# suchapalaver/krust

Measured on AMD Instinct MI355X. Metric: canonical k-mers/s at k=21, 100M x 150bp reads; bit-exact vs krust CPU, higher is better.
Workload: dtype u64; 1 GPU; S100M: 100000000 x 150 bp reads per GPU (rank r: reads [r x 100000000, (r + 1) x 100000000)), k=21, genome 2^27 bp, seed 20260130; resident in HBM; k=21, reads_per_gpu=100000000, distinct_per_gpu=1085824844, table_slots=2147483648, capacity_hint=1115311478, parallelism=reads sharded x1

## Files before the change

### krust_amd/csrc/batch.hip

```cpp
#include "ctx.hip.h"
#include "level1_api.h"

namespace khi {

template <bool QUAL>
void launch_count(kh_ctx *c, const uint8_t *abase, const uint8_t *qbase, int qaligned, u64 vbeg, u64 vend,
                  u64 wlo, u64 tile0, u64 ntiles) {
    u64 blocks = ntiles < (u64)grid_cap() ? ntiles : (u64)grid_cap();
    uint32_t tpb = (uint32_t)((ntiles + blocks - 1) / blocks);
    blocks = (ntiles + tpb - 1) / tpb;
    uint32_t thr = 0;
    if (QUAL) {
        int t = c->minq + 33;
        thr = (uint32_t)(t > 255 ? 255 : t);
    }
    hipLaunchKernelGGL(kh::count_direct_kernel<QUAL>, dim3((unsigned)blocks), dim3(kh::BLOCK), 0, c->stream, abase,
                       qbase, qaligned, vbeg, vend, wlo, tile0, ntiles, tpb, c->k, thr, table_geom(c, c->table, c->cap), c->d_ctr);
}

struct RangeArgs {
    const uint8_t *abase, *qbase;
    int qaligned;
    bool use_qual;
    u64 vbeg, vend, wlo;
    double survive = 1.0;
};

constexpr int KH_RETRY_FULL_SIZE = 1000;
constexpr int KH_RETRY_WIDE = 1001;

u64 sized_for(u64 n, double survive) {
    if (survive >= 1.0) return n;
    const double e = (double)n * (survive * 1.125 + 1.0 / 64) + 65536.0;
    return e >= (double)n ? n : (u64)e;
}

uint32_t qual_thr(const kh_ctx *c) {
    int t = c->minq + 33;
    return (uint32_t)(t > 255 ? 255 : t);
}

template <typename PT>
void launch_region(kh_ctx *c, const kh::PartGeom &g, u64 nregions, u64 hot, const u64 *bend, bool narrow, u64 skip, u64 expect);
bool region_small_groups(const kh_ctx *c, u64 expect, u64 nregions) {
    const int forced = c->knobs.region_nt;
    if (forced) return forced == 512;
    const double keys = c->est_keys ? (double)(c->distinct_known + c->est_keys) : c->hinted ? (double)c->hint_keys : (double)(c->distinct_known + expect);
    return !(keys > 0.6 * (double)c->cap && expect / nregions > 16384);
}
static bool want_heads(const kh_ctx *c) { return c->comm != nullptr || c->exports_seen || c->knobs.heads_always; }
template <>
void launch_region<u64>(kh_ctx *c, const kh::PartGeom &g, u64 nregions, u64 hot, const u64 *bend, bool, u64 skip, u64 expect) {
    const kh::TableGeom tg = table_geom(c, c->table, c->cap);
#define KH_REGION64(FRESH, NT) \
    hipLaunchKernelGGL((kh::region_count_kernel64<FRESH, NT>), dim3((unsigned)nregions), dim3(NT), 0, c->stream, tg, g, \
                       (const u64 *)c->keysB, bend, (const u64 *)c->bstart, c->rfail, c->rnew, hot, (uint32_t)c->table_dirty, c->rreal, skip)
    if (c->table_empty && region_small_groups(c, expect, nregions)) KH_REGION64(true, 512);
    else if (c->table_empty) KH_REGION64(true, kh::REGION_NT);
    else KH_REGION64(false, kh::REGION_NT);
#undef KH_REGION64
}
template <>
void launch_region<uint32_t>(kh_ctx *c, const kh::PartGeom &g, u64 nregions, u64 hot, const u64 *bend, bool narrow, u64 skip, u64 expect) {
    const kh::TableGeom tg = table_geom(c, c->table, c->cap);
    const int cb = (c->table_empty && !c->shard_shift && want_heads(c)) ? head_count_bits(c, nregions) : -1;
    c->rheads_cb = cb > 0 ? (uint32_t)cb : 0u;
    const bool pow2 = g.p2_bits != 0xFFFFFFFFu;
#define KH_REGION32_P(FRESH, NARROW, NT, DIRTY, CB, RH, P2) \
    hipLaunchKernelGGL((kh::region_count_kernel32<FRESH, NARROW, NT, P2>), dim3((unsigned)nregions), dim3(NT), 0, c->stream, tg, g, \
                       (const uint32_t *)c->keysB, bend, (const u64 *)c->bstart, c->rfail, c->rnew, hot, DIRTY, CB, RH, c->d_ctr, c->rreal, c->ntab, skip, \
                       (bend == (const u64 *)c->bend && g.p1_bits <= kh::MAX_P1_BITS) ? (const uint8_t *)c->heavy : (const uint8_t *)nullptr)
#define KH_REGION32(FRESH, NARROW, NT, DIRTY, CB, RH)                     \
    do {                                                                  \
        if (pow2) KH_REGION32_P(FRESH, NARROW, NT, DIRTY, CB, RH, true);  \
        else KH_REGION32_P(FRESH, NARROW, NT, DIRTY, CB, RH, false);      \
    } while (0)
    const bool small = region_small_groups(c, expect, nregions);
    if (c->table_empty && narrow && small) KH_REGION32(true, true, 512, 1u, c->rheads_cb, c->rheads);
    else if (c->table_empty && narrow) KH_REGION32(true, true, kh::REGION_NT, 1u, c->rheads_cb, c->rheads);
    else if (c->table_empty && small) KH_REGION32(true, false, 512, (uint32_t)c->table_dirty, c->rheads_cb, c->rheads);
    else if (c->table_empty) KH_REGION32(true, false, kh::REGION_NT, (uint32_t)c->table_dirty, c->rheads_cb, c->rheads);
    else if (narrow) KH_REGION32(false, true, kh::REGION_NT, 0u, 0u, (uint32_t *)nullptr);
    else KH_REGION32(false, false, kh::REGION_NT, 0u, 0u, (uint32_t *)nullptr);
#undef KH_REGION32
#undef KH_REGION32_P
}

constexpr double LOAD_SIZED = 0.50;
constexpr double LOAD_KEEP_MAX = 0.53;
constexpr double LOAD_KEEP_MIN = 0.36;
u64 policy_cap(double keys) {
    const u64 cap512 = 512ull * 1024 * kh::REGION_SLOTS;
    const double want = keys / LOAD_SIZED;
    if (want > (double)cap512 && keys / LOAD_KEEP_MAX <= (double)cap512) return cap512;
    return round_cap(std::max(want, (double)(2048ull * kh::REGION_SLOTS)));
}

template <typename PT>
int finish_batch(kh_ctx *c, const kh::PartGeom &g, PT *bufB, const u64 *bend, u64 nregions, u64 n_all, u64 n_ub, u64 ovf_lim, bool heavy_exact) {
    int rc;
    const bool was_empty = c->table_empty;
    const bool narrow_on = c->knobs.narrow;
    bool nar = sizeof(PT) == 4 && narrow_on && !c->narrow_banned && !c->shard_shift && (c->table_empty || c->narrow);
    if (nar && c->ntab_cap != c->cap) {
        if (c->ntab) {
            HIP_TRY(c, hipStreamSynchronize(c->stream));
            (void)dev_free(c->ntab);
            c->ntab = nullptr;
            c->ntab_cap = 0;
        }
        if (dev_malloc((void **)&c->ntab, c->cap * sizeof(u64)) != hipSuccess) {
            (void)hipGetLastError();
            c->ntab = nullptr;
            nar = false;
        } else {
            c->ntab_cap = c->cap;
        }
    }
    if (!nar && c->narrow && (rc = ensure_wide(c)) != KH_OK) return rc;
    if (!nar && (rc = need_table(c)) != KH_OK) return rc;
    if (nar) c->narrow_g = g;
    const u64 hot_cut = [&] {
        if (c->knobs.hot_cut) return c->knobs.hot_cut;
        return std::max<u64>(std::max<u64>(n_all >> 10, 1ull << 20), 64 * (n_all / nregions));
    }();
    if (hot_cut != ~0ull) {
        StageTimer t(c, ST_MISC);
        hipLaunchKernelGGL(kh::hot_list_kernel, dim3((unsigned)((nregions + kh::BLOCK - 1) / kh::BLOCK)), dim3(kh::BLOCK), 0, c->stream,
                           (const u64 *)c->bstart, bend, (u64)nregions, hot_cut, c->hot_list, c->d_ctr);
    }
    {
        StageTimer t(c, ST_REGION);
        launch_region<PT>(c, g, nregions, 4 * (n_ub / nregions) + 4096, bend, nar, hot_cut, n_ub);
    }
    if (nar) c->narrow = true;
    bool heads_marked = false;
    {
        StageTimer t(c, ST_MISC);
        hipLaunchKernelGGL(kh::region_reduce_kernel, dim3((unsigned)std::min<u64>(128, (nregions + kh::BLOCK - 1) / kh::BLOCK)), dim3(kh::BLOCK), 0, c->stream,
                           (const u64 *)c->bstart, (const uint8_t *)c->rfail, (const uint32_t *)c->rnew, (const u64 *)c->rreal, (u64)nregions, c->d_ctr);
        heads_marked = was_empty && sizeof(PT) == 4 && c->rheads_cb != 0 && c->ovf_pending && c->ovf_pending <= (64ull << 20) && !heavy_exact &&
                       mark_touched_regions(c, c->ovf_list, c->ovf, ovf_lim) == KH_OK;
        const int agg_env = c->knobs.ovf_agg;
        const bool ovf_agg = sizeof(PT) == 4 && agg_env != 0 && (agg_env == 1 || c->ovf_pending >= (1u << 16)) &&
                             (!nar || c->h_ctr->kmers + n_all < 0xFFFFFFFFull);
        if (c->ovf_pending && ovf_agg) {
            const unsigned grid = (unsigned)std::min<u64>(2048, (c->ovf_pending + 8191) / 8192);
            if (nar)
                hipLaunchKernelGGL((kh::ovf_agg_insert_kernel<true>), dim3(grid), dim3(kh::OVF_AGG_NT), 0, c->stream, table_geom(c, c->table, c->cap), g,
                                   (const kh::OvfEntry *)c->ovf_list, (const u64 *)c->ovf, ovf_lim, c->d_ctr, c->ntab);
            else
                hipLaunchKernelGGL((kh::ovf_agg_insert_kernel<false>), dim3(grid), dim3(kh::OVF_AGG_NT), 0, c->stream, table_geom(c, c->table, c->cap), g,
                                   (const kh::OvfEntry *)c->ovf_list, (const u64 *)c->ovf, ovf_lim, c->d_ctr, (u64 *)nullptr);
        } else if (c->ovf_pending) {
            if (nar)
                hipLaunchKernelGGL((kh::ovf_insert_kernel<PT, true>), dim3(grid_for(c->ovf_pending)), dim3(kh::BLOCK), 0, c->stream,
                                   table_geom(c, c->table, c->cap), g, c->ovf_list, (const u64 *)c->ovf, ovf_lim, c->d_ctr, c->ntab);
            else
                hipLaunchKernelGGL((kh::ovf_insert_kernel<PT, false>), dim3(grid_for(c->ovf_pending)), dim3(kh::BLOCK), 0, c->stream,
                                   table_geom(c, c->table, c->cap), g, c->ovf_list, (const u64 *)c->ovf, ovf_lim, c->d_ctr, (u64 *)nullptr);
        }
    }
    HIP_TRY(c, hipGetLastError());
    bool heads_recounted = false;
    if (heads_marked) heads_recounted = recount_touched_heads(c, nregions) == KH_OK;
    c->table_empty = false;
    c->table_dirty = false;
    c->launches++;
    c->part_batches++;

    rc = sync_counters(c);
    if (rc != KH_OK) return rc;
    c->rheads_valid = was_empty && sizeof(PT) == 4 && c->rheads_cb != 0 && c->h_ctr->part_failed == 0 && (c->ovf_pending == 0 || heads_recounted) &&
                      !(nar && c->h_ctr->narrow_ovf);
    c->rheads_wide = c->h_ctr->heads_wide != 0;
    if (nar && c->h_ctr->narrow_ovf) {
        if ((rc = ensure_wide(c)) != KH_OK) return rc;
        c->narrow_banned = true;
        HIP_TRY(c, hipMemsetAsync(&c->d_ctr->narrow_ovf, 0, sizeof(u64), c->stream));
        hipLaunchKernelGGL((kh::ovf_insert_kernel<PT, false>), dim3(grid_for(c->ovf_pending)), dim3(kh::BLOCK), 0, c->stream,
                           table_geom(c, c->table, c->cap), g, c->ovf_list, (const u64 *)c->ovf, ovf_lim, c->d_ctr, (u64 *)nullptr);
        HIP_TRY(c, hipGetLastError());
        if ((rc = sync_counters(c)) != KH_OK) return rc;
    }
    if (c->h_ctr->part_failed) {
        std::vector<uint8_t> hf(nregions);
        std::vector<u64> hb(nregions), he(nregions);
        HIP_TRY(c, hipMemcpy(hf.data(), c->rfail, nregions, hipMemcpyDeviceToHost));
        HIP_TRY(c, hipMemcpy(hb.data(), c->bstart, nregions * sizeof(u64), hipMemcpyDeviceToHost));
        HIP_TRY(c, hipMemcpy(he.data(), bend, nregions * sizeof(u64), hipMemcpyDeviceToHost));
        u64 failed_keys = 0;
        bool any_full = false, any_count = false;
        for (u64 r = 0; r < nregions; ++r)
            if (hf[r]) {
                failed_keys += he[r] - hb[r];
                any_full |= hf[r] == 1;
                any_count |= hf[r] == 2;
            }
        if (any_count) c->narrow_banned = true;
        if ((rc = ensure_wide(c)) != KH_OK) return rc;
        u64 newcap = c->cap;
        if (any_full) {
            newcap *= 2;
            while ((double)(c->distinct_known + failed_keys) > LOAD_HARD * (double)newcap ||
                   (double)c->distinct_known > LOAD_TARGET * (double)newcap)
                newcap *= 2;
            c->hinted = false;
        } else {
            while ((double)(c->distinct_known + failed_keys) > LOAD_HARD * (double)newcap) newcap *= 2;
        }
        if (c->trace)
            fprintf(stderr, any_full ? "[kmerhip] %llu regions overflowed (%llu keys): growing and re-inserting them directly\n"
                                     : "[kmerhip] a count left 32 bits in %llu regions (%llu keys): 16-byte table from here on, re-inserting them directly\n",
                    (u64)c->h_ctr->part_failed, failed_keys);
        {
            StageTimer t(c, ST_GROW);
            if (newcap != c->cap) {
                rc = grow_to(c, newcap);
                if (rc != KH_OK) return rc;
            }
            hipLaunchKernelGGL(kh::failed_buckets_insert_kernel<PT>, dim3((unsigned)nregions), dim3(kh::BLOCK), 0, c->stream,
                               table_geom(c, c->table, c->cap), g, (const PT *)bufB, (const u64 *)c->bstart, bend,
                               (const uint8_t *)c->rfail, c->d_ctr);
            HIP_TRY(c, hipMemsetAsync(&c->d_ctr->part_failed, 0, sizeof(u64), c->stream));
        }
        HIP_TRY(c, hipGetLastError());
        rc = sync_counters(c);
        if (rc != KH_OK) return rc;
    }
    if (c->h_ctr->hot) {
        const u64 nhot = c->h_ctr->hot, hot_total = c->h_ctr->hot_total;
        const bool crowded = nhot > nregions / 64 && (double)(c->distinct_known + hot_total) > LOAD_HARD * (double)c->cap;
        const bool hot_narrow = sizeof(PT) == 4 && c->narrow && !crowded && c->h_ctr->kmers + hot_total < 0xFFFFFFFFull;
        if (c->trace)
            fprintf(stderr, "[kmerhip] %llu hot bucket(s) (more than %llu payloads each, %llu together) counted apart from the region pass%s\n", nhot,
                    hot_cut, hot_total, hot_narrow ? ", into the 8-byte image" : "");
        if (!hot_narrow && (rc = ensure_wide(c)) != KH_OK) return rc;
        if (crowded) {
            u64 newcap = c->cap * 2;
            while ((double)(c->distinct_known + hot_total) > LOAD_TARGET * (double)newcap) newcap *= 2;
            StageTimer t(c, ST_GROW);
            if ((rc = grow_to(c, newcap)) != KH_OK) return rc;
        }
        {
            StageTimer t(c, ST_MISC);
            if (hot_narrow)
                hipLaunchKernelGGL((kh::hot_buckets_kernel<PT, sizeof(PT) == 4>), dim3(kh::HOT_GRID), dim3(kh::BLOCK), 0, c->stream, table_geom(c, c->table, c->cap), g,
                                   (const PT *)bufB, (const u64 *)c->bstart, bend, (const uint32_t *)c->hot_list, nhot, c->d_ctr, c->ntab);
            else
                hipLaunchKernelGGL((kh::hot_buckets_kernel<PT, false>), dim3(kh::HOT_GRID), dim3(kh::BLOCK), 0, c->stream, table_geom(c, c->table, c->cap), g,
                                   (const PT *)bufB, (const u64 *)c->bstart, bend, (const uint32_t *)c->hot_list, nhot, c->d_ctr, (u64 *)nullptr);
            HIP_TRY(c, hipMemsetAsync(&c->d_ctr->hot, 0, 2 * sizeof(u64), c->stream));
        }
        HIP_TRY(c, hipGetLastError());
        c->rheads_valid = false;
        if ((rc = sync_counters(c)) != KH_OK) return rc;
    }
    if ((double)c->distinct_known > LOAD_PART * (double)c->cap) {
        u64 newcap = c->cap * 2;
        while ((double)c->distinct_known > LOAD_TARGET * (double)newcap) newcap *= 2;
        StageTimer t(c, ST_GROW);
        rc = grow_to(c, newcap);
        if (rc != KH_OK) return rc;
    }
    return KH_OK;
}

template <typename PT>
int partition_batch(kh_ctx *c, const RangeArgs &ra, GeomChoice &gc, u64 tile0, u64 ntiles, bool size_from_sample, double range_scale, bool sized_narrow, bool may_narrow) {
    constexpr bool CHUNKED = true;
    kh::PartGeom &g = gc.g;
    const u64 P1 = 1ull << g.p1_bits;
    const u64 n_all = ntiles * kh::PART_TILE;
    const bool estimated = ra.survive < 1.0;
    const u64 n_ub = sized_for(n_all, ra.survive);
    const u64 pool_chunks = (n_ub / kh::CHUNK_PAY) + (n_ub / kh::CHUNK_PAY) / 24 + (u64)PART_G1 * (P1 + kh::POOL_GRAB) + 1024;
    const u64 max_blocks = pool_chunks / kh::CPB + P1 + 1;
    int rc;
    {
        auto fixed = [&](auto **ptr, u64 entries, const char *what) -> int {
            u64 z = *ptr ? entries : 0;
            return ensure_buf(c, ptr, &z, entries, what);
        };
        if ((rc = fixed(&c->moff, (u64)kh::MAX_P1 + 1, "hipMalloc(moff)")) != KH_OK) return rc;
        if ((rc = fixed(&c->nch, (u64)kh::MAX_P1 + 1, "hipMalloc(nch)")) != KH_OK) return rc;
        if ((rc = fixed(&c->info, 8, "hipMalloc(info)")) != KH_OK) return rc;
        if ((rc = fixed(&c->pcount, (u64)kh::MAX_P1, "hipMalloc(pcount)")) != KH_OK) return rc;
        if ((rc = fixed(&c->pstart, (u64)kh::MAX_P1 + 1, "hipMalloc(pstart)")) != KH_OK) return rc;
        if ((rc = fixed(&c->pool_next, 1, "hipMalloc(pool_next)")) != KH_OK) return rc;
        if ((rc = fixed(&c->ptotal, (u64)kh::MAX_P1, "hipMalloc(ptotal)")) != KH_OK) return rc;
        if ((rc = fixed(&c->pcap, (u64)kh::MAX_P1, "hipMalloc(pcap)")) != KH_OK) return rc;
        if ((rc = fixed(&c->ovf, 4, "hipMalloc(ovf)")) != KH_OK) return rc;
        if ((rc = fixed(&c->heavy, (u64)kh::MAX_P1, "hipMalloc(heavy)")) != KH_OK) return rc;
    }
    if ((rc = ensure_buf(c, &c->blocks, &c->blocks_cap, max_blocks, "hipMalloc(blocks)")) != KH_OK) return rc;
    if (c->pool_cap < pool_chunks) {
        const u64 have = c->pool_cap;
        c->pool_cap = 0;
        u64 z = c->chunk_part ? have : 0;
        if ((rc = ensure_buf(c, &c->chunk_part, &z, pool_chunks, "hipMalloc(chunk_part)")) != KH_OK) return rc;
        z = c->fill8 ? have : 0;
        if ((rc = ensure_buf(c, &c->fill8, &z, pool_chunks, "hipMalloc(fill8)")) != KH_OK) return rc;
        z = c->plist ? have : 0;
        if ((rc = ensure_buf(c, &c->plist, &z, pool_chunks, "hipMalloc(plist)")) != KH_OK) return rc;
        c->pool_cap = pool_chunks;
    }
    const u64 a_bytes = pool_chunks * kh::CHUNK_PAY * sizeof(PT);
    if (c->key_cap < a_bytes) {
        u64 z = c->keysA ? c->key_cap : 0;
        c->key_cap = 0;
        if ((rc = ensure_buf(c, &c->keysA, &z, a_bytes, "hipMalloc(keysA)")) != KH_OK) return rc;
        c->key_cap = a_bytes;
    }
    const uint32_t est_np = size_from_sample ? (uint32_t)std::min<u64>(16, std::max<u64>(1, (2ull << 20) / std::max<u64>(1, n_ub / P1))) : 0u;
    constexpr uint32_t EST_P0 = 517;
    u64 est_slots = 0;
    uint32_t est_sub = 0;
    if (size_from_sample) {
        while (est_sub < 6 && (n_ub / P1) >> (est_sub + 1) >= (1ull << 19)) ++est_sub;
        est_slots = 1ull << 16;
        while (est_slots < 3 * (u64)est_np * ((n_ub / P1 >> est_sub) + 1)) est_slots *= 2;
        if ((rc = ensure_buf(c, &c->est_set, &c->est_set_cap, est_slots, "hipMalloc(distinct sample)")) != KH_OK) return rc;
    }

    const uint32_t tpb = (uint32_t)((ntiles + PART_G1 - 1) / PART_G1);
    const uint32_t thr = ra.use_qual ? qual_thr(c) : 0;
    const dim3 b1(kh::PART_NT);
    kh::ChunkSrc cs;
    cs.pay = c->keysA;
    cs.plist = c->plist;
    cs.fill8 = c->fill8;
    const uint32_t force_wide = c->knobs.p2_force_wide ? 1u : 0u;
    bool have_total = false;
    u64 batch_total = 0;

    {
        {
            StageTimer t(c, ST_MISC);
            HIP_TRY(c, hipMemsetAsync(c->chunk_part, 0xFF, pool_chunks * sizeof(uint16_t), c->stream));
            HIP_TRY(c, hipMemsetAsync(c->fill8, 0xFF, pool_chunks, c->stream));
            HIP_TRY(c, hipMemsetAsync(c->pcount, 0, kh::MAX_P1 * sizeof(uint32_t), c->stream));
            HIP_TRY(c, hipMemsetAsync(c->pool_next, 0, sizeof(u64), c->stream));
        }
        {
            StageTimer t(c, ST_P1_SCATTER);
            kh::L1Launch l1;
            l1.stream = c->stream;
            l1.grid = (unsigned)PART_G1;
            l1.abase = ra.abase;
            l1.qbase = ra.qbase;
            l1.qaligned = ra.qaligned;
            l1.use_qual = ra.use_qual;
            l1.vbeg = ra.vbeg;
            l1.vend = ra.vend;
            l1.wlo = ra.wlo;
            l1.tile0 = tile0;
            l1.ntiles = ntiles;
            l1.tiles_per_block = tpb;
            l1.k = c->k;
            l1.thr = thr;
            l1.g = g;
            l1.pool = c->keysA;
            l1.chunk_part = c->chunk_part;
            l1.fill8 = c->fill8;
            l1.pool_next = c->pool_next;
            l1.pool_chunks = pool_chunks;
            l1.ctr = c->d_ctr;
            l1.survive = ra.survive;
            l1.generic_k = c->knobs.generic_k;
            l1.legacy = c->knobs.p1_legacy;
            if (sizeof(PT) == 4) kh::launch_level1_32(l1, nullptr);
            else kh::launch_level1_64(l1, nullptr);
        }
#if KH_ABL
        if (c->knobs.stop_after_p1) {
            HIP_TRY(c, hipGetLastError());
            return sync_counters(c);
        }
#endif
        {
            StageTimer t(c, ST_MISC);
            HIP_TRY(c, hipMemsetAsync(c->ptotal, 0, kh::MAX_P1 * sizeof(u64), c->stream));
            hipLaunchKernelGGL(kh::chunk_hist_kernel, dim3(1024), dim3(1024), 0, c->stream, (const uint16_t *)c->chunk_part,
                               (const u64 *)c->pool_next, pool_chunks, c->pcount, (const uint8_t *)c->fill8, c->ptotal);
            if ((rc = device_scan(c, c->pcount, P1, c->pstart)) != KH_OK) return rc;
            hipLaunchKernelGGL(kh::part2_plan_chunked_kernel, dim3(1), dim3(1024), 0, c->stream, (const u64 *)c->pstart, g,
                               c->blocks, max_blocks, c->moff, c->nch, c->info, c->pcount, force_wide, (const uint8_t *)nullptr);
            hipLaunchKernelGGL(kh::chunk_list_kernel, dim3((unsigned)((pool_chunks + 16383) / 16384)), dim3(1024), 0, c->stream,
                               (const uint16_t *)c->chunk_part, (const u64 *)c->pool_next, pool_chunks, c->pcount, c->plist);
            if (size_from_sample) {
                u64 *est_out = c->info + 4;
                HIP_TRY(c, hipMemsetAsync(est_out, 0, 3 * sizeof(u64), c->stream));
                HIP_TRY(c, hipMemsetAsync(c->est_set, 0xFF, est_slots * sizeof(u64), c->stream));
                hipLaunchKernelGGL(kh::distinct_sample_kernel<PT>, dim3(1024), dim3(kh::BLOCK), 0, c->stream, cs, (const u64 *)c->pstart,
                                   EST_P0 % (uint32_t)(P1 - est_np + 1), est_np, est_sub, c->est_set, est_slots - 1, est_out);
            }
        }
        if (estimated || size_from_sample) {
            std::vector<u64> pt(kh::MAX_P1);
            u64 lost = 0, total = 0, est[3] = {0, 0, 0};
            HIP_TRY(c, hipMemcpyAsync(pt.data(), c->ptotal, kh::MAX_P1 * sizeof(u64), hipMemcpyDeviceToHost, c->stream));
            HIP_TRY(c, hipMemcpyAsync(&lost, &c->d_ctr->failed, sizeof(u64), hipMemcpyDeviceToHost, c->stream));
            if (size_from_sample) HIP_TRY(c, hipMemcpyAsync(est, c->info + 4, sizeof(est), hipMemcpyDeviceToHost, c->stream));
            HIP_TRY(c, hipStreamSynchronize(c->stream));
            for (u64 p = 0; p < P1; ++p) total += pt[p];
            have_total = true;
            batch_total = total;
            if (estimated && (lost || total > n_ub)) {
                HIP_TRY(c, hipMemsetAsync(&c->d_ctr->failed, 0, sizeof(u64), c->stream));
                if (c->trace)
                    fprintf(stderr, "[kmerhip] sized for %.3f of the windows (%llu payloads), found %llu%s: again at full size\n", ra.survive, n_ub,
                            total, lost ? " and more that did not fit the pool" : "");
                return KH_RETRY_FULL_SIZE;
            }
            if (size_from_sample) {
                double keys = (double)total;
                if (est[2] == 0 && est[1] > 0) keys = std::min((double)total, (double)est[0] * ((double)P1 / (double)est_np) * (double)(1u << est_sub));
                c->est_keys = (u64)(keys * range_scale) + 1;
                const double load_now = (double)c->est_keys / (double)c->cap;
                u64 newcap = c->cap;
                if (load_now > LOAD_KEEP_MAX || (!c->hinted && (load_now < LOAD_KEEP_MIN || c->cap < 2048ull * kh::REGION_SLOTS))) newcap = policy_cap((double)c->est_keys);
                if (c->hinted && newcap < c->cap) newcap = c->cap;
                newcap = std::min<u64>(newcap, (u64)kh::MAX_P1 * kh::MAX_B2 * kh::REGION_SLOTS);
                size_t fr = 0, tot = 0;
                if (hipMemGetInfo(&fr, &tot) == hipSuccess) {
                    u64 room = ((u64)fr + (c->table ? c->cap * sizeof(Slot) : 0) + (c->ntab ? c->ntab_cap * sizeof(u64) : 0)) / 3;
                    if (c->knobs.table_room_mb) room = c->knobs.table_room_mb << 20;
                    while (newcap > c->cap && newcap * sizeof(Slot) > room) {
                        u64 next = round_cap((double)newcap * 0.8);
                        if (next >= newcap) next = round_cap((double)newcap * 0.5);
                        if (next >= newcap) break;
                        newcap = std::max(next, c->cap);
                    }
                }
                if (sizeof(PT) == 8 && c->knobs.l2_narrow && c->shard_shift == 0 && (newcap & (newcap - 1)) && !c->knobs.table_regions) {
                    u64 p2cap = 2048ull * kh::REGION_SLOTS;
                    uint32_t rb = 11;
                    while (p2cap < newcap) {
                        p2cap <<= 1;
                        ++rb;
                    }
                    const int below = 2 * (int)c->k - (int)rb;
                    size_t fr2 = 0, tot2 = 0;
                    const u64 image_have = c->ntab ? c->ntab_cap * sizeof(u64) : 0, later = 7 * total > c->keyb_cap ? 7 * total - c->keyb_cap : 0;
                    const bool fits = p2cap == c->cap ||
                                      (hipMemGetInfo(&fr2, &tot2) == hipSuccess && p2cap * sizeof(u64) <= ((u64)fr2 + image_have) / 3 &&
                                       (u64)fr2 + image_have >= p2cap * sizeof(u64) + later + (6ull << 30));
                    if (below >= 1 && below <= 32 && rb <= kh::MAX_P1_BITS + kh::MAX_P2_BITS && fits && (!c->hinted || p2cap >= c->cap)) newcap = p2cap;
                }
                if (c->trace)
                    fprintf(stderr, "[kmerhip] %llu payloads, ~%llu distinct (sample: %llu of %llu in %u partition(s)%s): table %llu -> %llu slots, load %.3f\n", total,
                            c->est_keys, est[0], est[1], est_np, est[2] ? ", VOID" : "", c->cap, newcap, (double)c->est_keys / (double)newcap);
                if (newcap != c->cap) {
                    resize_empty_table(c, newcap);
                    c->sized_by_sample = true;
                    const GeomChoice g2 = make_geom(c, c->cap);
                    if (!g2.ok || g2.g.p1_bits != g.p1_bits || g2.use32 != gc.use32) return fail(c, KH_ERR_STATE, "table geometry changed under a running batch");
                    gc = g2;
                }
            }
        }
    }
    const u64 n_pay = have_total ? std::min(n_ub, batch_total) : n_ub;
    const u64 nregions = kh::part_regions(g);
    const u64 n2 = max_blocks * g.b2;
    if (c->h2_cap < n2) {
        const u64 have = c->h2_cap;
        c->h2_cap = 0;
        u64 z = c->H2 ? have : 0;
        if ((rc = ensure_buf(c, &c->H2, &z, n2, "hipMalloc(H2)")) != KH_OK) return rc;
        z = c->O2 ? have + 1 : 0;
        if ((rc = ensure_buf(c, &c->O2, &z, n2 + 1, "hipMalloc(O2)")) != KH_OK) return rc;
        c->h2_cap = n2;
    }
    if ((rc = ensure_region_scratch(c, nregions)) != KH_OK) return rc;
    const bool lines_on = c->knobs.p2_lines;
    const bool lines = lines_on && g.b2 >= 2 && g.b2 <= 512;
    const bool arena_on = c->knobs.l2_arena;
    const bool arena = arena_on && g.p1_bits >= 8 && g.b2 >= 32 && g.b2 <= kh::MAX_B2;
    const u64 arena_pay = arena ? (n_pay + nregions) + ((n_pay + nregions) >> 2) + 1056ull * nregions : 0;
    const u64 ovf_need = arena ? n_pay / 16 + 2 * P1 * 8192ull + (1ull << 20) : 0;
    const u64 pad_ub = lines ? (max_blocks * g.b2) * (u64)(kh::P2L<PT>::UNIT - 1) : 0;
    const u64 heavy_room = arena ? n_pay / 8 : 0;
    const u64 heavy_base = (arena_pay + 31) & ~31ull;
    const u64 heavy_pad = (arena && lines) ? ((heavy_room / (kh::CPB * kh::CHUNK_PAY) + 2 * P1) * g.b2) * (u64)(kh::P2L<PT>::UNIT - 1) : 0;
    const int below_region_bits = 2 * (int)c->k - (int)g.shard_shift - (int)g.p1_bits - (g.p2_bits != 0xFFFFFFFFu ? (int)g.p2_bits : 64);
    const bool can_narrow = sizeof(PT) == 8 && arena && c->knobs.l2_narrow && may_narrow && g.p2_bits != 0xFFFFFFFFu && g.p2_bits >= 5 && g.b2 <= kh::MAX_B2 &&
                            below_region_bits >= 1 && below_region_bits <= 32 && g.shard_shift == 0;
    const u64 b_bytes_wide = std::max((n_pay + pad_ub) * (u64)sizeof(PT), arena ? (heavy_base + heavy_room + heavy_pad + 64) * (u64)sizeof(PT) : 0);
    const u64 b_bytes = can_narrow ? (arena_pay + 64) * (u64)sizeof(uint32_t) : b_bytes_wide;
    auto room_for_wide = [&]() -> int {
        if (c->keyb_cap >= b_bytes_wide) return KH_OK;
        size_t fr = 0, tot = 0;
        if (hipMemGetInfo(&fr, &tot) != hipSuccess) {
            (void)hipGetLastError();
            fr = 0;
        }
        if (sized_narrow && ((u64)fr + c->keyb_cap < b_bytes_wide + (c->table ? 0 : c->cap * sizeof(Slot)) + (4ull << 30) || c->knobs.l2_no_room_wide)) return KH_RETRY_WIDE;
        u64 z = c->keysB ? c->keyb_cap : 0;
        c->keyb_cap = 0;
        const int r = ensure_buf(c, &c->keysB, &z, b_bytes_wide, "hipMalloc(keysB)");
        if (r == KH_OK) c->keyb_cap = b_bytes_wide;
        return r;
    };
    if (!can_narrow) {
        if ((rc = room_for_wide()) != KH_OK) return rc;
    } else if (c->keyb_cap < b_bytes) {
        u64 z = c->keysB ? c->keyb_cap : 0;
        c->keyb_cap = 0;
        if ((rc = ensure_buf(c, &c->keysB, &z, b_bytes, "hipMalloc(keysB)")) != KH_OK) return rc;
        c->keyb_cap = b_bytes;
    }
    PT *bufA = reinterpret_cast<PT *>(c->keysA), *bufB = reinterpret_cast<PT *>(c->keysB);
    if (arena && c->ovf_cap < ovf_need) {
        u64 z = c->ovf_list ? c->ovf_cap : 0;
        c->ovf_cap = 0;
        if ((rc = ensure_buf(c, &c->ovf_list, &z, ovf_need, "hipMalloc(ovf_list)")) != KH_OK) return rc;
        c->ovf_cap = ovf_need;
    }
    const u64 *bend = c->bstart + 1;
    bool arena_done = false, heavy_exact = false;
    const u64 ovf_test_cap = c->knobs.l2_ovf_cap;
    const u64 ovf_lim = std::min(c->ovf_cap, ovf_test_cap);
    bool narrowed = false;
    if (arena) {
        u64 hov[4] = {0, 0, 0, 0};
        for (int attempt = can_narrow ? 0 : 1; attempt < 2; ++attempt) {
            const bool nw = attempt == 0;
            StageTimer t(c, ST_P2_SCATTER);
            const uint32_t skew_x = c->knobs.l2_skew_x >= 0 ? (uint32_t)c->knobs.l2_skew_x : 2u;
            const u64 room = std::min<u64>(heavy_room, c->knobs.l2_heavy_room);
            hipLaunchKernelGGL(kh::arena_plan_kernel, dim3((unsigned)std::min<u64>(64, (nregions + 1023) / 1024)), dim3(1024), 0, c->stream, (const u64 *)c->ptotal, g, c->bstart, c->pcap,
                               c->ovf, skew_x, c->heavy, room);
#define KH_ARENA(UB, NBK, P2)                                                                                                              \
    hipLaunchKernelGGL((kh::part2_arena_kernel<PT, UB, NBK, P2>), dim3((unsigned)P1), dim3(kh::P2L_NT), 0, c->stream, cs, (const u64 *)c->pstart, g, \
                       (const u64 *)c->bstart, (const uint32_t *)c->pcap, bufB, c->bend, c->ovf_list, c->ovf, ovf_lim, (const uint8_t *)c->heavy)
            const bool pow2 = g.p2_bits != 0xFFFFFFFFu;
            constexpr int UB512 = sizeof(PT) == 4 ? KH_ARENA_UNITB : 64;
#define KH_ARENA_NARROW(UB, NBK)                                                                                                           \
    hipLaunchKernelGGL((kh::part2_arena_kernel<uint32_t, UB, NBK, true, u64>), dim3((unsigned)P1), dim3(kh::P2L_NT), 0, c->stream, cs, (const u64 *)c->pstart, g, \
                       (const u64 *)c->bstart, (const uint32_t *)c->pcap, (uint32_t *)c->keysB, c->bend, c->ovf_list, c->ovf, ovf_lim, (const uint8_t *)c->heavy)
            if (nw) {
                if constexpr (sizeof(PT) == 8) {
                    if (g.b2 > 512) KH_ARENA_NARROW(64, 1024);
                    else KH_ARENA_NARROW(KH_ARENA_UNITB, 512);
                }
            } else
            if (g.b2 > 768) {
                if (pow2) KH_ARENA(64, 1024, true);
                else KH_ARENA(64, 1024, false);
            } else if (g.b2 > 512) {
#ifndef KH_ARENA_UNITB_768
#define KH_ARENA_UNITB_768 128
#endif
                if (KH_ARENA_UNITB_768 == 128 && sizeof(PT) == 4 && g.b2 <= 682) KH_ARENA(128, 768, false);
                else KH_ARENA(64, 768, false);
            } else if (pow2) {
                KH_ARENA(UB512, 512, true);
            } else {
                KH_ARENA(UB512, 512, false);
            }
#undef KH_ARENA
#undef KH_ARENA_NARROW
            t.stop();
            HIP_TRY(c, hipMemcpyAsync(hov, c->ovf, sizeof(hov), hipMemcpyDeviceToHost, c->stream));
            HIP_TRY(c, hipStreamSynchronize(c->stream));
            if (nw && (hov[1] != 0 || hov[2] != 0)) {
                if (c->trace) fprintf(stderr, "[kmerhip] level 2 narrowed to 4-byte payloads met %s: again with 8-byte payloads\n", hov[1] ? "a full overflow list" : "heavy partitions");
                if ((rc = room_for_wide()) != KH_OK) return rc;
                bufB = reinterpret_cast<PT *>(c->keysB);
                continue;
            }
            narrowed = nw;
            break;
        }
        if (hov[1] == 0) {
            arena_done = true;
            heavy_exact = hov[2] != 0;
            bend = c->bend;
            c->ovf_pending = std::min<u64>(hov[0], ovf_lim);
            HIP_TRY(c, hipMemsetAsync(c->rfail, 0, nregions, c->stream));
            if (c->trace && c->ovf_pending)
                fprintf(stderr, "[kmerhip] level 2: %llu entries handed out to the overflow list (%.2f %% of the batch's payload room)\n", (u64)c->ovf_pending,
                        100.0 * (double)c->ovf_pending / (double)n_ub);
            if (heavy_exact && c->trace)
                fprintf(stderr, "[kmerhip] %llu heavy level-1 partition(s) (%llu payloads) take the exact level-2 kernels, the others the arenas\n", hov[2], hov[3]);
        } else if (c->trace) {
            fprintf(stderr, hov[1] == 2 ? "[kmerhip] heavy level-1 partitions hold %llu payloads, more than the room behind the arenas: this batch takes the exact level-2 path\n"
                                        : "[kmerhip] level-2 overflow list full (%llu entries): this batch takes the exact path\n", (u64)(hov[1] == 2 ? hov[3] : hov[0]));
        }
    }
    if (!arena_done || heavy_exact) {
    PT *const outB = heavy_exact ? bufB + heavy_base : bufB;
    {
        StageTimer t(c, ST_MISC);
        if (heavy_exact || size_from_sample)
            hipLaunchKernelGGL(kh::part2_plan_chunked_kernel, dim3(1), dim3(1024), 0, c->stream, (const u64 *)c->pstart, g,
                               c->blocks, max_blocks, c->moff, c->nch, c->info, c->pcount, force_wide, heavy_exact ? (const uint8_t *)c->heavy : (const uint8_t *)nullptr);
        HIP_TRY(c, hipMemsetAsync(c->H2, 0, n2 * sizeof(uint32_t), c->stream));
    }
    {
        StageTimer t(c, heavy_exact ? ST_MISC : ST_P2_COUNT);
        hipLaunchKernelGGL((kh::part2_count_kernel<PT, CHUNKED>), dim3((unsigned)max_blocks), b1, 0, c->stream, (const PT *)bufA, cs,
                           (const kh::Part2Block *)c->blocks, (const u64 *)c->info, g, c->H2, lines ? (uint32_t)kh::P2L<PT>::UNIT : 1u);
    }
    {
        StageTimer t(c, ST_MISC);
        if ((rc = device_scan(c, c->H2, n2, c->O2)) != KH_OK) return rc;
    }
    {
        StageTimer t(c, ST_P2_SCATTER);
        const uint32_t fallback = lines ? 1u : 0u;
        if (lines)
            hipLaunchKernelGGL((kh::part2_scatter_lines_kernel<PT, CHUNKED>), dim3((unsigned)max_blocks), dim3(kh::P2L_NT), 0, c->stream,
                               (const PT *)bufA, cs, (const kh::Part2Block *)c->blocks, (const u64 *)c->info, g, (const u64 *)c->O2, outB);
        if (g.b2 <= 512)
            hipLaunchKernelGGL((kh::part2_scatter_kernel<PT, CHUNKED, 512>), dim3((unsigned)max_blocks), dim3(kh::PART2_NT), 0, c->stream,
                               (const PT *)bufA, cs, (const kh::Part2Block *)c->blocks, (const u64 *)c->info, g, (const u64 *)c->O2, outB, fallback);
        else
            hipLaunchKernelGGL((kh::part2_scatter_kernel<PT, CHUNKED, 1024>), dim3((unsigned)max_blocks), dim3(kh::PART2_NT), 0, c->stream,
                               (const PT *)bufA, cs, (const kh::Part2Block *)c->blocks, (const u64 *)c->info, g, (const u64 *)c->O2, outB, fallback);
    }
#if KH_ABL2 || KH_ABL3
    if (c->knobs.stop_after_p2) {
        HIP_TRY(c, hipGetLastError());
        return sync_counters(c);
    }
#endif
    {
        StageTimer t(c, ST_MISC);
        if (heavy_exact) {
            hipLaunchKernelGGL(kh::bucket_bounds_heavy_kernel, dim3((unsigned)((nregions + 255) / 256)), dim3(256), 0, c->stream,
                               (const u64 *)c->O2, (const u64 *)c->moff, (const uint32_t *)c->nch, g, (const uint8_t *)c->heavy, heavy_base,
                               c->bstart, c->bend);
        } else {
            hipLaunchKernelGGL(kh::bucket_bounds_kernel, dim3((unsigned)((nregions + 256) / 256)), dim3(256), 0, c->stream,
                               (const u64 *)c->O2, (u64)n2, (const u64 *)c->moff, (const uint32_t *)c->nch, g, c->bstart);
            HIP_TRY(c, hipMemsetAsync(c->rfail, 0, nregions, c->stream));
        }
    }
    if (!heavy_exact) c->ovf_pending = 0;
    }
    if (narrowed) {
        kh::PartGeom g2 = g;
        g2.p1_bits = g.p1_bits + g.p2_bits;
        g2.b2 = 1;
        g2.b2_magic = kh::part_magic_of(1);
        g2.p2_bits = 0;
        g2.defer = 0;
        c->narrow2_refused = false;
        if (c->trace) fprintf(stderr, "[kmerhip] level 2 narrowed the batch's payloads to the %d bits below the region index\n", below_region_bits);
        return finish_batch<uint32_t>(c, g2, reinterpret_cast<uint32_t *>(c->keysB), bend, nregions, n_all, n_ub, ovf_lim, false);
    }
    return finish_batch<PT>(c, g, bufB, bend, nregions, n_all, n_ub, ovf_lim, heavy_exact);
}

int direct_range(kh_ctx *c, const RangeArgs &ra, u64 first_tile, u64 end_tile) {
    {
        int rc = ensure_wide(c);
        if (rc == KH_OK) rc = clear_if_dirty(c);
        if (rc != KH_OK) return rc;
    }
    u64 t = first_tile;
    u64 sub = SUB_TILES;
    while (t < end_tile) {
        u64 nt = std::min(sub, end_tile - t);
        bool smaller = false;
        int rc = ensure_room(c, nt * kh::TILE, nt > SUB_TILES_MIN, &smaller);
        if (rc != KH_OK) return rc;
        if (smaller) {
            sub = std::max(SUB_TILES_MIN, nt / 4);
            continue;
        }
        {
            StageTimer tm(c, ST_DIRECT);
            if (ra.use_qual) launch_count<true>(c, ra.abase, ra.qbase, ra.qaligned, ra.vbeg, ra.vend, ra.wlo, t, nt);
            else launch_count<false>(c, ra.abase, nullptr, 0, ra.vbeg, ra.vend, ra.wlo, t, nt);
        }
        HIP_TRY(c, hipGetLastError());
        c->table_empty = false;
        c->rheads_valid = false;
        c->launches++;
        c->pending_bound += nt * kh::TILE;
        t += nt;
    }
    return KH_OK;
}

void ensure_part_budget(kh_ctx *c) {
    if (c->part_budget) return;
    size_t fr = 0, tot = 0;
    u64 budget = 224ull << 30;
    const double share = 0.80;
    if (hipMemGetInfo(&fr, &tot) == hipSuccess) {
        budget = std::min<u64>(budget, (u64)((double)(fr + c->key_cap + c->keyb_cap) * share));
        const u64 image = c->ntab ? 0 : 8ull * c->cap;
        if (c->prev_part_budget > budget && (u64)fr + c->key_cap + c->keyb_cap >= c->prev_part_budget + image + (3ull << 30)) budget = c->prev_part_budget;
    } else (void)hipGetLastError();
    if (c->knobs.part_budget_gb > 0) budget = (u64)(c->knobs.part_budget_gb * (double)(1ull << 30));
    c->part_budget = std::max<u64>(budget, 64ull << 20);
}

int count_device_range(kh_ctx *c, const uint8_t *d_bases, const uint8_t *d_qual, u64 n, u64 wlo_off) {
    if (n == 0) return KH_OK;
    const uintptr_t addr = (uintptr_t)d_bases;
    const u64 lead = addr & 15;
    RangeArgs ra;
    ra.abase = d_bases - lead;
    ra.vbeg = lead;
    ra.vend = lead + n;
    ra.wlo = lead + wlo_off;
    ra.use_qual = (d_qual != nullptr) && (c->minq >= 0);
    ra.qbase = nullptr;
    ra.qaligned = 0;
    if (ra.use_qual) {
        ra.qbase = d_qual - lead;
        ra.qaligned = (((uintptr_t)ra.qbase) & 15) == 0;
    }
    const u64 windows = ra.vend - ra.wlo;

    bool part = false;
    if (c->path_mode == 2) part = true;
    else if (c->path_mode == 0) part = windows >= PART_MIN_WINDOWS && (double)c->cap <= 7.0 * (double)windows;
    if (part) ensure_part_budget(c);
    const bool tight = part && (double)windows * 11.0 > 0.85 * (double)c->part_budget;
    if (part && (ra.use_qual || (windows >= (64ull << 20) && (tight || !c->hinted)))) {
        if (c->knobs.survival > 0) {
            ra.survive = std::min(1.0, c->knobs.survival);
        } else {
            const u64 t0 = ra.wlo / kh::TILE, t1 = (ra.vend + kh::TILE - 1) / kh::TILE, stride = 64;
            const u64 nsamp = (t1 - t0 + stride - 1) / stride;
            u64 *d_out = &c->d_ctr->cursor;
            u64 good = 0;
            StageTimer tm(c, ST_MISC);
            HIP_TRY(c, hipMemsetAsync(d_out, 0, sizeof(u64), c->stream));
            if (ra.use_qual)
                hipLaunchKernelGGL(kh::survival_sample_kernel<true>, dim3((unsigned)std::min<u64>(nsamp, 2048)), dim3(kh::BLOCK), 0, c->stream, ra.abase, ra.qbase,
                                   ra.qaligned, ra.vbeg, ra.vend, ra.wlo, t0, t1 - t0, stride, c->k, qual_thr(c), d_out);
            else
                hipLaunchKernelGGL(kh::survival_sample_kernel<false>, dim3((unsigned)std::min<u64>(nsamp, 2048)), dim3(kh::BLOCK), 0, c->stream, ra.abase, (const uint8_t *)nullptr,
                                   0, ra.vbeg, ra.vend, ra.wlo, t0, t1 - t0, stride, c->k, 0u, d_out);
            HIP_TRY(c, hipMemcpyAsync(&good, d_out, sizeof(u64), hipMemcpyDeviceToHost, c->stream));
            HIP_TRY(c, hipStreamSynchronize(c->stream));
            ra.survive = std::min(1.0, (double)good / (double)(nsamp * kh::TILE));
        }
        if (c->trace) fprintf(stderr, "[kmerhip] %s range: %.3f of the windows expected to survive\n", ra.use_qual ? "quality-masked" : "unhinted", ra.survive);
    }
    const bool sample = part && c->estimate_on && c->table_empty && c->shard_shift == 0 && c->k >= kh::MAX_P1_BITS && windows >= PART_MIN_WINDOWS;
    c->est_keys = 0;
    if (sample && c->cap < 2048ull * kh::REGION_SLOTS) {
        HIP_TRY(c, hipStreamSynchronize(c->stream));
        resize_empty_table(c, 2048ull * kh::REGION_SLOTS);
    }
    if (part && !c->hinted && !sample) {
        if (c->pending_bound) {
            int rc = sync_counters(c);
            if (rc != KH_OK) return rc;
        }
        u64 limit = c->cap;
        size_t fr = 0, tot = 0;
        if (hipMemGetInfo(&fr, &tot) == hipSuccess) {
            const u64 bytes = ((u64)fr + (c->table ? c->cap * sizeof(Slot) : 0)) / 4;
            u64 lim = MIN_CAP;
            while (lim * 2 * sizeof(Slot) <= bytes) lim *= 2;
            limit = std::max(limit, lim);
        }
        u64 expect = sized_for(windows, ra.survive);
        if (c->new_rate >= 0.0) expect = std::min<u64>(expect, (u64)((double)windows * std::max(c->new_rate * 1.5, 1.0 / 16)) + (1u << 20));
        const u64 want = std::min(round_cap((double)(c->distinct_known + expect) / LOAD_PART), limit);
        if (want > c->cap) {
            if (c->table_empty) {
                HIP_TRY(c, hipStreamSynchronize(c->stream));
                resize_empty_table(c, want);
            } else {
                StageTimer t(c, ST_GROW);
                int rc = grow_to(c, want);
                if (rc != KH_OK) c->poisoned = false;
            }
        }
    }
    if (part && !make_geom(c, c->cap).ok) part = false;

    if (!part) return direct_range(c, ra, ra.wlo / kh::TILE, (ra.vend + kh::TILE - 1) / kh::TILE);

    if (c->pending_bound) {
        int rc = sync_counters(c);
        if (rc != KH_OK) return rc;
    }
    if (c->borrow_on) {
        int rc = end_borrow(c);
        if (rc != KH_OK) return rc;
    }
    ensure_part_budget(c);
    const u64 first_tile = ra.wlo / kh::PART_TILE;
    const u64 end_tile = (ra.vend + kh::PART_TILE - 1) / kh::PART_TILE;
    const u64 distinct_before = c->distinct_known;
    bool no_narrow = false;
    for (u64 t = first_tile; t < end_tile;) {
        const GeomChoice gc = make_geom(c, c->cap);
        if (!gc.ok) return direct_range(c, ra, t * (kh::PART_TILE / kh::TILE), (ra.vend + kh::TILE - 1) / kh::TILE);
        const int rb_now = (int)kh::kh_floor_log2((uint32_t)std::min<u64>(c->cap / kh::REGION_SLOTS, 1u << 20));
        const bool expect_narrow = !gc.use32 && !no_narrow && !c->narrow2_refused && c->knobs.l2_narrow && c->shard_shift == 0 && c->knobs.l2_arena &&
                                   (c->table_empty ? (sample && 2 * (int)c->k - 20 <= 32) : (cap_is_pow2(c->cap) && rb_now >= 15 && 2 * (int)c->k - rb_now <= 32 && 2 * (int)c->k - rb_now >= 1));
        const u64 per_key = gc.use32 ? 11 : (expect_narrow ? 15 : 20);
        const u64 left = end_tile - t;
        const double share = (double)sized_for(left * kh::PART_TILE, ra.survive) / (double)(left * kh::PART_TILE);
        u64 batch_tiles = std::max<u64>(1, (u64)((double)(c->part_budget / per_key / kh::PART_TILE) / share));
        const u64 nb = (left + batch_tiles - 1) / batch_tiles;
        batch_tiles = (left + nb - 1) / nb;
        const u64 nt = std::min(batch_tiles, left);
        GeomChoice gcb = gc;
        const bool from_sample = sample && t == first_tile && gcb.g.p1_bits == kh::MAX_P1_BITS;
        const double range_scale = (double)(end_tile - first_tile) / (double)nt;
        int rc = gcb.use32 ? partition_batch<uint32_t>(c, ra, gcb, t, nt, from_sample, range_scale, false, false)
                           : partition_batch<u64>(c, ra, gcb, t, nt, from_sample, range_scale, expect_narrow, !no_narrow);
        if (rc == KH_RETRY_FULL_SIZE) {
            ra.survive = 1.0;
            continue;
        }
        if (rc == KH_RETRY_WIDE) {
            no_narrow = true;
            c->narrow2_refused = true;
            {
                size_t fr = 0, tot = 0;
                if (hipMemGetInfo(&fr, &tot) == hipSuccess) {
                    const u64 have = (u64)fr + c->key_cap + c->keyb_cap, tab = c->table ? 0 : c->cap * sizeof(Slot);
                    if (have > tab + (8ull << 30)) c->part_budget = std::min<u64>(c->part_budget, (u64)(0.9 * (double)(have - tab - (8ull << 30))));
                } else (void)hipGetLastError();
            }
            if (c->trace) fprintf(stderr, "[kmerhip] the batch was sized for 4-byte level-2 payloads and cannot have them: again in smaller batches\n");
            continue;
        }
        if (rc != KH_OK) return rc;
        t += nt;
    }
    c->new_rate = (double)(c->distinct_known - distinct_before) / (double)windows;
    return KH_OK;
}


}
```

### krust_amd/csrc/ctx.hip.h

```cpp
#pragma once
#include "../../include/kmerhip.h"

#include <hip/hip_runtime.h>
#include <sys/mman.h>

#include <algorithm>
#include <atomic>
#include <chrono>
#include <cstdio>
#include <cstdlib>
#include <cstring>
#include <functional>
#include <map>
#include <mutex>
#include <new>
#include <string>
#include <thread>
#include <type_traits>
#include <vector>

#include "alloc_inject.h"
#include "kernels.hip.h"
#include "partition.hip.h"

using kh::Counters;
using kh::Slot;
using kh::u64;

namespace khi __attribute__((visibility("hidden"))) {

constexpr double LOAD_HARD = 0.80;
constexpr double LOAD_TARGET = 0.50;
constexpr double HINT_LOAD = 0.65;
constexpr u64 MIN_CAP = 8ull * kh::REGION_SLOTS;
constexpr u64 DEFAULT_CAP = 1ull << 20;
constexpr u64 SUB_TILES = 1ull << 16;
constexpr u64 SUB_TILES_MIN = 1ull << 10;
constexpr u64 STAGE_BYTES = 64ull << 20;
constexpr u64 ACC_MAX = 8ull << 30;
constexpr u64 ACC_MIN = 1ull << 20;
constexpr u64 HALO = 32;
constexpr int GRID_CAP = 256 * 8;
#ifndef KH_ARENA_UNITB
#define KH_ARENA_UNITB 128
#endif
#ifndef KH_PART_G1
#define KH_PART_G1 512
#endif
constexpr int PART_G1 = KH_PART_G1;
constexpr u64 PART_MIN_WINDOWS = 1ull << 22;
constexpr double LOAD_PART = 0.70;
enum { ST_DIRECT = 0, ST_P1_COUNT, ST_P1_SCATTER, ST_P2_COUNT, ST_P2_SCATTER, ST_REGION, ST_MISC, ST_GROW, ST_N, ST_TEXT = ST_N };

struct Comm;

#ifndef KH_TESTING
#define KH_TESTING 0
#endif
struct Knobs {
    bool trace = false;
    int path = 0;
    double part_budget_gb = 0;
    u64 acc_max_mb = 0;
    u64 text_acc_mb = 0;
    int copy_threads = 0;
    bool estimate = true;
    bool pow2_table = false;
    int payload = 0;
    u64 table_regions = 0;
    int region_nt = 0;
    bool p2_force_wide = false;
    bool generic_k = false;
    bool p1_legacy = false;
    bool p2_lines = true;
    bool l2_arena = true;
    u64 l2_ovf_cap = ~0ull;
    int l2_skew_x = -1;
    u64 l2_heavy_room = ~0ull;
    bool narrow = true;
    bool l2_narrow = true;
    bool l2_no_room_wide = false;
    u64 hot_cut = 0;
    int ovf_agg = -1;
    double survival = 0;
    bool heads_always = false;
    u64 table_room_mb = 0;
    bool stop_after_p1 = false, stop_after_p2 = false;
    u64 profile_chunk_kb = 0;
    u64 uni_text_chunk_kb = 0;
};
inline const char *env_of(const char *name) {
    const char *e = getenv(name);
    return (e && *e) ? e : nullptr;
}
void read_knobs(Knobs &k);

#if KH_TESTING
extern std::atomic<int> g_grid_cap;
inline int grid_cap() { return g_grid_cap.load(std::memory_order_relaxed); }
#else
constexpr int grid_cap() { return GRID_CAP; }
#endif

#if KH_TESTING
bool alloc_inject_fails(const char *kind, size_t bytes);
void alloc_trace_event(char ev, const char *kind, const void *p, size_t bytes);
inline hipError_t dev_malloc(void **p, size_t bytes) {
    if (alloc_inject_fails("dev", bytes)) { *p = nullptr; return hipErrorOutOfMemory; }
    const hipError_t e = hipMalloc(p, bytes);
    if (e == hipSuccess) alloc_trace_event('A', "dev", *p, bytes);
    return e;
}
inline hipError_t pin_malloc(void **p, size_t bytes, unsigned flags) {
    if (alloc_inject_fails("pin", bytes)) { *p = nullptr; return hipErrorOutOfMemory; }
    const hipError_t e = hipHostMalloc(p, bytes, flags);
    if (e == hipSuccess) alloc_trace_event('A', "pin", *p, bytes);
    return e;
}
inline hipError_t dev_free(void *p) {
    if (p) alloc_trace_event('F', nullptr, p, 0);
    return hipFree(p);
}
inline hipError_t pin_free(void *p) {
    if (p) alloc_trace_event('F', nullptr, p, 0);
    return hipHostFree(p);
}
#else
inline hipError_t dev_malloc(void **p, size_t bytes) { return hipMalloc(p, bytes); }
inline hipError_t pin_malloc(void **p, size_t bytes, unsigned flags) { return hipHostMalloc(p, bytes, flags); }
inline hipError_t dev_free(void *p) { return hipFree(p); }
inline hipError_t pin_free(void *p) { return hipHostFree(p); }
#endif

}

struct kh_ctx {
    khi::Knobs knobs;
    int device = 0;
    khi::Comm *comm = nullptr;
    hipStream_t stream = nullptr;
    bool own_stream = false;
    uint32_t k = 0;
    int32_t minq = -1;
    uint32_t flags = 0;
    bool trace = false;

    Slot *table = nullptr;
    u64 cap = 0;
    u64 *ntab = nullptr;
    u64 ntab_cap = 0;
    bool narrow = false;
    bool narrow_banned = false;
    kh::PartGeom narrow_g;
    Counters *d_ctr = nullptr;
    Counters *h_ctr = nullptr;

    u64 distinct_known = 0;
    u64 pending_bound = 0;
    u64 bases_pushed = 0;
    u64 grows = 0;
    u64 launches = 0;
    double kernel_ms = 0.0;
    double h2d_ms = 0.0;

    hipStream_t cstream = nullptr;
    uint8_t *h_stage[2] = {nullptr, nullptr};
    u64 stage_bytes = 0;
    hipEvent_t stage_done[2] = {nullptr, nullptr};
    bool stage_used[2] = {false, false};
    int stage_next = 0;
    uint8_t *acc[2] = {nullptr, nullptr};
    u64 acc_cap = 0;
    int acc_cur = 0;
    u64 acc_len = 0;
    u64 acc_carry = 0;
    bool acc_qual = false;
    bool acc_has_qual = false;
    hipEvent_t acc_free[2] = {nullptr, nullptr};
    bool acc_busy[2] = {false, false};
    std::vector<std::pair<hipEvent_t, hipEvent_t>> h2d_events;

    bool table_empty = true;
    uint32_t win_piece = 0, win_n = 1;
    bool win_open = false, win_dirty = false;
    uint32_t win_open_n = 0;
    u64 win_mask = 0;
    bool table_dirty = false;
    bool hinted = false;
    u64 hint_keys = 0;
    double new_rate = -1.0;
    int path_mode = 0;
    int pay_mode = 0;
    uint32_t shard_shift = 0;
    uint32_t shard_index = 0;
    u64 *merge_off = nullptr;
    u64 merge_off_cap = 0;
    u64 part_budget = 0;
    u64 prev_part_budget = 0;
    uint8_t *keysA = nullptr, *keysB = nullptr;
    u64 key_cap = 0, keyb_cap = 0;
    bool exports_seen = false;
    bool borrow_on = false;
    u64 borrow_off[2] = {0, 0};
    bool table_borrowed = false;
    kh::Part2Block *blocks = nullptr;
    u64 blocks_cap = 0;
    u64 *moff = nullptr;
    uint32_t *nch = nullptr;
    u64 *info = nullptr;
    uint32_t *H2 = nullptr;
    u64 *O2 = nullptr;
    u64 h2_cap = 0;
    u64 *bstart = nullptr;
    uint8_t *rfail = nullptr;
    uint32_t *rnew = nullptr;
    u64 *rreal = nullptr;
    uint32_t *rheads = nullptr;
    bool rheads_valid = false;
    bool rheads_wide = false;
    uint32_t rheads_cb = 0;
    u64 *bend = nullptr;
    uint32_t *hot_list = nullptr;
    uint8_t *rtouch = nullptr;
    u64 *radd = nullptr;
    u64 *rdig = nullptr;
    u64 rdig_cap = 0;
    u64 *ptotal = nullptr;
    uint32_t *pcap = nullptr;
    uint8_t *heavy = nullptr;
    u64 *ovf = nullptr;
    kh::OvfEntry *ovf_list = nullptr;
    u64 ovf_cap = 0;
    u64 ovf_pending = 0;
    uint16_t *chunk_part = nullptr;
    uint8_t *fill8 = nullptr;
    uint32_t *plist = nullptr;
    u64 pool_cap = 0;
    uint32_t *pcount = nullptr;
    u64 *pstart = nullptr;
    u64 *pool_next = nullptr;
    u64 region_cap = 0;
    u64 *scan_partial = nullptr;
    u64 scan_cap = 0;
    u64 *est_set = nullptr;
    u64 est_set_cap = 0;
    u64 est_keys = 0;
    bool sized_by_sample = false;
    bool narrow2_refused = false;
    bool estimate_on = true;
    u64 part_batches = 0;
    double stage_ms[khi::ST_N] = {0};
    struct StageEv { int stage; hipEvent_t a, b; };
    std::vector<StageEv> stage_events;

    uint8_t *txt_raw2[2] = {nullptr, nullptr};  u64 txt_raw2_cap[2] = {0, 0};
    int txt_raw_next = 0;
    hipStream_t sstream = nullptr;
    hipEvent_t txt_copied[2] = {nullptr, nullptr};
    hipEvent_t txt_scanned[2] = {nullptr, nullptr};
    bool txt_scanned_on[2] = {false, false};
    hipStream_t cstream2 = nullptr;
    struct { bool on = false; int r = 0; u64 n = 0; int format = 0; } txt_unscanned;
    uint8_t *txt_acc[2] = {nullptr, nullptr};   u64 txt_acc_cap[2] = {0, 0};
    uint8_t *txt_accq[2] = {nullptr, nullptr};  u64 txt_accq_cap[2] = {0, 0};
    int txt_cur = 0;
    u64 txt_acc_len = 0;
    bool txt_acc_qual = false;
    hipEvent_t txt_acc_done[2] = {nullptr, nullptr};
    bool txt_acc_busy[2] = {false, false};
    hipStream_t txt_scan_stream = nullptr;
    u64 *txt_scan_partial = nullptr;  u64 txt_scan_cap = 0;
    u64 expect_bytes = 0;
    u64 *txt_ls = nullptr;        u64 txt_ls_cap = 0;
    uint8_t *txt_st = nullptr;    u64 txt_st_cap = 0;
    uint32_t *txt_tnl = nullptr;  u64 txt_tnl_cap = 0;
    u64 *txt_tbase = nullptr;     u64 txt_tbase_cap = 0;
    uint32_t *txt_tkeep = nullptr; u64 txt_tkeep_cap = 0;
    u64 *txt_tout = nullptr;      u64 txt_tout_cap = 0;
    uint32_t *txt_err = nullptr;  u64 txt_err_cap = 0;
    struct TxtHost { u64 total; u64 end_mark; uint32_t err; uint8_t first, last; } *h_txt = nullptr;
    double text_ms = 0.0;

    struct TextStream {
        bool on = false;
        uint32_t format = 0;
        u64 min_count = 0, ntiles = 0;
        u64 n_records = 0, rec_bytes = 0;
        u64 next_tile = 0;
        bool tail_done = false;
        std::vector<u64> toff;
        struct Chunk {
            uint8_t *d = nullptr;
            u64 cap = 0, len = 0, pos = 0;
            bool valid = false;
            hipEvent_t done = nullptr;
        } ch[2];
        int cur = 0;
        bool sorted = false;
        u64 sorted_n = 0;
    } ts;
    uint8_t *ts_own[2] = {nullptr, nullptr};  u64 ts_own_cap[2] = {0, 0};
    uint32_t *ts_trec = nullptr;  u64 ts_trec_cap = 0;
    uint32_t *ts_tbyt = nullptr;  u64 ts_tbyt_cap = 0;
    u64 *ts_roff = nullptr;       u64 ts_roff_cap = 0;
    u64 *ts_boff = nullptr;       u64 ts_boff_cap = 0;
    u64 *ts_skey = nullptr;       u64 ts_skey_cap = 0;
    u64 *ts_scnt = nullptr;       u64 ts_scnt_cap = 0;

    uint8_t *pf_d[2] = {nullptr, nullptr};
    uint8_t *pf_h[2] = {nullptr, nullptr};
    u64 pf_chunk = 0;
    u64 pf_out_bytes = 0;
    hipEvent_t pf_in[2] = {nullptr, nullptr}, pf_run[2] = {nullptr, nullptr}, pf_out[2] = {nullptr, nullptr};
    uint32_t *pr_rows = nullptr;  u64 pr_rows_cap = 0;
    u64 *pr_rec = nullptr;        u64 pr_rec_cap = 0;
    u64 *jn_words = nullptr;
    u64 *gr_words = nullptr;
    struct Unitigs {
        bool live = false;
        u64 *rows = nullptr;
        uint8_t *bases = nullptr;
        u64 n_unitigs = 0, n_bases = 0;
        bool linked = false;
        u64 *links = nullptr;
        u64 n_links = 0;
        u64 *where = nullptr;
        struct Text {
            bool on = false;
            uint32_t format = 0;
            u64 hdr = 0, rec_bytes = 0, link_bytes = 0, total = 0;
            u64 *off = nullptr;
            u64 chunk_bytes = 0;
            u64 next_off = 0;
            u64 sent = 0;
            struct Chunk {
                uint8_t *d = nullptr;
                u64 len = 0, pos = 0;
                bool valid = false;
                hipEvent_t done = nullptr;
            } ch[2];
            int cur = 0;
        } text;
    } un;

    bool poisoned = false;
    int poisoned_by = KH_OK;
    std::string last_error;
};

namespace khi __attribute__((visibility("hidden"))) {

inline int fail(kh_ctx *c, int code, const char *what, hipError_t e = hipSuccess) {
    if (c) {
        c->last_error = what;
        if (e != hipSuccess) {
            c->last_error += ": ";
            c->last_error += hipGetErrorString(e);
        }
        if (code == KH_ERR_HIP || code == KH_ERR_TABLE_FULL || code == KH_ERR_OOM) {
            if (!c->poisoned || code == KH_ERR_HIP) c->poisoned_by = code;
            c->poisoned = true;
        }
    }
    return code;
}
inline int soft_oom(kh_ctx *c, const char *what, hipError_t e = hipSuccess) {
    c->last_error = what;
    if (e != hipSuccess) {
        c->last_error += ": ";
        c->last_error += hipGetErrorString(e);
    }
    return KH_ERR_OOM;
}

#define HIP_TRY(c, call)                                              \
    do {                                                              \
        hipError_t e_ = (call);                                       \
        if (e_ != hipSuccess) return fail((c), KH_ERR_HIP, #call, e_); \
    } while (0)

inline int grid_for(u64 items) {
    u64 b = (items + kh::BLOCK - 1) / kh::BLOCK;
    if (b < 1) b = 1;
    if (b > (u64)grid_cap()) b = grid_cap();
    return (int)b;
}

struct Entry {
    bool flush_pending = true;
    bool need_table = true;
    bool keep_window = false;
    bool narrow_ok = false;
    bool reader = false;
};
constexpr Entry ENTER_WRITE{};
constexpr Entry ENTER_READ{true, true, false, true, true};
constexpr Entry ENTER_READ_TAKE{true, true, false, true, false};
constexpr Entry ENTER_PUSH{false, false, false, true, false};
constexpr Entry ENTER_PUSH_DEVICE{true, false, false, true, false};
constexpr Entry ENTER_TEXT_NEXT{false, false, false, true, true};
int enter(kh_ctx *c, Entry how = ENTER_WRITE);
int result_enter(kh_ctx *c, const void *keys, const void *counts, u64 cap, u64 min_count, uint64_t *n, uint64_t *need);
int need_table(kh_ctx *c);
void resize_empty_table(kh_ctx *c, u64 newcap);
int clear_if_dirty(kh_ctx *c);
int close_fresh_window(kh_ctx *c);
int ensure_wide(kh_ctx *c);
int sync_counters(kh_ctx *c);
u64 round_cap(double want);
kh::RegionGeom geom_of_cap(u64 cap);
bool cap_is_pow2(u64 cap);
kh::TableGeom table_geom(const kh_ctx *c, Slot *table, u64 cap);
int grow_to(kh_ctx *c, u64 newcap);
int ensure_room(kh_ctx *c, u64 bound, bool allow_shrink_hint, bool *want_smaller);
int drain_events(kh_ctx *c);
int ensure_region_scratch(kh_ctx *c, u64 nregions);
int release_part_buffers(kh_ctx *c);
void *borrow(kh_ctx *c, u64 bytes);
u64 borrow_room(const kh_ctx *c);
int end_borrow(kh_ctx *c);
void drop_table(kh_ctx *c);
struct CallScratch {
    kh_ctx *c;
    u64 loan0, loan1;
    bool lent = false;
    u64 used[2] = {0, 0};
    std::vector<void *> owned;
    explicit CallScratch(kh_ctx *ctx);
    ~CallScratch();
    CallScratch(const CallScratch &) = delete;
    CallScratch &operator=(const CallScratch &) = delete;
    void *take(u64 bytes);
    void *fresh(u64 bytes);
};
int device_scan(kh_ctx *c, const uint32_t *in, u64 n, u64 *out, bool soft = false, u64 *scratch = nullptr);
inline u64 device_scan_scratch(u64 n) { return ((n + kh::SCAN_CHUNK - 1) / kh::SCAN_CHUNK + 2) * sizeof(u64); }
int zero_cursors(kh_ctx *c);
int compact_pairs(kh_ctx *c, u64 *d_keys, u64 *d_counts, u64 cap, u64 min_count, u64 *n);
int read_cursor(kh_ctx *c, u64 *cursor, u64 *big);
int head_count_bits(const kh_ctx *c, u64 regions);
extern bool g_pow2_tables;
extern int g_copy_threads;
int count_device_range(kh_ctx *c, const uint8_t *d_bases, const uint8_t *d_qual, u64 n, u64 wlo_off);
int flush_acc(kh_ctx *c, bool carry);
int flush_text(kh_ctx *c);
int scan_unscanned(kh_ctx *c);
bool is_pinned_host(const void *p);
void staged_memcpy(void *dst, const void *src, size_t n);
int d2h_staged(kh_ctx *c, void *dst, const void *d_src, u64 bytes, hipEvent_t ready = nullptr);
enum { XF_WIDE = 0, XF_PACKED64 = 1, XF_HEADS32 = 2 };
int mark_touched_regions(kh_ctx *c, const void *ovf_list, const u64 *d_ovf, u64 ovf_lim);
int recount_touched_heads(kh_ctx *c, u64 nregions);
int export_regions(kh_ctx *c, int fmt, uint32_t nparts, void *d_keys, uint64_t *d_counts, uint64_t cap, uint32_t *d_region_counts,
                   uint64_t region_cap, uint64_t *part_counts, uint64_t *table_regions, u64 *d_digest = nullptr, bool *digest_done = nullptr);
int merge_regions(kh_ctx *c, int fmt, uint32_t nsenders, uint64_t sender_regions, const void *const *d_keys,
                  const uint64_t *const *d_counts, const uint32_t *const *d_region_counts, u64 *d_digest = nullptr, bool *digest_done = nullptr);
void comm_release(kh_ctx *c);
void text_release(kh_ctx *c);
int sorted_into(kh_ctx *c, u64 *out_keys, u64 *out_counts, u64 n, u64 min_count, CallScratch &sc);
int join_check(kh_ctx *err, const char *who, const kh_ctx *a, const kh_ctx *b, const kh_ctx *dst);
void unitigs_release(kh_ctx *c);
inline unsigned uni_grid(u64 items) { return (unsigned)grid_for(items); }
void unitigs_text_release(kh_ctx *c);
void profile_release(kh_ctx *c);
constexpr u64 PF_PAD = 64;
inline u64 pf_in_stride(u64 chunk) { return (chunk + PF_PAD + 15) & ~15ull; }
u64 profile_chunk(const kh_ctx *c, u64 n);
int profile_buffers(kh_ctx *c, u64 chunk, u64 out_bytes = 4, const char *who = "kh_profile: chunk buffers");
struct ChunkJob {
    u64 j, a, ns;
    const uint8_t *d_bases, *d_qual;
    u64 len;
    uint8_t *d_tail;
};
int chunk_pipeline(kh_ctx *c, const uint8_t *bases, const uint8_t *qual, u64 n, u64 chunk, u64 halo, void *out, u64 out_bytes,
                   const std::function<int(const ChunkJob &)> &launch);
inline bool qual_filter(const kh_ctx *c, const void *qual, uint32_t *thr = nullptr) {
    const bool on = qual != nullptr && c->minq >= 0;
    if (thr) *thr = on ? (uint32_t)std::min(c->minq + 33, 255) : 0u;
    return on;
}
struct ReadPlan {
    const uint8_t *abase, *qbase;
    int qaligned;
    u64 vbeg, vend, ntiles;
    uint32_t tpb, thr;
    unsigned blocks;
};
ReadPlan read_plan(const kh_ctx *c, const uint8_t *d_bases, const uint8_t *d_qual, u64 n, u64 nout);
int check_rec_start(kh_ctx *c, const char *who, const u64 *rec_start, u64 nrec, u64 n);
int enter_unitigs(kh_ctx *c, const char *who);
int locate_index(kh_ctx *c, const char *who);
int locate_range(kh_ctx *c, const uint8_t *d_bases, const uint8_t *d_qual, u64 n, u64 nout, u64 *d_out);

struct StageTimer {
    kh_ctx *c;
    int stage;
    hipEvent_t a = nullptr, b = nullptr;
    hipStream_t st_stream;
    StageTimer(kh_ctx *ctx, int st, hipStream_t s = nullptr) : c(ctx), stage(st), st_stream(s ? s : ctx->stream) {
        if (hipEventCreate(&a) == hipSuccess && hipEventCreate(&b) == hipSuccess) (void)hipEventRecord(a, st_stream);
    }
    void stop() {
        if (a && b) {
            (void)hipEventRecord(b, st_stream);
            c->stage_events.push_back({stage, a, b});
            a = b = nullptr;
        }
    }
    ~StageTimer() { stop(); }
};

inline double wall_ms() { return std::chrono::duration<double, std::milli>(std::chrono::steady_clock::now().time_since_epoch()).count(); }
template <typename T>
int ensure_buf(kh_ctx *c, T **ptr, u64 *cap, u64 need, const char *what, bool soft = false) {
    if (*cap >= need && *ptr) return KH_OK;
    const double t0 = c->trace ? wall_ms() : 0.0;
    struct Tr {
        kh_ctx *c; double t0; const char *what; u64 bytes;
        ~Tr() { if (c->trace && wall_ms() - t0 > 5.0) fprintf(stderr, "[kmerhip] %s: %.1f MB took %.1f ms\n", what, (double)bytes / 1e6, wall_ms() - t0); }
    } tr{c, t0, what, need * sizeof(T)};
    if (*ptr) {
        HIP_TRY(c, hipStreamSynchronize(c->stream));
        (void)dev_free(*ptr);
        *ptr = nullptr;
        *cap = 0;
    }
    hipError_t e = dev_malloc((void **)ptr, need * sizeof(T));
    if (e != hipSuccess) {
        (void)hipGetLastError();
        *ptr = nullptr;
        return soft ? soft_oom(c, what, e) : fail(c, KH_ERR_OOM, what, e);
    }
    *cap = need;
    return KH_OK;
}

struct GeomChoice {
    kh::PartGeom g;
    bool use32;
    bool ok;
// ... 6 lines not shown
```

### krust_amd/csrc/kmerhip.hip

```cpp
#include "ctx.hip.h"

namespace khi {

#if KH_TESTING
std::atomic<int> g_grid_cap{GRID_CAP};

static std::mutex g_alloc_mu;
static AllocInject g_alloc_inject;
void alloc_trace_event(char ev, const char *kind, const void *p, size_t bytes) {
    const char *path = env_of("KMERHIP_ALLOC_TRACE");
    if (!path) return;
    std::lock_guard<std::mutex> lk(g_alloc_mu);
    FILE *f = fopen(path, "a");
    if (!f) return;
    if (ev == 'A') fprintf(f, "A %s %p %zu\n", kind, p, bytes);
    else fprintf(f, "F %p\n", p);
    fclose(f);
}
bool alloc_inject_fails(const char *kind, size_t bytes) {
    std::lock_guard<std::mutex> lk(g_alloc_mu);
    const uint64_t ord = g_alloc_inject.step(env_of("KMERHIP_ALLOC_FAIL"));
    if (!ord) return false;
    if (const char *path = env_of("KMERHIP_ALLOC_TRACE"))
        if (FILE *f = fopen(path, "a")) {
// ... 225 lines not shown
        if (c->narrow)
            HIP_TRY(c, hipMemsetAsync(c->ntab + (u64)p * per_piece, 0, per_piece * sizeof(u64), c->stream));
        else
            hipLaunchKernelGGL(kh::table_init_kernel, dim3(grid_for(per_piece)), dim3(kh::BLOCK), 0, c->stream,
                               c->table + (u64)p * per_piece, per_piece);
    }
    HIP_TRY(c, hipGetLastError());
    return KH_OK;
}

int ensure_wide(kh_ctx *c) {
    if (!c->narrow) return KH_OK;
    {
        const int nrc = need_table(c);
        if (nrc != KH_OK) return nrc;
    }
    hipLaunchKernelGGL(kh::ntable_widen_kernel, dim3(grid_for(c->cap)), dim3(kh::BLOCK), 0, c->stream, (const u64 *)c->ntab, c->cap,
                       c->narrow_g, c->table);
    HIP_TRY(c, hipGetLastError());
    c->narrow = false;
    c->table_dirty = false;
    if (c->trace) fprintf(stderr, "[kmerhip] 8-byte table image widened to %llu 16-byte slots\n", c->cap);
    return KH_OK;
}

int sync_counters(kh_ctx *c) {
    HIP_TRY(c, hipMemcpyAsync(c->h_ctr, c->d_ctr, sizeof(Counters), hipMemcpyDeviceToHost, c->stream));
    HIP_TRY(c, hipStreamSynchronize(c->stream));
    c->distinct_known = c->h_ctr->distinct;
    c->pending_bound = 0;
    if (c->h_ctr->failed) return fail(c, KH_ERR_TABLE_FULL, "an upsert found no free slot");
    return KH_OK;
}

bool g_pow2_tables = false;
bool pow2_tables() { return g_pow2_tables; }
u64 round_cap(double want) {
    u64 cap = MIN_CAP;
    while ((double)cap < want && cap < 1024ull * kh::REGION_SLOTS) cap *= 2;
    if ((double)cap >= want) return cap;
    if (pow2_tables()) {
        while ((double)cap < want) cap *= 2;
        return cap;
    }
    const double per_b2 = 1024.0 * kh::REGION_SLOTS;
    u64 b2 = (u64)(want / per_b2);
    if ((double)b2 * per_b2 < want) ++b2;
    u64 step = 1;
    if (b2 > 64) {
        u64 top = 64;
        while (top * 2 < b2) top *= 2;
        step = std::min<u64>(top / 8, 64);
    } else {
        u64 q = 1;
        while (q < b2) q *= 2;
        b2 = q;
    }
    b2 = (b2 + step - 1) / step * step;
    return b2 * 1024ull * kh::REGION_SLOTS;
}
kh::RegionGeom geom_of_cap(u64 cap) { return kh::kh_geom_of_regions(cap / kh::REGION_SLOTS); }
bool cap_is_pow2(u64 cap) { return (cap & (cap - 1)) == 0; }

kh::TableGeom table_geom(const kh_ctx *c, Slot *table, u64 cap);

kh::TableGeom table_geom(const kh_ctx *c, Slot *table, u64 cap) {
    kh::TableGeom tg;
    tg.table = table;
    const kh::RegionGeom rg = geom_of_cap(cap);
    tg.p1_bits = rg.p1_bits;
    tg.b2 = rg.b2;
    tg.k = c->k;
    tg.shard_shift = c->shard_shift;
    tg.shard_index = c->shard_index;
    return tg;
}

int grow_to(kh_ctx *c, u64 newcap) {
    Slot *nt = nullptr;
    int rc = ensure_wide(c);
    if (rc != KH_OK) return rc;
    if (c->ntab) {
        HIP_TRY(c, hipStreamSynchronize(c->stream));
        (void)dev_free(c->ntab);
        c->ntab = nullptr;
        c->ntab_cap = 0;
    }
    if (!c->table) {
        resize_empty_table(c, newcap);
        c->grows++;
        return KH_OK;
    }
    rc = alloc_table(c, newcap, &nt);
    if (rc != KH_OK) return rc;
    if (c->table_dirty) {
        c->table_dirty = false;
    } else {
        hipLaunchKernelGGL(kh::table_rehash_kernel, dim3(grid_for(c->cap)), dim3(kh::BLOCK), 0, c->stream, c->table,
                           c->cap, table_geom(c, nt, newcap), c->d_ctr);
        HIP_TRY(c, hipGetLastError());
    }
    HIP_TRY(c, hipStreamSynchronize(c->stream));
    drop_table(c);
    if (c->trace) fprintf(stderr, "[kmerhip] table grown %llu -> %llu slots\n", c->cap, newcap);
    c->rheads_valid = false;
    c->table = nt;
    c->cap = newcap;
    c->grows++;
    return KH_OK;
}

int ensure_room(kh_ctx *c, u64 bound, bool allow_shrink_hint, bool *want_smaller) {
    if (want_smaller) *want_smaller = false;
    const double hard = LOAD_HARD * (double)c->cap;
    if ((double)(c->distinct_known + c->pending_bound + bound) <= hard) return KH_OK;
    if (c->pending_bound) {
        int rc = sync_counters(c);
        if (rc != KH_OK) return rc;
        if ((double)(c->distinct_known + bound) <= hard) return KH_OK;
    }
    if (allow_shrink_hint && want_smaller && (double)c->distinct_known <= LOAD_TARGET * (double)c->cap) {
        *want_smaller = true;
        return KH_OK;
    }
    u64 newcap = c->cap;
    while ((double)(c->distinct_known + bound) > LOAD_HARD * (double)newcap ||
           (double)c->distinct_known > LOAD_TARGET * (double)newcap)
        newcap *= 2;
    return grow_to(c, newcap);
}

int ensure_region_scratch(kh_ctx *c, u64 nregions) {
    if (c->region_cap >= nregions && c->bstart) return KH_OK;
    int rc;
    const u64 have = c->region_cap;
    u64 z = c->bstart ? have + 1 : 0;
    if ((rc = ensure_buf(c, &c->bstart, &z, nregions + 1, "hipMalloc(bstart)")) != KH_OK) return rc;
#define KH_REGION_ARRAY(field)                                                                    \
    z = c->field ? have : 0;                                                                      \
    if ((rc = ensure_buf(c, &c->field, &z, nregions, "hipMalloc(" #field ")")) != KH_OK) return rc
    KH_REGION_ARRAY(rfail);
    KH_REGION_ARRAY(rnew);
    KH_REGION_ARRAY(rheads);
    KH_REGION_ARRAY(rreal);
    KH_REGION_ARRAY(bend);
    KH_REGION_ARRAY(hot_list);
    KH_REGION_ARRAY(radd);
    KH_REGION_ARRAY(rtouch);
#undef KH_REGION_ARRAY
    HIP_TRY(c, hipMemsetAsync(c->rtouch, 0, nregions, c->stream));
    c->region_cap = nregions;
    c->rheads_valid = false;
    return KH_OK;
}

int drain_events(kh_ctx *c) {
    for (auto &e : c->stage_events) {
        float ms = 0.f;
        if (hipEventElapsedTime(&ms, e.a, e.b) == hipSuccess) {
            if (e.stage == ST_TEXT) {
                c->text_ms += ms;
            } else {
                c->stage_ms[e.stage] += ms;
                c->kernel_ms += ms;
            }
        }
        (void)hipEventDestroy(e.a);
        (void)hipEventDestroy(e.b);
    }
    c->stage_events.clear();
    for (auto &p : c->h2d_events) {
        float ms = 0.f;
        if (hipEventElapsedTime(&ms, p.first, p.second) == hipSuccess) c->h2d_ms += ms;
        (void)hipEventDestroy(p.first);
        (void)hipEventDestroy(p.second);
    }
    c->h2d_events.clear();
    return KH_OK;
}

int release_part_buffers(kh_ctx *c) {
    if (!c->keysA && !c->keysB) return KH_OK;
    int brc = end_borrow(c);
    if (brc != KH_OK) return brc;
    HIP_TRY(c, hipStreamSynchronize(c->stream));
    if (c->keysA) (void)dev_free(c->keysA);
    if (c->keysB) (void)dev_free(c->keysB);
    c->keysA = c->keysB = nullptr;
    c->key_cap = c->keyb_cap = 0;
    c->prev_part_budget = c->part_budget;
    c->part_budget = 0;
    return KH_OK;
}

GeomChoice make_geom(const kh_ctx *c, u64 cap) {
    GeomChoice gc;
    const int hbits = 2 * (int)c->k - (int)c->shard_shift;
    uint32_t p1, b2;
    if (cap_is_pow2(cap)) {
        uint32_t rbits = 0;
        while (((u64)kh::REGION_SLOTS << (rbits + 1)) <= cap) ++rbits;
        uint32_t p2 = std::min<uint32_t>(rbits, kh::MAX_P2_BITS);
        p1 = rbits - p2;
        const int need = hbits - 32;
        if (need > (int)p1 && need <= (int)kh::MAX_P1_BITS && need <= (int)rbits) {
            p1 = (uint32_t)need;
            p2 = rbits - p1;
        }
        if (rbits > kh::MAX_P1_BITS && c->shard_shift == 0 && c->k >= kh::MAX_P1_BITS) {
            p1 = kh::MAX_P1_BITS;
            p2 = rbits - p1;
        }
        if (p1 == 0 && rbits >= 1 && (hbits > 32 || c->pay_mode == 64)) {
            p1 = 1;
            p2 = rbits - 1;
        }
        gc.ok = p1 <= kh::MAX_P1_BITS && p2 <= kh::MAX_P2_BITS;
        b2 = p2 <= 20 ? 1u << p2 : 0u;
    } else {
        const kh::RegionGeom rg = geom_of_cap(cap);
        p1 = rg.p1_bits;
        b2 = rg.b2;
        gc.ok = p1 == kh::MAX_P1_BITS && b2 <= kh::MAX_B2 && c->shard_shift == 0;
    }
    gc.g.p1_bits = p1;
    gc.g.b2 = b2 ? b2 : 1u;
    gc.g.b2_magic = kh::part_magic_of(gc.g.b2);
    gc.g.p2_bits = kh::part_p2_bits_of(gc.g.b2);
    gc.g.k = c->k;
    gc.g.shard_shift = c->shard_shift;
    gc.g.shard_index = c->shard_index;
    gc.use32 = (hbits - (int)p1) <= 32 && c->pay_mode != 64;
    gc.g.defer = (gc.use32 && kh::p1_fast_ok(gc.g)) ? 1u : 0u;
    return gc;
}

int device_scan(kh_ctx *c, const uint32_t *in, u64 n, u64 *out, bool soft, u64 *scratch) {
    const u64 nb = (n + kh::SCAN_CHUNK - 1) / kh::SCAN_CHUNK;
    if (!scratch) {
        int rc = ensure_buf(c, &c->scan_partial, &c->scan_cap, nb + 2, "hipMalloc(scan)", soft);
        if (rc != KH_OK) return rc;
        scratch = c->scan_partial;
    }
    hipLaunchKernelGGL(kh::scan_partials_kernel, dim3((unsigned)nb), dim3(kh::SCAN_NT), 0, c->stream, in, n, scratch);
    hipLaunchKernelGGL(kh::scan_spine_kernel, dim3(1), dim3(1024), 0, c->stream, scratch, nb);
    hipLaunchKernelGGL(kh::scan_apply_kernel, dim3((unsigned)nb), dim3(kh::SCAN_NT), 0, c->stream, in, n,
                       (const u64 *)scratch, out);
    HIP_TRY(c, hipGetLastError());
    return KH_OK;
}
int head_count_bits(const kh_ctx *c, u64 regions) {
    const int hb = kh::kh_below_bits(c->k, 0, kh::kh_geom_of_regions(regions));
    return (hb >= 1 && hb <= 28) ? 32 - hb : -1;
}

}
using namespace khi;

extern "C" int kh_abi_version(void) { return KMERHIP_ABI_VERSION; }

extern "C" int kh_create(kh_ctx **out, const kh_config *cfg) {
    if (!out || !cfg) return KH_ERR_BAD_ARG;
    *out = nullptr;
    if (cfg->struct_size != sizeof(kh_config)) return KH_ERR_BAD_ARG;
    if (cfg->k < 1 || cfg->k > 32) return KH_ERR_BAD_K;
    if (cfg->min_quality < -1 || cfg->min_quality > 255) return KH_ERR_BAD_ARG;
    int ndev = 0;
    if (hipGetDeviceCount(&ndev) != hipSuccess || ndev <= 0) {
        (void)hipGetLastError();
        return KH_ERR_NO_DEVICE;
    }
    int dev = cfg->device;
    if (dev < 0 && hipGetDevice(&dev) != hipSuccess) return KH_ERR_NO_DEVICE;
    if (dev >= ndev) return KH_ERR_BAD_ARG;

    kh_ctx *c = new (std::nothrow) kh_ctx();
    if (!c) return KH_ERR_OOM;
    c->device = dev;
    c->k = cfg->k;
    c->minq = cfg->min_quality;
    c->flags = cfg->flags;
    read_knobs(c->knobs);
    g_pow2_tables = c->knobs.pow2_table;
    if (!g_copy_threads) g_copy_threads = c->knobs.copy_threads;
    c->trace = (cfg->flags & KH_FLAG_TRACE) || c->knobs.trace;
    c->expect_bytes = (u64)cfg->input_mib << 20;
    c->hinted = cfg->capacity_hint != 0;
    c->hint_keys = cfg->capacity_hint;
    c->path_mode = (cfg->flags & KH_FLAG_FORCE_DIRECT) ? 1 : (cfg->flags & KH_FLAG_FORCE_PARTITION) ? 2 : 0;
    if (c->knobs.path) c->path_mode = c->knobs.path;
    c->pay_mode = c->knobs.payload;
    c->estimate_on = c->knobs.estimate;

    int rc = KH_OK;
    do {
        if (hipSetDevice(dev) != hipSuccess) { rc = KH_ERR_NO_DEVICE; break; }
        if (cfg->stream || (cfg->flags & KH_FLAG_CALLER_STREAM)) {
            c->stream = (hipStream_t)cfg->stream;
        } else {
            if (hipStreamCreateWithFlags(&c->stream, hipStreamNonBlocking) != hipSuccess) { rc = KH_ERR_HIP; break; }
            c->own_stream = true;
        }
        if (dev_malloc((void **)&c->d_ctr, sizeof(Counters)) != hipSuccess) { rc = KH_ERR_OOM; break; }
        if (pin_malloc((void **)&c->h_ctr, sizeof(Counters), hipHostMallocDefault) != hipSuccess) { rc = KH_ERR_OOM; break; }
        if (hipMemsetAsync(c->d_ctr, 0, sizeof(Counters), c->stream) != hipSuccess) { rc = KH_ERR_HIP; break; }
        u64 cap = cfg->capacity_hint ? round_cap((double)cfg->capacity_hint / HINT_LOAD) : DEFAULT_CAP;
        if (const u64 nr = c->knobs.table_regions)
            if (kh::kh_regions_valid(nr) && nr * kh::REGION_SLOTS >= MIN_CAP) cap = nr * kh::REGION_SLOTS;
        c->cap = cap;
        if (hipStreamSynchronize(c->stream) != hipSuccess) { rc = KH_ERR_HIP; break; }
    } while (0);
    if (rc != KH_OK) {
        kh_destroy(c);
        return rc;
    }
    *out = c;
    return KH_OK;
}

extern "C" void kh_destroy(kh_ctx *c) {
    if (!c) return;
    (void)hipSetDevice(c->device);
    if (c->stream) (void)hipStreamSynchronize(c->stream);
    comm_release(c);
    drain_events(c);
    if (c->cstream) (void)hipStreamSynchronize(c->cstream);
    text_release(c);
    if (c->cstream2) (void)hipStreamSynchronize(c->cstream2);
    profile_release(c);
    unitigs_release(c);
    for (int i = 0; i < 2; ++i) {
        if (c->h_stage[i]) (void)pin_free(c->h_stage[i]);
        if (c->acc[i]) (void)dev_free(c->acc[i]);
        if (c->stage_done[i]) (void)hipEventDestroy(c->stage_done[i]);
        if (c->acc_free[i]) (void)hipEventDestroy(c->acc_free[i]);
    }
    if (c->cstream) (void)hipStreamDestroy(c->cstream);
    void *scratch[] = {c->keysA, c->keysB, c->blocks, c->moff, c->nch, c->info, c->H2, c->O2,
                       c->bstart, c->bend, c->hot_list, c->ptotal, c->pcap, c->heavy, c->ovf, c->ovf_list, c->rfail, c->rnew, c->rreal, c->rheads, c->radd, c->rdig, c->rtouch, c->scan_partial, c->est_set, c->merge_off, c->chunk_part, c->fill8, c->plist,
                       c->pcount, c->pstart, c->pool_next, c->txt_raw2[0], c->txt_raw2[1], c->txt_acc[0], c->txt_acc[1], c->txt_accq[0], c->txt_accq[1], c->txt_scan_partial, c->txt_ls, c->txt_st,
                       c->txt_tnl, c->txt_tbase, c->txt_tkeep, c->txt_tout, c->txt_err, c->jn_words, c->gr_words};
    for (void *q : scratch)
        if (q) (void)dev_free(q);
    drop_table(c);
    if (c->ntab) (void)dev_free(c->ntab);
    if (c->d_ctr) (void)dev_free(c->d_ctr);
    if (c->h_ctr) (void)pin_free(c->h_ctr);
    if (c->h_txt) (void)pin_free(c->h_txt);
    for (int i = 0; i < 2; ++i) {
        if (c->txt_acc_done[i]) (void)hipEventDestroy(c->txt_acc_done[i]);
        if (c->txt_copied[i]) (void)hipEventDestroy(c->txt_copied[i]);
        if (c->txt_scanned[i]) (void)hipEventDestroy(c->txt_scanned[i]);
    }
    if (c->sstream) {
        (void)hipStreamSynchronize(c->sstream);
        (void)hipStreamDestroy(c->sstream);
    }
    if (c->cstream2) {
        (void)hipStreamSynchronize(c->cstream2);
        (void)hipStreamDestroy(c->cstream2);
    }
    if (c->own_stream && c->stream) (void)hipStreamDestroy(c->stream);
    delete c;
}

extern "C" int kh_reset(kh_ctx *c) {
    if (c && c->win_open) {
        c->win_open = false;
        if (c->win_dirty) c->table_dirty = true;
    }
    const bool revived = c && c->poisoned && c->poisoned_by != KH_ERR_HIP;
    if (revived) {
        c->poisoned = false;
        c->poisoned_by = KH_OK;
    }
    int rc = enter(c, ENTER_PUSH);
    if (rc != KH_OK) return rc;
    if (c->cstream) HIP_TRY(c, hipStreamSynchronize(c->cstream));
    c->acc_len = c->acc_carry = 0;
    c->txt_acc_len = 0;
    if (c->sstream) HIP_TRY(c, hipStreamSynchronize(c->sstream));
    c->txt_unscanned.on = false;
    HIP_TRY(c, hipStreamSynchronize(c->stream));
    drain_events(c);
    unitigs_release(c);
    if (!c->table_empty || revived) c->table_dirty = true;
    if (c->table_borrowed) drop_table(c);
    c->borrow_on = false;
    c->borrow_off[0] = c->borrow_off[1] = 0;
    c->narrow = false;
    c->narrow_banned = false;
    c->new_rate = -1.0;
    c->est_keys = 0;
    c->rheads_valid = false;
    HIP_TRY(c, hipMemsetAsync(c->d_ctr, 0, sizeof(Counters), c->stream));
    memset(c->h_ctr, 0, sizeof(Counters));
    c->distinct_known = c->pending_bound = 0;
    c->bases_pushed = 0;
    c->launches = 0;
    c->kernel_ms = c->h2d_ms = c->text_ms = 0.0;
    for (double &m : c->stage_ms) m = 0.0;
    c->table_empty = true;
    c->part_batches = 0;
    c->shard_shift = c->shard_index = 0;
    return KH_OK;
}

extern "C" int kh_finish(kh_ctx *c, kh_stats *st) {
    int rc = enter(c, ENTER_READ);
    if (rc != KH_OK) return rc;
    rc = sync_counters(c);
    if (rc != KH_OK) return rc;
    if (c->cstream) HIP_TRY(c, hipStreamSynchronize(c->cstream));
    drain_events(c);
    if (st) {
        st->bases = c->bases_pushed;
        st->kmers = c->h_ctr->kmers;
        st->distinct = c->h_ctr->distinct;
        st->table_slots = c->cap;
        st->grows = c->grows;
        st->launches = c->launches;
        st->count_kernel_ms = c->kernel_ms;
        st->h2d_ms = c->h2d_ms;
        st->part_batches = c->part_batches;
        for (int i = 0; i < KH_NUM_STAGES; ++i) st->stage_ms[i] = i < ST_N ? c->stage_ms[i] : 0.0;
        st->text_scan_ms = c->text_ms;
        st->slot_bytes = c->narrow ? 8 : 16;
    }
    if (c->trace)
        fprintf(stderr, "[kmerhip] bases=%llu kmers=%llu distinct=%llu slots=%llu load=%.3f launches=%llu kernel=%.3f ms h2d=%.3f ms | direct=%.2f p1c=%.2f p1s=%.2f p2c=%.2f p2s=%.2f region=%.2f misc=%.2f grow=%.2f\n",
                (u64)c->bases_pushed, c->h_ctr->kmers, c->h_ctr->distinct, c->cap,
                (double)c->h_ctr->distinct / (double)c->cap, (u64)c->launches, c->kernel_ms, c->h2d_ms,
                c->stage_ms[0], c->stage_ms[1], c->stage_ms[2], c->stage_ms[3], c->stage_ms[4], c->stage_ms[5],
                c->stage_ms[6], c->stage_ms[7]);
    return KH_OK;
}


namespace khi {

int zero_cursors(kh_ctx *c) {
    HIP_TRY(c, hipMemsetAsync(&c->d_ctr->cursor, 0, 2 * sizeof(u64), c->stream));
    return KH_OK;
}

int read_cursor(kh_ctx *c, u64 *cursor, u64 *big) {
    HIP_TRY(c, hipMemcpyAsync(c->h_ctr, c->d_ctr, sizeof(Counters), hipMemcpyDeviceToHost, c->stream));
    HIP_TRY(c, hipStreamSynchronize(c->stream));
    if (cursor) *cursor = c->h_ctr->cursor;
    if (big) *big = c->h_ctr->big;
    return KH_OK;
}

}

extern "C" int kh_result_size(kh_ctx *c, uint64_t min_count, uint64_t *n) {
    int rc = enter(c, ENTER_READ);
    if (rc != KH_OK) return rc;
    if (!n) return fail(c, KH_ERR_BAD_ARG, "n is NULL");
    rc = zero_cursors(c);
    if (rc != KH_OK) return rc;
    if (c->narrow)
        hipLaunchKernelGGL(kh::ntable_count_kernel, dim3(grid_for(c->cap)), dim3(kh::BLOCK), 0, c->stream, (const u64 *)c->ntab,
                           c->cap, (u64)min_count, c->d_ctr);
    else
    hipLaunchKernelGGL(kh::table_count_kernel, dim3(grid_for(c->cap)), dim3(kh::BLOCK), 0, c->stream, c->table,
                       c->cap, (u64)min_count, c->d_ctr);
    HIP_TRY(c, hipGetLastError());
    u64 cur = 0;
    rc = read_cursor(c, &cur, nullptr);
    if (rc != KH_OK) return rc;
    *n = cur;
    return KH_OK;
}

namespace khi {
int compact_pairs(kh_ctx *c, u64 *d_keys, u64 *d_counts, u64 cap, u64 min_count, u64 *n) {
    int rc = zero_cursors(c);
    if (rc != KH_OK) return rc;
    if (c->narrow)
        hipLaunchKernelGGL(kh::ntable_compact_kernel, dim3(grid_for(c->cap)), dim3(kh::BLOCK), 0, c->stream, (const u64 *)c->ntab,
                           c->cap, c->narrow_g, (u64)min_count, (u64 *)d_keys, (u64 *)d_counts, (u64)cap, c->d_ctr);
    else
    hipLaunchKernelGGL(kh::table_compact_kernel, dim3(grid_for(c->cap)), dim3(kh::BLOCK), 0, c->stream, c->table,
                       c->cap, (u64)min_count, (u64 *)d_keys, (u64 *)d_counts, (u64)cap, c->d_ctr);
    HIP_TRY(c, hipGetLastError());
    u64 cur = 0;
    rc = read_cursor(c, &cur, nullptr);
    if (rc != KH_OK) return rc;
    *n = cur < cap ? cur : cap;
    if (cur > cap) return fail(c, KH_ERR_RANGE, "output arrays too small");
    return KH_OK;
}
}

extern "C" int kh_result_copy_device(kh_ctx *c, uint64_t *d_keys, uint64_t *d_counts, uint64_t cap,
                                     uint64_t min_count, uint64_t *n) {
    int rc = enter(c, ENTER_READ_TAKE);
    if (rc != KH_OK) return rc;
    if (!n || (cap && (!d_keys || !d_counts))) return fail(c, KH_ERR_BAD_ARG, "NULL output");
    return compact_pairs(c, (u64 *)d_keys, (u64 *)d_counts, cap, min_count, (u64 *)n);
}

namespace khi {
int result_enter(kh_ctx *c, const void *keys, const void *counts, u64 cap, u64 min_count, uint64_t *n, uint64_t *need) {
    int rc = enter(c, ENTER_READ_TAKE);
    if (rc != KH_OK) return rc;
    if (!n || (cap && (!keys || !counts))) return fail(c, KH_ERR_BAD_ARG, "NULL output");
    *n = 0;
    if ((rc = kh_result_size(c, min_count, need)) != KH_OK) return rc;
    if (*need > cap) return fail(c, KH_ERR_RANGE, "output arrays too small");
    return KH_OK;
}
}

extern "C" int kh_result_copy(kh_ctx *c, uint64_t *keys, uint64_t *counts, uint64_t cap, uint64_t min_count,
                              uint64_t *n) {
    uint64_t need = 0;
    int rc = result_enter(c, keys, counts, cap, min_count, n, &need);
    if (rc != KH_OK || need == 0) return rc;
    CallScratch sc(c);
    uint64_t *const dk = (uint64_t *)sc.take(need * sizeof(u64));
    uint64_t *const dc = dk ? (uint64_t *)sc.take(need * sizeof(u64)) : nullptr;
    if (!dc) return soft_oom(c, "hipMalloc(result)");
    uint64_t got = 0;
    rc = kh_result_copy_device(c, dk, dc, need, min_count, &got);
    if (rc == KH_OK) rc = d2h_staged(c, keys, dk, got * sizeof(u64));
    if (rc == KH_OK) rc = d2h_staged(c, counts, dc, got * sizeof(u64));
    if (rc == KH_OK) *n = got;
    return rc;
}

extern "C" int kh_histogram(kh_ctx *c, uint64_t min_count, uint64_t *count, uint64_t *freq, uint64_t cap,
                            uint64_t *n) {
    int rc = enter(c, ENTER_READ);
    if (rc != KH_OK) return rc;
    if (!n || (cap && (!count || !freq))) return fail(c, KH_ERR_BAD_ARG, "NULL output");
    u64 big_cap = 1ull << 16;
    std::vector<u64> dense(kh::HIST_DENSE), big;
    for (int attempt = 0; attempt < 2; ++attempt) {
        CallScratch sc(c);
        u64 *const d_dense = (u64 *)sc.fresh(kh::HIST_DENSE * sizeof(u64));
        u64 *const d_big = d_dense ? (u64 *)sc.fresh(big_cap * sizeof(u64)) : nullptr;
        if (!d_big) return soft_oom(c, "hipMalloc(histogram)");
        rc = zero_cursors(c);
        if (rc == KH_OK && hipMemsetAsync(d_dense, 0, kh::HIST_DENSE * sizeof(u64), c->stream) != hipSuccess)
            rc = fail(c, KH_ERR_HIP, "hipMemsetAsync(histogram)");
        u64 nbig = 0;
        if (rc == KH_OK) {
            if (c->narrow)
                hipLaunchKernelGGL(kh::ntable_hist_kernel, dim3(grid_for(c->cap)), dim3(kh::BLOCK), 0, c->stream, (const u64 *)c->ntab,
                                   c->cap, (u64)min_count, d_dense, d_big, big_cap, c->d_ctr);
            else
            hipLaunchKernelGGL(kh::table_hist_kernel, dim3(grid_for(c->cap)), dim3(kh::BLOCK), 0, c->stream, c->table,
                               c->cap, (u64)min_count, d_dense, d_big, big_cap, c->d_ctr);
            if (hipGetLastError() != hipSuccess) rc = fail(c, KH_ERR_HIP, "table_hist_kernel");
        }
        if (rc == KH_OK) rc = read_cursor(c, nullptr, &nbig);
        if (rc == KH_OK && nbig <= big_cap) {
            big.resize(nbig);
            if (hipMemcpy(dense.data(), d_dense, kh::HIST_DENSE * sizeof(u64), hipMemcpyDeviceToHost) != hipSuccess ||
                (nbig && hipMemcpy(big.data(), d_big, nbig * sizeof(u64), hipMemcpyDeviceToHost) != hipSuccess))
                rc = fail(c, KH_ERR_HIP, "hipMemcpy(histogram)");
        }
        if (rc != KH_OK) return rc;
        if (nbig <= big_cap) break;
        big_cap = nbig;
    }
    std::map<u64, u64> tail;
    for (u64 v : big) tail[v]++;
    u64 out = 0;
    for (u64 i = 0; i < kh::HIST_DENSE; ++i)
        if (dense[i]) {
            if (out < cap) { count[out] = i; freq[out] = dense[i]; }
            ++out;
        }
    for (auto &kv : tail) {
        if (out < cap) { count[out] = kv.first; freq[out] = kv.second; }
        ++out;
    }
    *n = out < cap ? out : cap;
    if (out > cap) return fail(c, KH_ERR_RANGE, "histogram arrays too small");
    return KH_OK;
}

extern "C" int kh_lookup(kh_ctx *c, const uint64_t *keys, uint64_t n, uint64_t *counts) {
    int rc = enter(c, ENTER_READ);
    if (rc != KH_OK) return rc;
    if (n == 0) return KH_OK;
    if (!keys || !counts) return fail(c, KH_ERR_BAD_ARG, "NULL argument");
    CallScratch sc(c);
    u64 *const dk = (u64 *)sc.fresh(n * sizeof(u64));
    u64 *const dc = dk ? (u64 *)sc.fresh(n * sizeof(u64)) : nullptr;
    if (!dc) return soft_oom(c, "hipMalloc(lookup)");
    hipError_t e = hipMemcpyAsync(dk, keys, n * sizeof(u64), hipMemcpyHostToDevice, c->stream);
    if (e == hipSuccess) {
        if (c->narrow)
            hipLaunchKernelGGL(kh::ntable_lookup_kernel, dim3(grid_for(n)), dim3(kh::BLOCK), 0, c->stream, (const u64 *)c->ntab,
                               c->narrow_g, dk, (u64)n, dc);
        else
        hipLaunchKernelGGL(kh::table_lookup_kernel, dim3(grid_for(n)), dim3(kh::BLOCK), 0, c->stream,
                           table_geom(c, c->table, c->cap), dk, (u64)n, dc);
        e = hipGetLastError();
    }
    if (e == hipSuccess) e = hipMemcpyAsync(counts, dc, n * sizeof(u64), hipMemcpyDeviceToHost, c->stream);
    if (e == hipSuccess) e = hipStreamSynchronize(c->stream);
    if (e != hipSuccess) return fail(c, KH_ERR_HIP, "kh_lookup", e);
    return KH_OK;
}

extern "C" int kh_host_alloc(void **out, uint64_t bytes) {
    if (!out) return KH_ERR_BAD_ARG;
    *out = nullptr;
    int ndev = 0;
    if (hipGetDeviceCount(&ndev) != hipSuccess || ndev <= 0) {
        (void)hipGetLastError();
        return KH_ERR_NO_DEVICE;
    }
    void *p = nullptr;
    if (pin_malloc(&p, bytes ? bytes : 1, hipHostMallocPortable) != hipSuccess) {
        (void)hipGetLastError();
        return KH_ERR_OOM;
    }
    *out = p;
    return KH_OK;
}

extern "C" int kh_host_free(void *p) {
    if (!p) return KH_OK;
    if (pin_free(p) != hipSuccess) {
        (void)hipGetLastError();
        return KH_ERR_BAD_ARG;
    }
    return KH_OK;
}

extern "C" int kh_host_register(void *p, uint64_t bytes) {
    if (!p || !bytes) return KH_ERR_BAD_ARG;
    int ndev = 0;
    if (hipGetDeviceCount(&ndev) != hipSuccess || ndev <= 0) {
        (void)hipGetLastError();
        return KH_ERR_NO_DEVICE;
    }
    if (hipHostRegister(p, bytes, hipHostRegisterPortable) != hipSuccess) {
        (void)hipGetLastError();
        return KH_ERR_OOM;
    }
    return KH_OK;
}

// ... 74 lines not shown
```

### krust_amd/csrc/level1.hip.h

```cpp
#pragma once
#include <utility>

#include "part_common.hip.h"
#include "window.hip.h"

namespace kh {

struct ChunkDst {
    u64 a;
    u64 b;
};
constexpr u64 CHUNK_DST_DROP = 1ull << 63;

template <bool QUAL, int MODE, bool FAST, typename PT, int KT>
__global__ __launch_bounds__(PART_NT) void part1_scatter_chunked_kernel(
    const uint8_t *__restrict__ abase, const uint8_t *__restrict__ qbase, int qaligned, u64 vbeg, u64 vend, u64 wlo,
    u64 tile0, u64 ntiles, uint32_t tiles_per_block, uint32_t k, uint32_t thr, PartGeom g, PT *__restrict__ pool,
    uint16_t *__restrict__ chunk_part, uint8_t *__restrict__ fill8, u64 *__restrict__ pool_next, u64 pool_chunks,
    Counters *ctr) {
    constexpr int ROUNDS = sizeof(PT) == 8 ? 2 : 1;
    constexpr int WPR = CHUNK / ROUNDS;
    constexpr int RTILE = PART_NT * WPR;
    __shared__ uint32_t s_code[2][PART_NT + 2];
    __shared__ uint16_t s_val[2][PART_NT + 2];
    __shared__ PT s_stage[RTILE + 2];
    __shared__ uint16_t s_pid[RTILE + 2];
    __shared__ uint32_t s_cnt[MAX_P1];
    __shared__ uint32_t s_meta[MAX_P1];
    __shared__ ChunkDst s_dst[MAX_P1];
    __shared__ uint32_t s_wsum[4];
    __shared__ uint16_t s_lofs[MAX_P1];
    __shared__ u64 s_priv_next, s_priv_end;
    const int tid = threadIdx.x;
    if (KT) k = KT;
    const uint32_t p1b = (KT == 21 && FAST) ? 10u : g.p1_bits;
    s_cnt[tid] = 0;
    if (tid == 0) {
        s_priv_next = atomicAdd(pool_next, (u64)POOL_GRAB);
        s_priv_end = s_priv_next + POOL_GRAB;
    }
    u64 cur = 0;
    uint32_t fill = CHUNK_PAY;
    bool have_chunk = false;
    const u64 tb = tile0 + (u64)blockIdx.x * tiles_per_block;
    u64 te = tb + tiles_per_block;
    if (te > tile0 + ntiles) te = tile0 + ntiles;
    int buf = 0;
    uint32_t lost = 0;
    __syncthreads();
    {
        const RawChunk raw0 = load_raw<QUAL>(abase, qbase, qaligned, chunk_pos<PART_NT>(tb, tid), vbeg, tb < te ? vend : 0);
        stage_encode<QUAL, PART_NT>(s_code, s_val, 0, true, tid, raw0, abase, qbase, qaligned, tb, vbeg, vend, thr);
    }
    for (u64 t = tb; t < te; ++t, buf ^= 1) {
        __syncthreads();
        const RawChunk raw = load_raw<QUAL>(abase, qbase, qaligned, chunk_pos<PART_NT>(t + 1, tid), vbeg, t + 1 < te ? vend : 0);
        const WinCtx w = stage_collect<PART_NT>(s_code, s_val, buf, tid, t);
        Roller roll;
        roll.init(w, k, wlo);
#pragma unroll
        for (int h = 0; h < ROUNDS; ++h) {
            PT pay[WPR];
            uint32_t tag[WPR];
#pragma unroll
            for (int j = 0; j < WPR; ++j) {
                u64 key;
#if KH_ABL & 8
                key = (u64)roll.code * (2 * j + 1) + tid;
                const bool ok = true;
#else
                const bool ok = roll.next(h * WPR + j, key);
#endif
                uint32_t p1 = 0;
                if (!QUAL || ok) {
                    if (sizeof(PT) == 8) {
                        const u64 H = kh_table_hash<MODE>(key, k) << g.shard_shift;
                        pay[j] = (PT)(H << g.p1_bits);
                        p1 = p1_of_hash(H, g);
                    } else if (FAST) {
                        uint32_t pw;
#if KH_ABL & 1
                        p1 = (uint32_t)key & 1023u;
                        pw = (uint32_t)(key >> 10);
#else
                        hash_p1_pay32<MODE>(k, p1b, key, p1, pw);
#endif
                        pay[j] = (PT)pw;
                    } else {
                        const u64 H = part_hash<MODE>(g, key);
                        pay[j] = (PT)Pay<uint32_t>::make(key, H, g);
                        p1 = p1_of_hash(H, g);
                    }
                }
                tag[j] = ok ? (p1 << 16) : 0xFFFFFFFFu;
            }
#pragma unroll
            for (int j = 0; j < WPR; ++j)
#if KH_ABL & 16
                tag[j] &= 0xFFFF0000u;
#else
                if (tag[j] != 0xFFFFFFFFu) tag[j] |= atomicAdd(&s_cnt[tag[j] >> 16], 1u);
#endif
            __syncthreads();
            block_exclusive_scan_1024(s_cnt, s_lofs, s_wsum, tid);
            uint32_t rs[WPR];
#pragma unroll
            for (int j = 0; j < WPR; ++j) rs[j] = s_lofs[(tag[j] >> 16) & (MAX_P1 - 1)];
#pragma unroll
            for (int j = 0; j < WPR; ++j) {
                const uint32_t slot = tag[j] != 0xFFFFFFFFu ? rs[j] + (tag[j] & 0xFFFFu) : (uint32_t)RTILE;
                s_stage[slot] = pay[j];
                s_pid[slot] = (uint16_t)(tag[j] >> 16);
            }
            {
                const uint32_t c = s_cnt[tid], lo = s_lofs[tid];
                const uint32_t space = CHUNK_PAY - fill;
                ChunkDst d;
                d.a = cur * CHUNK_PAY + fill - lo;
                d.b = 0;
                if (c > space) {
                    const uint32_t r = c - space;
                    const uint32_t nnew = (r + CHUNK_PAY - 1) / CHUNK_PAY;
                    u64 first = atomicAdd(&s_priv_next, (u64)nnew);
                    if (first + nnew > s_priv_end) first = atomicAdd(pool_next, (u64)nnew);
                    if (first + nnew > pool_chunks) {
                        lost += r;
                        first = 0;
                        d.b = CHUNK_DST_DROP;
                    } else {
                        for (uint32_t q = 0; q < nnew; ++q) chunk_part[first + q] = (uint16_t)tid;
                        d.b = first * CHUNK_PAY - space - lo;
                        cur = first + nnew - 1;
                        fill = r - (nnew - 1) * CHUNK_PAY;
                        have_chunk = true;
                    }
                } else {
                    fill += c;
                }
                s_dst[tid] = d;
                s_meta[tid] = lo | (space << 16);
            }
            const uint32_t total = (uint32_t)s_lofs[MAX_P1 - 1] + s_cnt[MAX_P1 - 1];
            __syncthreads();
            s_cnt[tid] = 0;
            if (tid == 0 && s_priv_next + POOL_LOW > s_priv_end) {
                s_priv_next = atomicAdd(pool_next, (u64)POOL_GRAB);
                s_priv_end = s_priv_next + POOL_GRAB;
            }
            if (h == 0)
                stage_encode<QUAL, PART_NT>(s_code, s_val, buf ^ 1, false, tid, raw, abase, qbase, qaligned, t + 1, vbeg, vend, thr);
#if !(KH_ABL & 4)
#pragma unroll 2
            for (uint32_t i = tid; i < total; i += PART_NT) {
                const uint32_t p = s_pid[i];
                const uint32_t meta = s_meta[p];
                const ChunkDst d = s_dst[p];
                const uint32_t e = i - (meta & 0xFFFFu);
#if KH_ABL & 2
                if (s_stage[i] == 0x12345678u && e == 77 && d.a == 5) pool[0] = 1;
#else
                if (e < (meta >> 16)) pool[d.a + i] = s_stage[i];
                else if (d.b != CHUNK_DST_DROP) pool[d.b + i] = s_stage[i];
#endif
            }
#endif
            if (h + 1 < ROUNDS) __syncthreads();
        }
    }
    if (have_chunk) fill8[cur] = (uint8_t)(fill - 1);
    const u64 l = wave_sum((u64)lost);
    if (lane_id() == 0 && l) atomicAdd(&ctr->failed, l);
}

constexpr uint32_t P1B_CAP = 32;
constexpr uint32_t P1B_WORDS = MAX_P1 * P1B_CAP;

__device__ __forceinline__ uint32_t rev2_complement(uint32_t x) {
    const uint32_t y = __builtin_bitreverse32(~x);
    return ((y >> 1) & 0x55555555u) | ((y & 0x55555555u) << 1);
}

typedef __attribute__((address_space(3))) uint32_t lds_u32;
#ifndef KH_L1_SWIZZLE
#define KH_L1_SWIZZLE 1
#endif
constexpr uint32_t L1_ROT_MASK = KH_L1_SWIZZLE ? 0x70u : 0u;
constexpr uint32_t K21_CNT_OFF = 0;
constexpr uint32_t K21_BIN_OFF = (MAX_P1 + PART_NT) * 4;
constexpr uint32_t K21_TRASH_OFF = K21_BIN_OFF + P1B_WORDS * 4;
constexpr uint32_t K21_WASTE0 = 0x10000u;
__device__ __forceinline__ uint32_t l1_bin_offset(uint32_t p) { return (p << 7) | ((p << 4) & L1_ROT_MASK); }
__device__ __forceinline__ uint32_t l1_word(uint32_t p, uint32_t w) { return w ^ (((p << 4) & L1_ROT_MASK) >> 2); }
__device__ __forceinline__ uint32_t l1_word64(uint32_t p, uint32_t w) { return w ^ (((p << 4) & L1_ROT_MASK) >> 3); }
__device__ __forceinline__ uint32_t l1_unit(uint32_t p, uint32_t u) { return u ^ (((p << 4) & L1_ROT_MASK) >> 4); }

template <bool QUAL, int MODE, bool FAST, int KW>
__global__ __launch_bounds__(PART_NT) void part1_bins_kernel(
    const uint8_t *__restrict__ abase, const uint8_t *__restrict__ qbase, int qaligned, u64 vbeg, u64 vend, u64 wlo,
    u64 tile0, u64 ntiles, uint32_t tiles_per_block, uint32_t k_rt, uint32_t thr, PartGeom g, uint32_t *__restrict__ pool,
    uint16_t *__restrict__ chunk_part, uint8_t *__restrict__ fill8, u64 *__restrict__ pool_next, u64 pool_chunks,
    Counters *ctr) {
    constexpr bool ASM = KW != 0;
    const uint32_t k = ASM ? (uint32_t)KW : k_rt, p1b = ASM ? 10u : g.p1_bits;
    constexpr int HALF = CHUNK / 2;
    constexpr uint32_t SEG = 16;
    __shared__ __attribute__((aligned(16))) uint32_t s_mem[(K21_TRASH_OFF + 16) / 4];
    __shared__ uint32_t s_code[2][PART_NT + 2];
    __shared__ uint16_t s_val[2][PART_NT + 2];
    __shared__ uint32_t s_flag;
    __shared__ u64 s_priv_next, s_priv_end;
    uint32_t *const s_cnt = s_mem + K21_CNT_OFF / 4;
    uint32_t *const s_bin = s_mem + K21_BIN_OFF / 4;
    __attribute__((address_space(3))) char *const lds = (__attribute__((address_space(3))) char *)s_mem;
    const int tid = threadIdx.x;
    s_cnt[tid] = 0;
    s_cnt[MAX_P1 + tid] = K21_WASTE0;
    if (tid == 0) {
        s_flag = 0;
        s_priv_next = atomicAdd(pool_next, (u64)POOL_GRAB);
        s_priv_end = s_priv_next + POOL_GRAB;
    }
    u64 cur = 0;
    uint32_t fill = CHUNK_PAY;
    uint32_t res = 0;
    bool have_chunk = false;
    const u64 tb = tile0 + (u64)blockIdx.x * tiles_per_block;
    u64 te = tb + tiles_per_block;
    if (te > tile0 + ntiles) te = tile0 + ntiles;
    int buf = 0;
    uint32_t lost = 0;
    const uint32_t waste = K21_CNT_OFF + 4u * (MAX_P1 + (uint32_t)tid);
    uint32_t *const bin = s_bin + (uint32_t)tid * P1B_CAP;
    __syncthreads();
    auto take_chunk = [&](u64 &first) -> bool {
        first = atomicAdd(&s_priv_next, 1ull);
        if (first + 1 > s_priv_end) first = atomicAdd(pool_next, 1ull);
        if (first + 1 > pool_chunks) return false;
        chunk_part[first] = (uint16_t)tid;
        return true;
    };
    auto flush = [&](uint32_t c) -> uint32_t {
        const uint32_t nseg = c / SEG;
        const uint32_t bseg = min(nseg, P1B_CAP / SEG);
        const uint32_t r = c % SEG;
        uint32_t nout = nseg;
        u64 dst[P1B_CAP / SEG];
        const uint32_t space = (CHUNK_PAY - fill) / SEG;
        u64 ib = 0;
        uint32_t ntaken = 0;
        u64 run_a = cur * CHUNK_PAY + fill, run_b = 0;
        if (nseg > space) {
            const uint32_t need = nseg - space;
            const uint32_t nnew = (need * SEG + CHUNK_PAY - 1) / CHUNK_PAY;
            u64 first = 0;
            bool ok = true;
            if (nnew == 1) ok = take_chunk(first);
            else {
                first = atomicAdd(pool_next, (u64)nnew);
                ok = first + nnew <= pool_chunks;
                if (ok) for (uint32_t q = 0; q < nnew; ++q) chunk_part[first + q] = (uint16_t)tid;
            }
            if (!ok) {
                lost += need * SEG;
                nout = space;
            } else {
                ib = first;
                ntaken = nnew;
                run_b = first * CHUNK_PAY - (u64)space * SEG;
                cur = first + nnew - 1;
                fill = need * SEG - (nnew - 1) * CHUNK_PAY;
                have_chunk = true;
            }
        } else {
            fill += nseg * SEG;
        }
        (void)ib; (void)ntaken;
#pragma unroll
        for (uint32_t sg = 0; sg < P1B_CAP / SEG; ++sg) dst[sg] = (sg < space ? run_a : run_b) + (u64)sg * SEG;
        const uint32_t nb = min(bseg, nout);
        uint4 *const bin4 = reinterpret_cast<uint4 *>(bin);
#pragma unroll
        for (uint32_t sg = 0; sg < P1B_CAP / SEG; ++sg)
            if (sg < nb) {
                uint4 *d = reinterpret_cast<uint4 *>(pool + dst[sg]);
                const uint4 x0 = bin4[l1_unit(tid, 4 * sg)], x1 = bin4[l1_unit(tid, 4 * sg + 1)], x2 = bin4[l1_unit(tid, 4 * sg + 2)],
                            x3 = bin4[l1_unit(tid, 4 * sg + 3)];
                d[0] = x0; d[1] = x1; d[2] = x2; d[3] = x3;
            }
        if (c <= P1B_CAP) {
            if (bseg) {
                const uint32_t nu = (r + 3u) / 4u;
                for (uint32_t i = 0; i < nu; ++i) bin4[l1_unit(tid, i)] = bin4[l1_unit(tid, 4 * bseg + i)];
            }
            s_cnt[tid] = r * 4u;
        } else {
            bin[l1_word(tid, 16)] = (uint32_t)run_a;
            bin[l1_word(tid, 17)] = (uint32_t)(run_a >> 32);
            bin[l1_word(tid, 18)] = (uint32_t)run_b;
            bin[l1_word(tid, 19)] = (uint32_t)(run_b >> 32);
            bin[l1_word(tid, 20)] = space * SEG;
            bin[l1_word(tid, 21)] = nout * SEG;
            bin[l1_word(tid, 22)] = nseg * SEG;
            s_cnt[tid] = (r - (c - P1B_CAP)) * 4u;
        }
        s_cnt[MAX_P1 + tid] = K21_WASTE0;
        return r;
    };
    {
        const RawChunk raw0 = load_raw<QUAL>(abase, qbase, qaligned, chunk_pos<PART_NT>(tb, tid), vbeg, tb < te ? vend : 0);
        stage_encode<QUAL, PART_NT>(s_code, s_val, 0, true, tid, raw0, abase, qbase, qaligned, tb, vbeg, vend, thr);
    }
    for (u64 t = tb; t < te; ++t, buf ^= 1) {
        __syncthreads();
        const RawChunk raw = load_raw<QUAL>(abase, qbase, qaligned, chunk_pos<PART_NT>(t + 1, tid), vbeg, t + 1 < te ? vend : 0);
        const WinCtx w = stage_collect<PART_NT>(s_code, s_val, buf, tid, t);
        const uint32_t good = window_good(w, k, wlo);
        const uint32_t w0 = (uint32_t)w.lo64, w1 = (uint32_t)(w.lo64 >> 32), w2 = w.hi;
        const uint32_t c0 = ASM ? rev2_complement(w2) : 0u, c1 = ASM ? rev2_complement(w1) : 0u, c2 = ASM ? rev2_complement(w0) : 0u;
        Roller roll;
        if (!ASM) roll.init(w, k, wlo);
        auto window = [&](int j, uint32_t &pay, uint32_t &cnta, uint32_t &binb) {
            u64 key;
            const bool ok = roll.next(j, key);
            uint32_t p1 = 0;
            pay = 0;
            if (!QUAL || ok) {
                if (FAST) {
                    hash_p1_pay32<MODE>(k, p1b, key, p1, pay);
                } else {
                    const u64 H = part_hash<MODE>(g, key);
                    pay = Pay<uint32_t>::make(key, H, g);
                    p1 = p1_of_hash(H, g);
                }
            }
            cnta = ok ? K21_CNT_OFF + 4u * p1 : waste;
            binb = l1_bin_offset(p1);
        };
#define KH_W21(J)                                                                                            \
    {                                                                                                        \
        uint32_t cnta;                                                                                       \
        if constexpr (ASM) {                                                                                 \
            uint32_t flo, fhi, rlo, rhi;                                                                     \
            win_fields<KW ? KW : 21, J>(w0, w1, w2, c0, c1, c2, flo, fhi, rlo, rhi);                         \
            win_hash32<KW ? KW : 21, J>(flo, fhi, rlo, rhi, good, waste, L1_ROT_MASK, pay[(J) % HALF], cnta, binb[(J) % HALF]); \
        } else window(J, pay[(J) % HALF], cnta, binb[(J) % HALF]);                                           \
        rk[(J) % HALF] = __hip_atomic_fetch_add((lds_u32 *)(lds + cnta), 4u, __ATOMIC_RELAXED, __HIP_MEMORY_SCOPE_WORKGROUP); \
    }
#pragma unroll
        for (int h = 0; h < 2; ++h) {
            uint32_t omask = 0;
            {
                uint32_t pay[HALF], binb[HALF], rk[HALF];
                if (h == 0) { KH_W21(0) KH_W21(1) KH_W21(2) KH_W21(3) KH_W21(4) KH_W21(5) KH_W21(6) KH_W21(7) }
                else { KH_W21(8) KH_W21(9) KH_W21(10) KH_W21(11) KH_W21(12) KH_W21(13) KH_W21(14) KH_W21(15) }
                uint32_t racc = 0;
#pragma unroll
                for (int j = 0; j < HALF; ++j) {
                    const uint32_t r4 = rk[j];
                    *(lds_u32 *)(lds + K21_BIN_OFF + (r4 < 4u * P1B_CAP ? (binb[j] ^ r4) : K21_TRASH_OFF - K21_BIN_OFF)) = pay[j];
                    racc |= r4;
                }
                if (racc & (K21_WASTE0 - 4u * P1B_CAP)) {
                    s_flag = 1u;
#pragma unroll
                    for (int j = 0; j < HALF; ++j)
                        if (rk[j] >= 4u * P1B_CAP && rk[j] < K21_WASTE0) omask |= 1u << j;
                }
            }
            if (h == 1 && tid == 0 && s_priv_next + 2 * POOL_LOW > s_priv_end) {
                s_priv_next = atomicAdd(pool_next, (u64)POOL_GRAB);
                s_priv_end = s_priv_next + POOL_GRAB;
            }
            __syncthreads();
            const bool slow = s_flag != 0u;
            if (h == 0)
                stage_encode<QUAL, PART_NT>(s_code, s_val, buf ^ 1, false, tid, raw, abase, qbase, qaligned, t + 1, vbeg, vend, thr);
            res = flush(s_cnt[tid] >> 2);
            if (slow) {
                __syncthreads();
                if (omask) {
                    Roller again;
                    again.init(w, k, wlo);
#pragma unroll
                    for (int j = 0; j < CHUNK; ++j) {
                        u64 key;
                        again.next(j, key);
                        if (j / HALF == h && ((omask >> (j % HALF)) & 1u)) {
                            uint32_t p, pv;
                            if (FAST) {
                                hash_p1_pay32<MODE>(k, p1b, key, p, pv);
                            } else {
                                const u64 H = part_hash<MODE>(g, key);
                                pv = Pay<uint32_t>::make(key, H, g);
                                p = p1_of_hash(H, g);
                            }
                            uint32_t *const pbin = s_bin + p * P1B_CAP;
                            const int32_t r2 = (int32_t)atomicAdd(&s_cnt[p], 4u) >> 2;
                            if (r2 >= 0) {
                                pbin[l1_word(p, (uint32_t)r2)] = pv;
                            } else {
                                const u64 ra = ((u64)pbin[l1_word(p, 17)] << 32) | pbin[l1_word(p, 16)];
                                const u64 rb = ((u64)pbin[l1_word(p, 19)] << 32) | pbin[l1_word(p, 18)];
                                const uint32_t split = pbin[l1_word(p, 20)], lim = pbin[l1_word(p, 21)];
                                const uint32_t e = pbin[l1_word(p, 22)] + (uint32_t)r2;
                                if (e < lim) pool[(e < split ? ra : rb) + e] = pv;
                            }
                        }
                    }
                }
                if (tid == 0) s_flag = 0u;
            }
            if (h == 0) __syncthreads();
        }
#undef KH_W21
    }
    __syncthreads();
    res = s_cnt[tid] >> 2;
    if (res) {
        bool room = true;
        if (fill + res > CHUNK_PAY) {
            u64 first;
            room = take_chunk(first);
            if (room) {
                cur = first;
                fill = 0;
                have_chunk = true;
            } else {
                lost += res;
            }
        }
        if (room) {
            for (uint32_t i = 0; i < res; ++i) pool[cur * CHUNK_PAY + fill + i] = bin[l1_word(tid, i)];
            fill += res;
        }
    }
    if (have_chunk) fill8[cur] = (uint8_t)(fill - 1);
    const u64 l = wave_sum((u64)lost);
    if (lane_id() == 0 && l) atomicAdd(&ctr->failed, l);
}

constexpr uint32_t P1B64_CAP = 16;
constexpr uint32_t P1B64_SEG = 8;
constexpr uint32_t K64_BIN_OFF = (MAX_P1 + PART_NT) * 4;
constexpr uint32_t K64_TRASH_OFF = K64_BIN_OFF + MAX_P1 * P1B64_CAP * 8;

template <int... Is, typename F>
__device__ __forceinline__ void static_for_seq(std::integer_sequence<int, Is...>, F &&f) {
    (f(std::integral_constant<int, Is>{}), ...);
}
template <int N, typename F>
__device__ __forceinline__ void static_for(F &&f) {
    static_for_seq(std::make_integer_sequence<int, N>{}, f);
}

template <bool QUAL, int MODE, int KW, int FW>
__global__ __launch_bounds__(PART_NT) void part1_bins64_kernel(
    const uint8_t *__restrict__ abase, const uint8_t *__restrict__ qbase, int qaligned, u64 vbeg, u64 vend, u64 wlo,
    u64 tile0, u64 ntiles, uint32_t tiles_per_block, uint32_t k_rt, uint32_t thr, PartGeom g, u64 *__restrict__ pool,
    uint16_t *__restrict__ chunk_part, uint8_t *__restrict__ fill8, u64 *__restrict__ pool_next, u64 pool_chunks,
    Counters *ctr) {
    constexpr bool ASM = KW != 0;
    const uint32_t k = ASM ? (uint32_t)KW : k_rt;
    constexpr uint32_t SEG = P1B64_SEG, CAP = P1B64_CAP;
    constexpr int NFLUSH = CHUNK / FW;
    __shared__ __attribute__((aligned(16))) uint32_t s_mem[(K64_TRASH_OFF + 16) / 4];
    __shared__ uint32_t s_code[2][PART_NT + 2];
    __shared__ uint16_t s_val[2][PART_NT + 2];
    __shared__ uint32_t s_flag;
    __shared__ u64 s_priv_next, s_priv_end;
    __shared__ uint32_t s_live[QUAL ? 2 : 1][QUAL ? PART_NT : 1];
    __shared__ uint32_t s_nlive[2];
    uint32_t *const s_cnt = s_mem;
    u64 *const s_bin = reinterpret_cast<u64 *>(s_mem + K64_BIN_OFF / 4);
    __attribute__((address_space(3))) char *const lds = (__attribute__((address_space(3))) char *)s_mem;
    typedef __attribute__((address_space(3))) u64 lds_u64;
    const int tid = threadIdx.x;
    s_cnt[tid] = 0;
    s_cnt[MAX_P1 + tid] = K21_WASTE0;
    if (tid == 0) {
        s_flag = 0;
        s_nlive[0] = s_nlive[1] = 0;
        s_priv_next = atomicAdd(pool_next, (u64)POOL_GRAB);
        s_priv_end = s_priv_next + POOL_GRAB;
    }
    u64 cur = 0;
    uint32_t fill = CHUNK_PAY;
    bool have_chunk = false;
    const u64 tb = tile0 + (u64)blockIdx.x * tiles_per_block;
    u64 te = tb + tiles_per_block;
    if (te > tile0 + ntiles) te = tile0 + ntiles;
    int buf = 0;
    uint32_t lost = 0;
    const uint32_t waste = 4u * (MAX_P1 + (uint32_t)tid);
    u64 *const bin = s_bin + (uint32_t)tid * CAP;
    __syncthreads();
    auto take_chunk = [&](u64 &first) -> bool {
        first = atomicAdd(&s_priv_next, 1ull);
        if (first + 1 > s_priv_end) first = atomicAdd(pool_next, 1ull);
        if (first + 1 > pool_chunks) return false;
        chunk_part[first] = (uint16_t)tid;
        return true;
    };
    auto flush = [&](uint32_t c) {
        const uint32_t nseg = c / SEG;
        const uint32_t bseg = min(nseg, CAP / SEG);
        const uint32_t r = c % SEG;
        uint32_t nout = nseg;
        const uint32_t space = (CHUNK_PAY - fill) / SEG;
        u64 run_a = cur * CHUNK_PAY + fill, run_b = 0;
        if (nseg > space) {
            const uint32_t need = nseg - space;
            const uint32_t nnew = (need * SEG + CHUNK_PAY - 1) / CHUNK_PAY;
            u64 first = 0;
            bool ok = true;
            if (nnew == 1) ok = take_chunk(first);
            else {
                first = atomicAdd(pool_next, (u64)nnew);
                ok = first + nnew <= pool_chunks;
                if (ok) for (uint32_t q = 0; q < nnew; ++q) chunk_part[first + q] = (uint16_t)tid;
            }
            if (!ok) {
                lost += need * SEG;
                nout = space;
            } else {
                run_b = first * CHUNK_PAY - (u64)space * SEG;
                cur = first + nnew - 1;
                fill = need * SEG - (nnew - 1) * CHUNK_PAY;
                have_chunk = true;
            }
        } else {
            fill += nseg * SEG;
        }
        const uint32_t nb = min(bseg, nout);
        uint4 *const bin4 = reinterpret_cast<uint4 *>(bin);
#pragma unroll
        for (uint32_t sg = 0; sg < CAP / SEG; ++sg)
            if (sg < nb) {
                uint4 *d = reinterpret_cast<uint4 *>(pool + (sg < space ? run_a : run_b) + (u64)sg * SEG);
                const uint4 x0 = bin4[l1_unit(tid, 4 * sg)], x1 = bin4[l1_unit(tid, 4 * sg + 1)], x2 = bin4[l1_unit(tid, 4 * sg + 2)],
                            x3 = bin4[l1_unit(tid, 4 * sg + 3)];
                d[0] = x0; d[1] = x1; d[2] = x2; d[3] = x3;
            }
        if (c <= CAP) {
            if (bseg) {
                const uint32_t nu = (r + 1u) / 2u;
                for (uint32_t i = 0; i < nu; ++i) bin4[l1_unit(tid, i)] = bin4[l1_unit(tid, 4 * bseg + i)];
            }
            s_cnt[tid] = r * 8u;
        } else {
            bin[l1_word64(tid, 8)] = run_a;
            bin[l1_word64(tid, 9)] = run_b;
            bin[l1_word64(tid, 10)] = (u64)(space * SEG) | ((u64)(nout * SEG) << 32);
            bin[l1_word64(tid, 11)] = (u64)(nseg * SEG);
            s_cnt[tid] = (r - (c - CAP)) * 8u;
        }
        s_cnt[MAX_P1 + tid] = K21_WASTE0;
    };
    auto p1_pay_of = [&](u64 key, u64 &pay) -> uint32_t {
        const u64 H = kh_table_hash<MODE>(key, k) << g.shard_shift;
        pay = H << g.p1_bits;
        return p1_of_hash(H, g);
    };
    {
        const RawChunk raw0 = load_raw<QUAL>(abase, qbase, qaligned, chunk_pos<PART_NT>(tb, tid), vbeg, tb < te ? vend : 0);
        stage_encode<QUAL, PART_NT>(s_code, s_val, 0, true, tid, raw0, abase, qbase, qaligned, tb, vbeg, vend, thr);
    }
#ifndef KH_L1_LIVE_LIST
#define KH_L1_LIVE_LIST 1
#endif
    constexpr bool LIVE = QUAL && KH_L1_LIVE_LIST != 0;
    auto build_list = [&](int cbuf, u64 tt, int lb) {
        WinCtx wn;
        wn.hi = s_code[cbuf][tid];
        wn.lo64 = ((u64)s_code[cbuf][tid + 1] << 32) | s_code[cbuf][tid + 2];
        wn.V = ((u64)s_val[cbuf][tid] << 32) | ((u64)s_val[cbuf][tid + 1] << 16) | (u64)s_val[cbuf][tid + 2];
        wn.p0 = (u64)chunk_pos<PART_NT>(tt, tid);
        const uint32_t gd = window_good(wn, k, wlo);
        const bool live = gd != 0u;
        const u64 m = kh_ballot(live);
        uint32_t lbase = 0;
        if (m) {
            if ((int)lane_id() == __builtin_ctzll(m)) lbase = atomicAdd(&s_nlive[lb], (uint32_t)__builtin_popcountll(m));
            lbase = (uint32_t)__shfl((int)lbase, __builtin_ctzll(m), 64);
        }
        if (live) s_live[lb][lbase + mbcnt(m)] = (uint32_t)tid | (gd << 16);
    };
    if constexpr (LIVE) {
        __syncthreads();
        build_list(0, tb, 0);
    }
    for (u64 t = tb; t < te; ++t, buf ^= 1) {
        __syncthreads();
        const RawChunk raw = load_raw<QUAL>(abase, qbase, qaligned, chunk_pos<PART_NT>(t + 1, tid), vbeg, t + 1 < te ? vend : 0);
        WinCtx w = stage_collect<PART_NT>(s_code, s_val, buf, tid, t);
        uint32_t good = LIVE ? 0u : window_good(w, k, wlo);
        bool wave_busy = true;
        const int lcur = (int)((t - tb) & 1);
        if constexpr (LIVE) {
            const uint32_t nlive = s_nlive[lcur];
            if (tid == 0) s_nlive[lcur ^ 1] = 0;
#ifndef KH_L1_WAVE_ORDER
#define KH_L1_WAVE_ORDER 0
#endif
            const uint32_t wv = (uint32_t)tid >> 6, seg = KH_L1_WAVE_ORDER ? ((wv & 3u) << 2) | (wv >> 2) : wv;
            const uint32_t li = (seg << 6) | ((uint32_t)tid & 63u);
            wave_busy = (seg << 6) < nlive;
            const uint32_t item = li < nlive ? s_live[lcur][li] : 0u;
            const uint32_t c = item & 0xFFFFu;
            good = item >> 16;
            w.hi = s_code[buf][c];
            w.lo64 = ((u64)s_code[buf][c + 1] << 32) | s_code[buf][c + 2];
            w.V = ((u64)s_val[buf][c] << 32) | ((u64)s_val[buf][c + 1] << 16) | (u64)s_val[buf][c + 2];
            w.p0 = (u64)chunk_pos<PART_NT>(t, (int)c);
        }
        const uint32_t w0 = (uint32_t)w.lo64, w1 = (uint32_t)(w.lo64 >> 32), w2 = w.hi;
        const uint32_t c0 = ASM ? rev2_complement(w2) : 0u, c1 = ASM ? rev2_complement(w1) : 0u, c2 = ASM ? rev2_complement(w0) : 0u;
        Roller roll;
        if (!ASM) {
            roll.init(w, k, wlo);
            if constexpr (QUAL) roll.good = good;
        }
        static_for<NFLUSH>([&](auto hc) {
            constexpr int h = decltype(hc)::value;
            uint32_t omask = 0;
            if (wave_busy) {
                uint32_t klo[FW], khi[FW], binb[FW], rk[FW];
                static_for<FW>([&](auto jc) {
                    constexpr int j = decltype(jc)::value, J = h * FW + j;
                    uint32_t cnta;
#ifndef KH_L1_WAVE_SKIP
#define KH_L1_WAVE_SKIP 0
#endif
                    if constexpr (ASM) {
                        if (KH_L1_WAVE_SKIP && QUAL && !kh_any(((good >> (15 - J)) & 1u) != 0u)) {
                            klo[j] = khi[j] = 0u;
                            cnta = waste;
                            binb[j] = 0u;
                        } else {
                            uint32_t flo, fhi, rlo, rhi;
                            win_fields<KW ? KW : 31, J>(w0, w1, w2, c0, c1, c2, flo, fhi, rlo, rhi);
                            win_hash64<KW ? KW : 31, J>(flo, fhi, rlo, rhi, good, waste, L1_ROT_MASK, klo[j], khi[j], cnta, binb[j]);
                        }
                    } else {
                        u64 key, pv = 0;
                        const bool ok = roll.next(J, key);
                        uint32_t p = 0;
                        if (!QUAL || ok) p = p1_pay_of(key, pv);
                        klo[j] = (uint32_t)pv;
                        khi[j] = (uint32_t)(pv >> 32);
                        cnta = ok ? 4u * p : waste;
                        binb[j] = l1_bin_offset(p);
                    }
                    rk[j] = __hip_atomic_fetch_add((lds_u32 *)(lds + cnta), 8u, __ATOMIC_RELAXED, __HIP_MEMORY_SCOPE_WORKGROUP);
                });
                uint32_t racc = 0;
#pragma unroll
                for (int j = 0; j < FW; ++j) {
                    const uint32_t r8 = rk[j];
                    *(lds_u64 *)(lds + (r8 < 8u * CAP ? K64_BIN_OFF + (binb[j] ^ r8) : K64_TRASH_OFF)) = ((u64)khi[j] << 32) | klo[j];
                    racc |= r8;
                }
                if (racc & (K21_WASTE0 - 8u * CAP)) {
                    s_flag = 1u;
#pragma unroll
                    for (int j = 0; j < FW; ++j)
                        if (rk[j] >= 8u * CAP && rk[j] < K21_WASTE0) omask |= 1u << j;
                }
            }
            if (h == NFLUSH - 1 && tid == 0 && s_priv_next + 2 * POOL_LOW > s_priv_end) {
                s_priv_next = atomicAdd(pool_next, (u64)POOL_GRAB);
                s_priv_end = s_priv_next + POOL_GRAB;
            }
            __syncthreads();
            const bool slow = s_flag != 0u;
            if (h == 0)
                stage_encode<QUAL, PART_NT>(s_code, s_val, buf ^ 1, false, tid, raw, abase, qbase, qaligned, t + 1, vbeg, vend, thr);
            flush(s_cnt[tid] >> 3);
            if (slow) {
                __syncthreads();
                if (omask) {
                    Roller again;
                    again.init(w, k, wlo);
#pragma unroll
                    for (int j = 0; j < CHUNK; ++j) {
                        u64 key;
                        again.next(j, key);
                        if (j / FW == h && ((omask >> (j % FW)) & 1u)) {
                            u64 pv;
                            const uint32_t p = p1_pay_of(key, pv);
                            u64 *const pbin = s_bin + p * CAP;
                            const int32_t r2 = (int32_t)atomicAdd(&s_cnt[p], 8u) >> 3;
                            if (r2 >= 0) {
                                pbin[l1_word64(p, (uint32_t)r2)] = pv;
                            } else {
                                const u64 ra = pbin[l1_word64(p, 8)], rb = pbin[l1_word64(p, 9)];
                                const u64 d10 = pbin[l1_word64(p, 10)];
                                const uint32_t split = (uint32_t)d10, lim = (uint32_t)(d10 >> 32);
                                const uint32_t e = (uint32_t)pbin[l1_word64(p, 11)] + (uint32_t)r2;
                                if (e < lim) pool[(e < split ? ra : rb) + e] = pv;
                            }
                        }
                    }
                }
                if (tid == 0) s_flag = 0u;
            }
            if (h + 1 < NFLUSH) __syncthreads();
            if constexpr (LIVE && h == 0 && NFLUSH > 1) build_list(buf ^ 1, t + 1, lcur ^ 1);
        });
        if constexpr (LIVE && NFLUSH == 1) {
            __syncthreads();
            build_list(buf ^ 1, t + 1, lcur ^ 1);
        }
    }
    __syncthreads();
    const uint32_t res = s_cnt[tid] >> 3;
    if (res) {
        bool room = true;
        if (fill + res > CHUNK_PAY) {
            u64 first;
            room = take_chunk(first);
            if (room) {
                cur = first;
                fill = 0;
                have_chunk = true;
            } else {
                lost += res;
            }
        }
        if (room) {
            for (uint32_t i = 0; i < res; ++i) pool[cur * CHUNK_PAY + fill + i] = bin[l1_word64(tid, i)];
            fill += res;
        }
    }
    if (have_chunk) fill8[cur] = (uint8_t)(fill - 1);
    const u64 l = wave_sum((u64)lost);
    if (lane_id() == 0 && l) atomicAdd(&ctr->failed, l);
}

}
```

### krust_amd/csrc/level1_32.hip

```cpp
#define KH_HELPERS_ONLY 1
#include "level1_api.h"
#include "level1.hip.h"

namespace kh {

namespace {
#define KH_L1_ARGS l.abase, l.qbase, l.qaligned, l.vbeg, l.vend, l.wlo, l.tile0, l.ntiles, l.tiles_per_block, l.k, l.thr, l.g, \
                   (uint32_t *)l.pool, l.chunk_part, l.fill8, l.pool_next, l.pool_chunks, l.ctr
template <int KW>
void launch_written(const L1Launch &l) {
    constexpr int MODE = (KW >= 16 && KW <= 24) ? KH_MUL_24 : KH_MUL_32;
    if (l.use_qual) hipLaunchKernelGGL((part1_bins_kernel<true, MODE, true, KW>), dim3(l.grid), dim3(PART_NT), 0, l.stream, KH_L1_ARGS);
    else hipLaunchKernelGGL((part1_bins_kernel<false, MODE, true, KW>), dim3(l.grid), dim3(PART_NT), 0, l.stream, KH_L1_ARGS);
}
template <int MODE, bool FAST>
void launch_cpp(const L1Launch &l) {
    if (l.use_qual) hipLaunchKernelGGL((part1_bins_kernel<true, MODE, FAST, 0>), dim3(l.grid), dim3(PART_NT), 0, l.stream, KH_L1_ARGS);
    else hipLaunchKernelGGL((part1_bins_kernel<false, MODE, FAST, 0>), dim3(l.grid), dim3(PART_NT), 0, l.stream, KH_L1_ARGS);
}
#if KH_TESTING
template <int MODE, bool FAST>
void launch_legacy(const L1Launch &l) {
    if (l.use_qual) hipLaunchKernelGGL((part1_scatter_chunked_kernel<true, MODE, FAST, uint32_t, 0>), dim3(l.grid), dim3(PART_NT), 0, l.stream, KH_L1_ARGS);
    else hipLaunchKernelGGL((part1_scatter_chunked_kernel<false, MODE, FAST, uint32_t, 0>), dim3(l.grid), dim3(PART_NT), 0, l.stream, KH_L1_ARGS);
}
#endif
}

void launch_level1_32(const L1Launch &l, const char **kernel) {
    const bool m24 = kh_k_uses_mul24(l.k);
    const bool fast = p1_fast_ok(l.g);
#if KH_TESTING
    if (l.legacy) {
        if (kernel) *kernel = "part1_scatter_chunked_kernel";
        if (m24 && fast) launch_legacy<KH_MUL_24, true>(l);
        else if (m24) launch_legacy<KH_MUL_24, false>(l);
        else if (fast) launch_legacy<KH_MUL_32, true>(l);
        else launch_legacy<KH_MUL_32, false>(l);
        return;
    }
#endif
    if (kernel) *kernel = "part1_bins_kernel";
    if (!l.generic_k && fast && l.g.p1_bits == 10 && l.k >= 11 && l.k <= 21) {
        switch (l.k) {
        case 11: launch_written<11>(l); return;
        case 12: launch_written<12>(l); return;
        case 13: launch_written<13>(l); return;
        case 14: launch_written<14>(l); return;
        case 15: launch_written<15>(l); return;
        case 16: launch_written<16>(l); return;
        case 17: launch_written<17>(l); return;
        case 18: launch_written<18>(l); return;
        case 19: launch_written<19>(l); return;
        case 20: launch_written<20>(l); return;
        default: launch_written<21>(l); return;
        }
    }
    if (m24 && fast) launch_cpp<KH_MUL_24, true>(l);
    else if (m24) launch_cpp<KH_MUL_24, false>(l);
    else if (fast) launch_cpp<KH_MUL_32, true>(l);
    else launch_cpp<KH_MUL_32, false>(l);
}

}
```

### krust_amd/csrc/level1_64.hip

```cpp
#define KH_HELPERS_ONLY 1
#include "level1_api.h"
#include "level1.hip.h"

namespace kh {

namespace {
#define KH_L1_ARGS l.abase, l.qbase, l.qaligned, l.vbeg, l.vend, l.wlo, l.tile0, l.ntiles, l.tiles_per_block, l.k, l.thr, l.g, \
                   (u64 *)l.pool, l.chunk_part, l.fill8, l.pool_next, l.pool_chunks, l.ctr
#ifndef KH_L1_FW_LOW
#define KH_L1_FW_LOW 8
#endif
#ifndef KH_L1_FW_HIGH
#define KH_L1_FW_HIGH 4
#endif
template <int MODE, int KW>
void launch_bins(const L1Launch &l) {
    const bool low = l.survive < 0.55;
    if (l.use_qual && low) hipLaunchKernelGGL((part1_bins64_kernel<true, MODE, KW, KH_L1_FW_LOW>), dim3(l.grid), dim3(PART_NT), 0, l.stream, KH_L1_ARGS);
    else if (l.use_qual) hipLaunchKernelGGL((part1_bins64_kernel<true, MODE, KW, KH_L1_FW_HIGH>), dim3(l.grid), dim3(PART_NT), 0, l.stream, KH_L1_ARGS);
    else if (low) hipLaunchKernelGGL((part1_bins64_kernel<false, MODE, KW, KH_L1_FW_LOW>), dim3(l.grid), dim3(PART_NT), 0, l.stream, KH_L1_ARGS);
    else hipLaunchKernelGGL((part1_bins64_kernel<false, MODE, KW, KH_L1_FW_HIGH>), dim3(l.grid), dim3(PART_NT), 0, l.stream, KH_L1_ARGS);
}
#if KH_TESTING
template <int MODE>
void launch_legacy(const L1Launch &l) {
    if (l.use_qual) hipLaunchKernelGGL((part1_scatter_chunked_kernel<true, MODE, false, u64, 0>), dim3(l.grid), dim3(PART_NT), 0, l.stream, KH_L1_ARGS);
    else hipLaunchKernelGGL((part1_scatter_chunked_kernel<false, MODE, false, u64, 0>), dim3(l.grid), dim3(PART_NT), 0, l.stream, KH_L1_ARGS);
}
#endif
}

void launch_level1_64(const L1Launch &l, const char **kernel) {
    const bool m24 = kh_k_uses_mul24(l.k);
#if KH_TESTING
    if (l.legacy) {
        if (kernel) *kernel = "part1_scatter_chunked_kernel";
        if (m24) launch_legacy<KH_MUL_24>(l);
        else launch_legacy<KH_MUL_32>(l);
        return;
    }
#endif
    if (kernel) *kernel = "part1_bins64_kernel";
    if (!l.generic_k && l.g.shard_shift == 0 && l.g.p1_bits == 10 && l.k >= 22) {
        switch (l.k) {
        case 22: launch_bins<KH_MUL_24, 22>(l); return;
        case 23: launch_bins<KH_MUL_24, 23>(l); return;
        case 24: launch_bins<KH_MUL_24, 24>(l); return;
        case 25: launch_bins<KH_MUL_32, 25>(l); return;
        case 26: launch_bins<KH_MUL_32, 26>(l); return;
        case 27: launch_bins<KH_MUL_32, 27>(l); return;
        case 28: launch_bins<KH_MUL_32, 28>(l); return;
        case 29: launch_bins<KH_MUL_32, 29>(l); return;
        case 30: launch_bins<KH_MUL_32, 30>(l); return;
        case 31: launch_bins<KH_MUL_32, 31>(l); return;
        default: launch_bins<KH_MUL_32, 32>(l); return;
        }
    }
    if (m24) launch_bins<KH_MUL_24, 0>(l);
    else launch_bins<KH_MUL_32, 0>(l);
}

}
```

### krust_amd/csrc/level1_api.h

```cpp
#pragma once
#include <hip/hip_runtime.h>
#include <stdint.h>

#include "part_common.hip.h"

#ifndef KH_TESTING
#define KH_TESTING 0
#endif

namespace kh {

struct L1Launch {
    hipStream_t stream;
    unsigned grid;
    const uint8_t *abase, *qbase;
    int qaligned;
    bool use_qual;
    u64 vbeg, vend, wlo, tile0, ntiles;
    uint32_t tiles_per_block, k, thr;
    PartGeom g;
    void *pool;
    uint16_t *chunk_part;
    uint8_t *fill8;
    u64 *pool_next;
    u64 pool_chunks;
    Counters *ctr;
    double survive;
    bool generic_k;
    bool legacy;
};

void launch_level1_32(const L1Launch &l, const char **kernel);
void launch_level1_64(const L1Launch &l, const char **kernel);

}
```

### krust_amd/csrc/partition.hip.h

```cpp
#pragma once
#include <type_traits>
#include "arena_bits.h"
#include "part_common.hip.h"

namespace kh {

KH_GLOBAL __launch_bounds__(1024) void chunk_hist_kernel(const uint16_t *__restrict__ chunk_part, const u64 *__restrict__ pool_next,
                                                          u64 pool_chunks, uint32_t *__restrict__ pcount,
                                                          const uint8_t *__restrict__ fill8, u64 *__restrict__ ptotal) {
    __shared__ uint32_t s_h[MAX_P1];
    __shared__ uint32_t s_f[MAX_P1];
    const int tid = threadIdx.x;
    s_h[tid] = 0;
    s_f[tid] = 0;
    __syncthreads();
    u64 n = *pool_next;
    if (n > pool_chunks) n = pool_chunks;
    const u64 stride = (u64)gridDim.x * 1024;
    for (u64 i = (u64)blockIdx.x * 1024 + tid; i < n; i += stride) {
        const uint16_t p = chunk_part[i];
        if (p != PART_NONE) {
            atomicAdd(&s_h[p], 1u);
            if (ptotal) atomicAdd(&s_f[p], (uint32_t)fill8[i] + 1u);
        }
    }
    __syncthreads();
    if (s_h[tid]) atomicAdd(&pcount[tid], s_h[tid]);
    if (ptotal && s_f[tid]) atomicAdd(&ptotal[tid], (u64)s_f[tid]);
}

KH_GLOBAL __launch_bounds__(1024) void chunk_list_kernel(const uint16_t *__restrict__ chunk_part, const u64 *__restrict__ pool_next,
                                                          u64 pool_chunks, uint32_t *__restrict__ cursors,
                                                          uint32_t *__restrict__ plist) {
    __shared__ uint32_t s_h[MAX_P1];
    __shared__ uint32_t s_base[MAX_P1];
    const int tid = threadIdx.x;
    u64 n = *pool_next;
    if (n > pool_chunks) n = pool_chunks;
    const u64 lo = (u64)blockIdx.x * 16384;
    if (lo >= n) return;
    s_h[tid] = 0;
    __syncthreads();
    uint32_t tag[16];
#pragma unroll
    for (int j = 0; j < 16; ++j) {
        const u64 i = lo + (u64)j * 1024 + tid;
        tag[j] = 0xFFFFFFFFu;
        if (i < n) {
            const uint16_t p = chunk_part[i];
            if (p != PART_NONE) tag[j] = ((uint32_t)p << 16) | atomicAdd(&s_h[p], 1u);
        }
    }
    __syncthreads();
    s_base[tid] = s_h[tid] ? atomicAdd(&cursors[tid], s_h[tid]) : 0u;
    __syncthreads();
#pragma unroll
    for (int j = 0; j < 16; ++j)
        if (tag[j] != 0xFFFFFFFFu) plist[s_base[tag[j] >> 16] + (tag[j] & 0xFFFFu)] = (uint32_t)(lo + (u64)j * 1024 + tid);
}

template <typename PT>
__global__ __launch_bounds__(BLOCK) void distinct_sample_kernel(ChunkSrc cs, const u64 *__restrict__ pstart, uint32_t p_first, uint32_t np,
                                                                uint32_t sub_bits, u64 *__restrict__ set, u64 set_mask, u64 *__restrict__ out) {
    const u64 c0 = pstart[p_first], c1 = pstart[p_first + np];
    uint32_t nd = 0, nf = 0;
    u64 seen = 0;
    uint32_t p = p_first;
    for (u64 ci = c0 + blockIdx.x; ci < c1; ci += gridDim.x) {
        while (pstart[p + 1] <= ci) ++p;
        const uint32_t chunk = cs.plist[ci];
        const uint32_t fill = (uint32_t)cs.fill8[chunk] + 1u;
        if (threadIdx.x >= fill) continue;
        const PT pay = reinterpret_cast<const PT *>(cs.pay)[(u64)chunk * CHUNK_PAY + threadIdx.x];
        if (sizeof(PT) == 8 && (u64)pay == KH_EMPTY_KEY) continue;
        if (sub_bits) {
            const uint32_t sel = sizeof(PT) == 4 ? (uint32_t)pay >> (32 - sub_bits) : (uint32_t)(kh_mix64((u64)pay) >> 40) >> (24 - sub_bits);
            if (sel) continue;
        }
        ++seen;
        const u64 v = sizeof(PT) == 4 ? ((u64)(p - p_first) << 32) | (u64)pay : ((u64)pay | (u64)(p - p_first));
        u64 h = kh_mix64(v) & set_mask;
        uint32_t probes = 0;
        for (; probes < 128; ++probes, h = (h + 1) & set_mask) {
            u64 cur = set[h];
            if (cur == ~0ull) {
                cur = atomicCAS((unsigned long long *)&set[h], ~0ull, (unsigned long long)v);
                if (cur == ~0ull) {
                    ++nd;
                    break;
                }
            }
            if (cur == v) break;
        }
        nf += probes == 128;
    }
    const u64 d = wave_sum((u64)nd), f = wave_sum((u64)nf);
    seen = wave_sum(seen);
    if (lane_id() == 0) {
        if (d) atomicAdd(&out[0], d);
        if (seen) atomicAdd(&out[1], seen);
        if (f) atomicAdd(&out[2], f);
    }
}

__device__ __forceinline__ u64 block_scan_1024(u64 v, u64 *s_scan, int tid, u64 *total) {
    s_scan[tid] = v;
    __syncthreads();
    for (int o = 1; o < 1024; o <<= 1) {
        const u64 add = tid >= o ? s_scan[tid - o] : 0ull;
        __syncthreads();
        s_scan[tid] += add;
        __syncthreads();
    }
    const u64 incl = s_scan[tid];
    if (total) *total = s_scan[1023];
    __syncthreads();
    return incl - v;
}

KH_GLOBAL __launch_bounds__(1024) void part2_plan_chunked_kernel(const u64 *__restrict__ pstart, PartGeom g,
                                                                  Part2Block *__restrict__ blocks, u64 max_blocks,
                                                                  u64 *__restrict__ moff, uint32_t *__restrict__ nch,
                                                                  u64 *__restrict__ info, uint32_t *__restrict__ cursors,
                                                                  uint32_t force_wide, const uint8_t *__restrict__ only) {
    __shared__ u64 s_bbase[MAX_P1 + 1];
    __shared__ u64 s_scan[1024];
    const int tid = threadIdx.x;
    const int P1 = 1 << g.p1_bits;
    if (tid < P1 && !only) cursors[tid] = (uint32_t)pstart[tid];
    auto nchunks_of = [&](int p) -> u64 { return (only && !only[p]) ? 0ull : pstart[p + 1] - pstart[p]; };
    const u64 my_chunks = tid < P1 ? nchunks_of(tid) : 0ull;
    const u64 my_blocks = (my_chunks + CPB - 1) / CPB;
    u64 b = 0;
    const u64 my_base = block_scan_1024(my_blocks, s_scan, tid, &b);
    if (tid < P1) s_bbase[tid] = my_base;
    const int wide = __syncthreads_or((force_wide || my_chunks * CHUNK_PAY + my_blocks * 1024ull * 64ull >= (1ull << 32)) ? 1 : 0);
    if (tid == 0) {
        s_bbase[P1] = b;
        info[0] = b;
        info[1] = b * g.b2;
        info[2] = 0;
        info[3] = wide ? 1 : 0;
    }
    __syncthreads();
    if (tid < P1) {
        const u64 lo = pstart[tid], hi = lo + nchunks_of(tid);
        const u64 b0 = s_bbase[tid];
        const uint32_t n = (uint32_t)(s_bbase[tid + 1] - b0);
        moff[tid] = b0 * g.b2;
        nch[tid] = n;
        for (uint32_t c = 0; c < n; ++c) {
            if (b0 + c >= max_blocks) break;
            Part2Block pb;
            pb.lo = lo + (u64)c * CPB;
            pb.hi = pb.lo + CPB < hi ? pb.lo + CPB : hi;
            pb.mbase = b0 * g.b2 + c;
            pb.mstride = n;
            pb.p1 = (uint32_t)tid;
            blocks[b0 + c] = pb;
        }
    }
}


constexpr int SCAN_NT = 256;
constexpr int SCAN_PER = 16;
constexpr int SCAN_CHUNK = SCAN_NT * SCAN_PER;

KH_GLOBAL __launch_bounds__(SCAN_NT) void scan_partials_kernel(const uint32_t *__restrict__ in, u64 n, u64 *__restrict__ partial) {
    __shared__ u64 s_w[SCAN_NT / 64];
    const u64 base = (u64)blockIdx.x * SCAN_CHUNK;
    u64 s = 0;
#pragma unroll
    for (int i = 0; i < SCAN_PER; ++i) {
        const u64 idx = base + (u64)i * SCAN_NT + threadIdx.x;
        if (idx < n) s += in[idx];
    }
    s = wave_sum(s);
    if ((threadIdx.x & 63) == 0) s_w[threadIdx.x >> 6] = s;
    __syncthreads();
    if (threadIdx.x == 0) partial[blockIdx.x] = s_w[0] + s_w[1] + s_w[2] + s_w[3];
}

KH_GLOBAL __launch_bounds__(1024) void scan_spine_kernel(u64 *__restrict__ partial, u64 nb) {
    __shared__ u64 s_w[16];
    __shared__ u64 s_carry;
    const int tid = threadIdx.x;
    if (tid == 0) s_carry = 0;
    __syncthreads();
    for (u64 base = 0; base < nb; base += 1024) {
        const u64 idx = base + tid;
        const u64 v = idx < nb ? partial[idx] : 0;
        u64 incl = v;
#pragma unroll
        for (int off = 1; off < 64; off <<= 1) {
            const u64 n = __shfl_up(incl, off, 64);
            if ((tid & 63) >= off) incl += n;
        }
        if ((tid & 63) == 63) s_w[tid >> 6] = incl;
        __syncthreads();
        u64 wbase = s_carry;
        for (int w = 0; w < (tid >> 6); ++w) wbase += s_w[w];
        if (idx < nb) partial[idx] = wbase + incl - v;
        __syncthreads();
        if (tid == 1023) s_carry = wbase + incl;
        __syncthreads();
    }
    if (tid == 0) partial[nb] = s_carry;
}

KH_GLOBAL __launch_bounds__(SCAN_NT) void scan_apply_kernel(const uint32_t *__restrict__ in, u64 n,
                                                             const u64 *__restrict__ partial, u64 *__restrict__ out) {
    __shared__ u64 s_w[SCAN_NT / 64];
    const int tid = threadIdx.x;
    const u64 first = (u64)blockIdx.x * SCAN_CHUNK + (u64)tid * SCAN_PER;
    uint32_t v[SCAN_PER];
    u64 sum = 0;
#pragma unroll
    for (int i = 0; i < SCAN_PER; ++i) {
        v[i] = (first + i < n) ? in[first + i] : 0u;
        sum += v[i];
    }
    u64 incl = sum;
#pragma unroll
    for (int off = 1; off < 64; off <<= 1) {
        const u64 nn = __shfl_up(incl, off, 64);
        if ((tid & 63) >= off) incl += nn;
    }
    if ((tid & 63) == 63) s_w[tid >> 6] = incl;
    __syncthreads();
    u64 run = partial[blockIdx.x] + incl - sum;
    for (int w = 0; w < (tid >> 6); ++w) run += s_w[w];
#pragma unroll
    for (int i = 0; i < SCAN_PER; ++i) {
        if (first + i < n) out[first + i] = run;
        run += v[i];
    }
    if (blockIdx.x == gridDim.x - 1 && tid == SCAN_NT - 1) out[n] = run;
}

template <typename PT, bool CHUNKED>
__global__ __launch_bounds__(PART_NT) void part2_count_kernel(const PT *__restrict__ pays, ChunkSrc cs,
                                                              const Part2Block *__restrict__ blocks,
                                                              const u64 *__restrict__ info, PartGeom g,
                                                              uint32_t *__restrict__ H2, uint32_t pad) {
    __shared__ uint32_t s_hist[1u << MAX_P2_BITS];
    __shared__ uint32_t s_chk[CHUNKED ? CPB : 1];
    __shared__ uint16_t s_cfill[CHUNKED ? CPB : 1];
    if ((u64)blockIdx.x >= info[0]) return;
    const Part2Block pb = blocks[blockIdx.x];
    const int tid = threadIdx.x;
    s_hist[tid] = 0;
    p2_stage_chunks<CHUNKED>(cs, pb, s_chk, s_cfill, tid, PART_NT);
    __syncthreads();
    const uint32_t n = p2_count_of<CHUNKED>(pb);
    for (uint32_t base = 0; base < n; base += 8 * PART_NT) {
        PT v[8];
        uint32_t ok = 0;
#pragma unroll
        for (int j = 0; j < 8; ++j)
            ok |= (uint32_t)p2_load<CHUNKED, PT>(pays, cs, pb, s_chk, s_cfill, base + (uint32_t)j * PART_NT + tid, n, v[j]) << j;
#pragma unroll
        for (int j = 0; j < 8; ++j)
            if (ok & (1u << j)) atomicAdd(&s_hist[Pay<PT>::p2(l2_finish(v[j], pb.p1, g), g)], 1u);
    }
    __syncthreads();
    if (pad > 1 && info[3]) pad = 1;
    if ((uint32_t)tid < g.b2) H2[pb.mbase + (u64)tid * pb.mstride] = (s_hist[tid] + pad - 1) / pad * pad;
}

#ifndef KH_PART2_NT
#define KH_PART2_NT 512
#endif
#ifndef KH_PART2_TILE
#define KH_PART2_TILE 16384
#endif
constexpr int PART2_NT = KH_PART2_NT;
constexpr int PART2_TILE = KH_PART2_TILE;
constexpr int P2_PER = PART2_TILE / PART2_NT;

template <typename PT, bool CHUNKED, int NBK>
__global__ __launch_bounds__(PART2_NT, (NBK == 512 && sizeof(PT) == 4) ? 4 : 2) void part2_scatter_kernel(
    const PT *__restrict__ pays, ChunkSrc cs, const Part2Block *__restrict__ blocks, const u64 *__restrict__ info, PartGeom g,
    const u64 *__restrict__ O2, PT *__restrict__ out, uint32_t only_if_wide) {
    constexpr int OWN = NBK / PART2_NT;
    __shared__ PT s_stage[PART2_TILE + 1];
    __shared__ uint32_t s_cnt[NBK];
    __shared__ uint16_t s_lofs[NBK];
    __shared__ u64 s_dst[NBK];
    __shared__ uint32_t s_wsum[4];
    __shared__ uint32_t s_chk[CHUNKED ? CPB : 1];
    __shared__ uint16_t s_cfill[CHUNKED ? CPB : 1];
    if ((u64)blockIdx.x >= info[0]) return;
    if (only_if_wide && !info[3]) return;
    const Part2Block pb = blocks[blockIdx.x];
    const int tid = threadIdx.x;
    const int P2 = (int)g.b2;
    p2_stage_chunks<CHUNKED>(cs, pb, s_chk, s_cfill, tid, PART2_NT);
    u64 gcur[OWN];
#pragma unroll
    for (int q = 0; q < OWN; ++q) {
        const int b = tid + q * PART2_NT;
        s_cnt[b] = 0;
        gcur[q] = b < P2 ? O2[pb.mbase + (u64)b * pb.mstride] : 0;
    }
    __syncthreads();
    const uint32_t n = p2_count_of<CHUNKED>(pb);
    PT pay[P2_PER];
    uint32_t have = 0;
#pragma unroll
    for (int j = 0; j < P2_PER; ++j)
        have |= (uint32_t)p2_load<CHUNKED, PT>(pays, cs, pb, s_chk, s_cfill, (uint32_t)j * PART2_NT + tid, n, pay[j]) << j;
    for (uint32_t base = 0; base < n; base += PART2_TILE) {
        uint32_t tag[P2_PER];
#pragma unroll
        for (int j = 0; j < P2_PER; ++j) pay[j] = l2_finish(pay[j], pb.p1, g);
#pragma unroll
        for (int j = 0; j < P2_PER; ++j) tag[j] = (have & (1u << j)) ? (Pay<PT>::p2(pay[j], g) << 16) : 0xFFFFFFFFu;
#pragma unroll
        for (int j = 0; j < P2_PER; ++j)
            if (tag[j] != 0xFFFFFFFFu) tag[j] |= atomicAdd(&s_cnt[tag[j] >> 16], 1u);
        __syncthreads();
        block_exclusive_scan_n<NBK>(s_cnt, s_lofs, s_wsum, tid);
        {
            uint32_t rs[P2_PER];
#pragma unroll
            for (int j = 0; j < P2_PER; ++j) rs[j] = s_lofs[(tag[j] >> 16) & (NBK - 1)];
#pragma unroll
            for (int j = 0; j < P2_PER; ++j)
                s_stage[tag[j] != 0xFFFFFFFFu ? rs[j] + (tag[j] & 0xFFFFu) : (uint32_t)PART2_TILE] = pay[j];
        }
#pragma unroll
        for (int q = 0; q < OWN; ++q) {
            const int b = tid + q * PART2_NT;
            s_dst[b] = gcur[q] - s_lofs[b];
            gcur[q] += s_cnt[b];
        }
        const uint32_t total = (uint32_t)s_lofs[NBK - 1] + s_cnt[NBK - 1];
        __syncthreads();
#pragma unroll
        for (int q = 0; q < OWN; ++q) s_cnt[tid + q * PART2_NT] = 0;
        have = 0;
#pragma unroll
        for (int j = 0; j < P2_PER; ++j)
            have |= (uint32_t)p2_load<CHUNKED, PT>(pays, cs, pb, s_chk, s_cfill, base + PART2_TILE + (uint32_t)j * PART2_NT + tid, n, pay[j]) << j;
#if KH_ABL2 & 28
        for (uint32_t i = tid; i < (uint32_t)PART2_TILE; i += PART2_NT) {
            constexpr uint32_t LP = ((KH_ABL2 & 4) ? 128 : (KH_ABL2 & 8) ? 64 : 32) / sizeof(PT);
            const uint32_t b = (i / LP) % (uint32_t)P2;
            out[((s_dst[b] + s_lofs[b]) & ~(u64)(LP - 1)) + (i % LP)] = s_stage[i];
        }
#else
#pragma unroll 2
        for (uint32_t i = tid; i < total; i += PART2_NT) {
            const PT v = s_stage[i];
#if KH_ABL2 & 1
            if (v == (PT)0x12345678u && s_dst[Pay<PT>::p2(v, g)] == 5) out[0] = v;
#elif KH_ABL2 & 2
            out[(u64)blockIdx.x * (CPB * CHUNK_PAY) + base + i + (s_dst[Pay<PT>::p2(v, g)] & 0)] = v;
#else
            out[s_dst[Pay<PT>::p2(v, g)] + i] = v;
#endif
        }
#endif
        __syncthreads();
    }
}

constexpr int P2L_NBK = 512;
constexpr int P2L_NT = 1024;
template <typename PT>
struct P2L {
    static constexpr int UNIT = 64 / (int)sizeof(PT);
    static constexpr int TILE = sizeof(PT) == 4 ? PART2_TILE : PART2_TILE / 2;
    static constexpr int PER = TILE / P2L_NT;
};

template <typename PT>
__device__ __forceinline__ PT p2_sentinel(uint32_t digit, uint32_t b2) {
    if (sizeof(PT) == 8) return (PT)KH_EMPTY_KEY;
    return (PT)kh_xlo(digit ? digit - 1u : 1u, b2);
}

template <typename PT, bool CHUNKED>
__global__ __launch_bounds__(P2L_NT) void part2_scatter_lines_kernel(const PT *__restrict__ pays, ChunkSrc cs,
                                                                     const Part2Block *__restrict__ blocks,
                                                                     const u64 *__restrict__ info, PartGeom g,
                                                                     const u64 *__restrict__ O2, PT *__restrict__ out) {
    constexpr int NBK = P2L_NBK, UNIT = P2L<PT>::UNIT, NT = P2L_NT, PER = P2L<PT>::PER, TILE = P2L<PT>::TILE;
    constexpr int MAXU = TILE / UNIT + NBK;
    constexpr uint32_t RES0 = TILE + 1;
    constexpr uint32_t RES_SZ = NBK * UNIT;
    __shared__ PT s_buf[TILE + 1 + 2 * NBK * UNIT];
    __shared__ uint32_t s_cnt[NBK];
    __shared__ uint2 s_ofs[NBK];
    __shared__ uint2 s_unit[MAXU];
    __shared__ uint32_t s_wsum[NBK / 64];
    __shared__ uint32_t s_nu;
    __shared__ uint32_t s_chk[CHUNKED ? CPB : 1];
    __shared__ uint16_t s_cfill[CHUNKED ? CPB : 1];
    if ((u64)blockIdx.x >= info[0] || info[3]) return;
    const Part2Block pb = blocks[blockIdx.x];
    const int tid = threadIdx.x;
    const int P2 = (int)g.b2;
    p2_stage_chunks<CHUNKED>(cs, pb, s_chk, s_cfill, tid, NT);
    const u64 gbase = O2[pb.mbase];
    uint32_t gdone = (tid < P2) ? (uint32_t)(O2[pb.mbase + (u64)tid * pb.mstride] - gbase) : 0u;
    uint32_t res = 0;
    uint32_t par = 0;
    if (tid < NBK) s_cnt[tid] = 0;
    __syncthreads();
    const uint32_t n = p2_count_of<CHUNKED>(pb);
    const uint32_t nchk = CHUNKED ? (uint32_t)(pb.hi - pb.lo) : 0u;
    const uint32_t woff = (uint32_t)tid & (CHUNK_PAY - 1);
    auto load_batch = [&](uint32_t first, PT (&pay)[PER], uint32_t &have) {
        have = 0;
        uint32_t mychunk = 0, myfill = 0;
        if (CHUNKED) {
            const uint32_t myci = (first >> 8) + ((uint32_t)tid & (PER - 1)) * (NT / CHUNK_PAY) + ((uint32_t)tid >> 8);
            const uint32_t mycc = myci < nchk ? myci : nchk - 1;
            mychunk = s_chk[mycc];
            myfill = myci < nchk ? (uint32_t)s_cfill[mycc] : 0u;
        }
#pragma unroll
        for (int j = 0; j < PER; ++j) {
            if (CHUNKED) {
                const uint32_t chunk = __builtin_amdgcn_readlane(mychunk, j);
                const uint32_t fillc = __builtin_amdgcn_readlane(myfill, j);
                const bool ok = woff < fillc;
                pay[j] = reinterpret_cast<const PT *>(cs.pay)[(u64)chunk * CHUNK_PAY + (ok ? woff : 0u)];
                have |= (uint32_t)ok << j;
            } else {
// ... 1789 lines not shown
```

Measured before the change: 208.8 billion k-mers/s.

## Fuse partition histogram into level-1 scatter and merge scan into chunk list

The level-1 scatter kernels now publish per-partition chunk counts and totals through atomics, which removes the separate chunk histogram kernel. The chunk list kernel computes the prefix scan itself and uses its own cursor array, so the device_scan call and the early plan launch are dropped. The sampling kernel now reads chunk_part directly in tiles, so it no longer depends on pstart and runs before the list kernel. Host readback goes to pinned memory and waits on an event, which lets the list kernel queue ahead of the host sync. In exchange, every scatter thread issues extra global atomics and each list block repeats the 1024-element scan.

```diff
diff --git a/krust_amd/csrc/batch.hip b/krust_amd/csrc/batch.hip
--- a/krust_amd/csrc/batch.hip
+++ b/krust_amd/csrc/batch.hip
@@ -285,7 +285,7 @@
         if ((rc = fixed(&c->moff, (u64)kh::MAX_P1 + 1, "hipMalloc(moff)")) != KH_OK) return rc;
         if ((rc = fixed(&c->nch, (u64)kh::MAX_P1 + 1, "hipMalloc(nch)")) != KH_OK) return rc;
         if ((rc = fixed(&c->info, 8, "hipMalloc(info)")) != KH_OK) return rc;
-        if ((rc = fixed(&c->pcount, (u64)kh::MAX_P1, "hipMalloc(pcount)")) != KH_OK) return rc;
+        if ((rc = fixed(&c->pcount, 2 * (u64)kh::MAX_P1, "hipMalloc(pcount)")) != KH_OK) return rc;
         if ((rc = fixed(&c->pstart, (u64)kh::MAX_P1 + 1, "hipMalloc(pstart)")) != KH_OK) return rc;
         if ((rc = fixed(&c->pool_next, 1, "hipMalloc(pool_next)")) != KH_OK) return rc;
         if ((rc = fixed(&c->ptotal, (u64)kh::MAX_P1, "hipMalloc(ptotal)")) != KH_OK) return rc;
@@ -339,7 +339,8 @@
             StageTimer t(c, ST_MISC);
             HIP_TRY(c, hipMemsetAsync(c->chunk_part, 0xFF, pool_chunks * sizeof(uint16_t), c->stream));
             HIP_TRY(c, hipMemsetAsync(c->fill8, 0xFF, pool_chunks, c->stream));
-            HIP_TRY(c, hipMemsetAsync(c->pcount, 0, kh::MAX_P1 * sizeof(uint32_t), c->stream));
+            HIP_TRY(c, hipMemsetAsync(c->pcount, 0, 2 * kh::MAX_P1 * sizeof(uint32_t), c->stream));
+            HIP_TRY(c, hipMemsetAsync(c->ptotal, 0, kh::MAX_P1 * sizeof(u64), c->stream));
             HIP_TRY(c, hipMemsetAsync(c->pool_next, 0, sizeof(u64), c->stream));
         }
         {
@@ -366,6 +367,8 @@
             l1.pool_next = c->pool_next;
             l1.pool_chunks = pool_chunks;
             l1.ctr = c->d_ctr;
+            l1.pcount = c->pcount;
+            l1.ptotal = c->ptotal;
             l1.survive = ra.survive;
             l1.generic_k = c->knobs.generic_k;
             l1.legacy = c->knobs.p1_legacy;
@@ -378,31 +381,37 @@
             return sync_counters(c);
         }
 #endif
+        const bool host_reads = estimated || size_from_sample;
+        static_assert(H_MID_WORDS >= kh::MAX_P1 + 4 && sizeof(Counters) % sizeof(u64) == 0, "the pinned words behind the counters");
+        u64 *const h_mid = reinterpret_cast<u64 *>(c->h_ctr + 1);
         {
             StageTimer t(c, ST_MISC);
-            HIP_TRY(c, hipMemsetAsync(c->ptotal, 0, kh::MAX_P1 * sizeof(u64), c->stream));
-            hipLaunchKernelGGL(kh::chunk_hist_kernel, dim3(1024), dim3(1024), 0, c->stream, (const uint16_t *)c->chunk_part,
-                               (const u64 *)c->pool_next, pool_chunks, c->pcount, (const uint8_t *)c->fill8, c->ptotal);
-            if ((rc = device_scan(c, c->pcount, P1, c->pstart)) != KH_OK) return rc;
-            hipLaunchKernelGGL(kh::part2_plan_chunked_kernel, dim3(1), dim3(1024), 0, c->stream, (const u64 *)c->pstart, g,
-                               c->blocks, max_blocks, c->moff, c->nch, c->info, c->pcount, force_wide, (const uint8_t *)nullptr);
-            hipLaunchKernelGGL(kh::chunk_list_kernel, dim3((unsigned)((pool_chunks + 16383) / 16384)), dim3(1024), 0, c->stream,
-                               (const uint16_t *)c->chunk_part, (const u64 *)c->pool_next, pool_chunks, c->pcount, c->plist);
             if (size_from_sample) {
                 u64 *est_out = c->info + 4;
                 HIP_TRY(c, hipMemsetAsync(est_out, 0, 3 * sizeof(u64), c->stream));
                 HIP_TRY(c, hipMemsetAsync(c->est_set, 0xFF, est_slots * sizeof(u64), c->stream));
-                hipLaunchKernelGGL(kh::distinct_sample_kernel<PT>, dim3(1024), dim3(kh::BLOCK), 0, c->stream, cs, (const u64 *)c->pstart,
+                hipLaunchKernelGGL(kh::distinct_sample_kernel<PT>, dim3((unsigned)std::min<u64>((u64)grid_cap(), (pool_chunks + kh::SAMPLE_TILE - 1) / kh::SAMPLE_TILE)),
+                                   dim3(kh::BLOCK), 0, c->stream, (const uint16_t *)c->chunk_part, (const u64 *)c->pool_next, pool_chunks, cs,
                                    EST_P0 % (uint32_t)(P1 - est_np + 1), est_np, est_sub, c->est_set, est_slots - 1, est_out);
             }
-        }
-        if (estimated || size_from_sample) {
-            std::vector<u64> pt(kh::MAX_P1);
-            u64 lost = 0, total = 0, est[3] = {0, 0, 0};
-            HIP_TRY(c, hipMemcpyAsync(pt.data(), c->ptotal, kh::MAX_P1 * sizeof(u64), hipMemcpyDeviceToHost, c->stream));
-            HIP_TRY(c, hipMemcpyAsync(&lost, &c->d_ctr->failed, sizeof(u64), hipMemcpyDeviceToHost, c->stream));
-            if (size_from_sample) HIP_TRY(c, hipMemcpyAsync(est, c->info + 4, sizeof(est), hipMemcpyDeviceToHost, c->stream));
-            HIP_TRY(c, hipStreamSynchronize(c->stream));
+            if (host_reads) {
+                if (!c->mid_ev) HIP_TRY(c, hipEventCreateWithFlags(&c->mid_ev, hipEventDisableTiming));
+                HIP_TRY(c, hipMemcpyAsync(h_mid, c->ptotal, kh::MAX_P1 * sizeof(u64), hipMemcpyDeviceToHost, c->stream));
+                HIP_TRY(c, hipMemcpyAsync(h_mid + kh::MAX_P1, &c->d_ctr->failed, sizeof(u64), hipMemcpyDeviceToHost, c->stream));
+                if (size_from_sample) HIP_TRY(c, hipMemcpyAsync(h_mid + kh::MAX_P1 + 1, c->info + 4, 3 * sizeof(u64), hipMemcpyDeviceToHost, c->stream));
+                HIP_TRY(c, hipEventRecord(c->mid_ev, c->stream));
+            }
+            hipLaunchKernelGGL(kh::chunk_list_kernel, dim3((unsigned)((pool_chunks + kh::LIST_SLICE - 1) / kh::LIST_SLICE)), dim3(1024), 0, c->stream,
+                               (const uint16_t *)c->chunk_part, (const u64 *)c->pool_next, pool_chunks, (const uint32_t *)c->pcount, c->pcount + kh::MAX_P1,
+                               c->plist, c->pstart);
+        }
+        if (host_reads) {
+            HIP_TRY(c, hipEventSynchronize(c->mid_ev));
+            const u64 *const pt = h_mid;
+            const u64 lost = h_mid[kh::MAX_P1];
+            u64 total = 0, est[3] = {0, 0, 0};
+            if (size_from_sample)
+                for (int i = 0; i < 3; ++i) est[i] = h_mid[kh::MAX_P1 + 1 + i];
             for (u64 p = 0; p < P1; ++p) total += pt[p];
             have_total = true;
             batch_total = total;
@@ -423,7 +432,7 @@
                 if (c->hinted && newcap < c->cap) newcap = c->cap;
                 newcap = std::min<u64>(newcap, (u64)kh::MAX_P1 * kh::MAX_B2 * kh::REGION_SLOTS);
                 size_t fr = 0, tot = 0;
-                if (hipMemGetInfo(&fr, &tot) == hipSuccess) {
+                if (newcap > c->cap && hipMemGetInfo(&fr, &tot) == hipSuccess) {
                     u64 room = ((u64)fr + (c->table ? c->cap * sizeof(Slot) : 0) + (c->ntab ? c->ntab_cap * sizeof(u64) : 0)) / 3;
                     if (c->knobs.table_room_mb) room = c->knobs.table_room_mb << 20;
                     while (newcap > c->cap && newcap * sizeof(Slot) > room) {
@@ -594,9 +603,8 @@
     PT *const outB = heavy_exact ? bufB + heavy_base : bufB;
     {
         StageTimer t(c, ST_MISC);
-        if (heavy_exact || size_from_sample)
-            hipLaunchKernelGGL(kh::part2_plan_chunked_kernel, dim3(1), dim3(1024), 0, c->stream, (const u64 *)c->pstart, g,
-                               c->blocks, max_blocks, c->moff, c->nch, c->info, c->pcount, force_wide, heavy_exact ? (const uint8_t *)c->heavy : (const uint8_t *)nullptr);
+        hipLaunchKernelGGL(kh::part2_plan_chunked_kernel, dim3(1), dim3(1024), 0, c->stream, (const u64 *)c->pstart, g,
+                           c->blocks, max_blocks, c->moff, c->nch, c->info, force_wide, heavy_exact ? (const uint8_t *)c->heavy : (const uint8_t *)nullptr);
         HIP_TRY(c, hipMemsetAsync(c->H2, 0, n2 * sizeof(uint32_t), c->stream));
     }
     {
diff --git a/krust_amd/csrc/ctx.hip.h b/krust_amd/csrc/ctx.hip.h
--- a/krust_amd/csrc/ctx.hip.h
+++ b/krust_amd/csrc/ctx.hip.h
@@ -48,6 +48,7 @@
 #define KH_PART_G1 512
 #endif
 constexpr int PART_G1 = KH_PART_G1;
+constexpr u64 H_MID_WORDS = 1024 + 4;
 constexpr u64 PART_MIN_WINDOWS = 1ull << 22;
 constexpr double LOAD_PART = 0.70;
 enum { ST_DIRECT = 0, ST_P1_COUNT, ST_P1_SCATTER, ST_P2_COUNT, ST_P2_SCATTER, ST_REGION, ST_MISC, ST_GROW, ST_N, ST_TEXT = ST_N };
@@ -237,6 +238,7 @@
     uint32_t *plist = nullptr;
     u64 pool_cap = 0;
     uint32_t *pcount = nullptr;
+    hipEvent_t mid_ev = nullptr;
     u64 *pstart = nullptr;
     u64 *pool_next = nullptr;
     u64 region_cap = 0;
diff --git a/krust_amd/csrc/kmerhip.hip b/krust_amd/csrc/kmerhip.hip
--- a/krust_amd/csrc/kmerhip.hip
+++ b/krust_amd/csrc/kmerhip.hip
@@ -551,7 +551,7 @@
             c->own_stream = true;
         }
         if (dev_malloc((void **)&c->d_ctr, sizeof(Counters)) != hipSuccess) { rc = KH_ERR_OOM; break; }
-        if (pin_malloc((void **)&c->h_ctr, sizeof(Counters), hipHostMallocDefault) != hipSuccess) { rc = KH_ERR_OOM; break; }
+        if (pin_malloc((void **)&c->h_ctr, sizeof(Counters) + H_MID_WORDS * sizeof(u64), hipHostMallocDefault) != hipSuccess) { rc = KH_ERR_OOM; break; }
         if (hipMemsetAsync(c->d_ctr, 0, sizeof(Counters), c->stream) != hipSuccess) { rc = KH_ERR_HIP; break; }
         u64 cap = cfg->capacity_hint ? round_cap((double)cfg->capacity_hint / HINT_LOAD) : DEFAULT_CAP;
         if (const u64 nr = c->knobs.table_regions)
@@ -595,6 +595,7 @@
     if (c->ntab) (void)dev_free(c->ntab);
     if (c->d_ctr) (void)dev_free(c->d_ctr);
     if (c->h_ctr) (void)pin_free(c->h_ctr);
+    if (c->mid_ev) (void)hipEventDestroy(c->mid_ev);
     if (c->h_txt) (void)pin_free(c->h_txt);
     for (int i = 0; i < 2; ++i) {
         if (c->txt_acc_done[i]) (void)hipEventDestroy(c->txt_acc_done[i]);
diff --git a/krust_amd/csrc/level1.hip.h b/krust_amd/csrc/level1.hip.h
--- a/krust_amd/csrc/level1.hip.h
+++ b/krust_amd/csrc/level1.hip.h
@@ -12,12 +12,18 @@
 };
 constexpr u64 CHUNK_DST_DROP = 1ull << 63;
 
+__device__ __forceinline__ void l1_publish_counts(bool have_chunk, uint32_t ntake, uint32_t fill, uint32_t *pcount_p, u64 *ptotal_p) {
+    if (!have_chunk) return;
+    (void)__hip_atomic_fetch_add(pcount_p, ntake, __ATOMIC_RELAXED, __HIP_MEMORY_SCOPE_AGENT);
+    (void)__hip_atomic_fetch_add(ptotal_p, (u64)(ntake - 1u) * CHUNK_PAY + fill, __ATOMIC_RELAXED, __HIP_MEMORY_SCOPE_AGENT);
+}
+
 template <bool QUAL, int MODE, bool FAST, typename PT, int KT>
 __global__ __launch_bounds__(PART_NT) void part1_scatter_chunked_kernel(
     const uint8_t *__restrict__ abase, const uint8_t *__restrict__ qbase, int qaligned, u64 vbeg, u64 vend, u64 wlo,
     u64 tile0, u64 ntiles, uint32_t tiles_per_block, uint32_t k, uint32_t thr, PartGeom g, PT *__restrict__ pool,
     uint16_t *__restrict__ chunk_part, uint8_t *__restrict__ fill8, u64 *__restrict__ pool_next, u64 pool_chunks,
-    Counters *ctr) {
+    Counters *ctr, uint32_t *__restrict__ pcount, u64 *__restrict__ ptotal) {
     constexpr int ROUNDS = sizeof(PT) == 8 ? 2 : 1;
     constexpr int WPR = CHUNK / ROUNDS;
     constexpr int RTILE = PART_NT * WPR;
@@ -47,6 +53,7 @@
     if (te > tile0 + ntiles) te = tile0 + ntiles;
     int buf = 0;
     uint32_t lost = 0;
+    uint32_t ntake = 0;
     __syncthreads();
     {
         const RawChunk raw0 = load_raw<QUAL>(abase, qbase, qaligned, chunk_pos<PART_NT>(tb, tid), vbeg, tb < te ? vend : 0);
@@ -129,6 +136,7 @@
                         d.b = CHUNK_DST_DROP;
                     } else {
                         for (uint32_t q = 0; q < nnew; ++q) chunk_part[first + q] = (uint16_t)tid;
+                        ntake += nnew;
                         d.b = first * CHUNK_PAY - space - lo;
                         cur = first + nnew - 1;
                         fill = r - (nnew - 1) * CHUNK_PAY;
@@ -168,6 +176,7 @@
         }
     }
     if (have_chunk) fill8[cur] = (uint8_t)(fill - 1);
+    l1_publish_counts(have_chunk, ntake, fill, pcount + tid, ptotal + tid);
     const u64 l = wave_sum((u64)lost);
     if (lane_id() == 0 && l) atomicAdd(&ctr->failed, l);
 }
@@ -199,7 +208,7 @@
     const uint8_t *__restrict__ abase, const uint8_t *__restrict__ qbase, int qaligned, u64 vbeg, u64 vend, u64 wlo,
     u64 tile0, u64 ntiles, uint32_t tiles_per_block, uint32_t k_rt, uint32_t thr, PartGeom g, uint32_t *__restrict__ pool,
     uint16_t *__restrict__ chunk_part, uint8_t *__restrict__ fill8, u64 *__restrict__ pool_next, u64 pool_chunks,
-    Counters *ctr) {
+    Counters *ctr, uint32_t *__restrict__ pcount, u64 *__restrict__ ptotal) {
     constexpr bool ASM = KW != 0;
     const uint32_t k = ASM ? (uint32_t)KW : k_rt, p1b = ASM ? 10u : g.p1_bits;
     constexpr int HALF = CHUNK / 2;
@@ -229,6 +238,7 @@
     if (te > tile0 + ntiles) te = tile0 + ntiles;
     int buf = 0;
     uint32_t lost = 0;
+    uint32_t ntake = 0;
     const uint32_t waste = K21_CNT_OFF + 4u * (MAX_P1 + (uint32_t)tid);
     uint32_t *const bin = s_bin + (uint32_t)tid * P1B_CAP;
     __syncthreads();
@@ -237,6 +247,7 @@
         if (first + 1 > s_priv_end) first = atomicAdd(pool_next, 1ull);
         if (first + 1 > pool_chunks) return false;
         chunk_part[first] = (uint16_t)tid;
+        ++ntake;
         return true;
     };
     auto flush = [&](uint32_t c) -> uint32_t {
@@ -258,7 +269,10 @@
             else {
                 first = atomicAdd(pool_next, (u64)nnew);
                 ok = first + nnew <= pool_chunks;
-                if (ok) for (uint32_t q = 0; q < nnew; ++q) chunk_part[first + q] = (uint16_t)tid;
+                if (ok) {
+                    for (uint32_t q = 0; q < nnew; ++q) chunk_part[first + q] = (uint16_t)tid;
+                    ntake += nnew;
+                }
             }
             if (!ok) {
                 lost += need * SEG;
@@ -435,6 +449,7 @@
         }
     }
     if (have_chunk) fill8[cur] = (uint8_t)(fill - 1);
+    l1_publish_counts(have_chunk, ntake, fill, pcount + tid, ptotal + tid);
     const u64 l = wave_sum((u64)lost);
     if (lane_id() == 0 && l) atomicAdd(&ctr->failed, l);
 }
@@ -458,7 +473,7 @@
     const uint8_t *__restrict__ abase, const uint8_t *__restrict__ qbase, int qaligned, u64 vbeg, u64 vend, u64 wlo,
     u64 tile0, u64 ntiles, uint32_t tiles_per_block, uint32_t k_rt, uint32_t thr, PartGeom g, u64 *__restrict__ pool,
     uint16_t *__restrict__ chunk_part, uint8_t *__restrict__ fill8, u64 *__restrict__ pool_next, u64 pool_chunks,
-    Counters *ctr) {
+    Counters *ctr, uint32_t *__restrict__ pcount, u64 *__restrict__ ptotal) {
     constexpr bool ASM = KW != 0;
     const uint32_t k = ASM ? (uint32_t)KW : k_rt;
     constexpr uint32_t SEG = P1B64_SEG, CAP = P1B64_CAP;
@@ -491,6 +506,7 @@
     if (te > tile0 + ntiles) te = tile0 + ntiles;
     int buf = 0;
     uint32_t lost = 0;
+    uint32_t ntake = 0;
     const uint32_t waste = 4u * (MAX_P1 + (uint32_t)tid);
     u64 *const bin = s_bin + (uint32_t)tid * CAP;
     __syncthreads();
@@ -499,6 +515,7 @@
         if (first + 1 > s_priv_end) first = atomicAdd(pool_next, 1ull);
         if (first + 1 > pool_chunks) return false;
         chunk_part[first] = (uint16_t)tid;
+        ++ntake;
         return true;
     };
     auto flush = [&](uint32_t c) {
@@ -517,7 +534,10 @@
             else {
                 first = atomicAdd(pool_next, (u64)nnew);
                 ok = first + nnew <= pool_chunks;
-                if (ok) for (uint32_t q = 0; q < nnew; ++q) chunk_part[first + q] = (uint16_t)tid;
+                if (ok) {
+                    for (uint32_t q = 0; q < nnew; ++q) chunk_part[first + q] = (uint16_t)tid;
+                    ntake += nnew;
+                }
             }
             if (!ok) {
                 lost += need * SEG;
@@ -733,6 +753,7 @@
         }
     }
     if (have_chunk) fill8[cur] = (uint8_t)(fill - 1);
+    l1_publish_counts(have_chunk, ntake, fill, pcount + tid, ptotal + tid);
     const u64 l = wave_sum((u64)lost);
     if (lane_id() == 0 && l) atomicAdd(&ctr->failed, l);
 }
diff --git a/krust_amd/csrc/level1_32.hip b/krust_amd/csrc/level1_32.hip
--- a/krust_amd/csrc/level1_32.hip
+++ b/krust_amd/csrc/level1_32.hip
@@ -6,7 +6,7 @@
 
 namespace {
 #define KH_L1_ARGS l.abase, l.qbase, l.qaligned, l.vbeg, l.vend, l.wlo, l.tile0, l.ntiles, l.tiles_per_block, l.k, l.thr, l.g, \
-                   (uint32_t *)l.pool, l.chunk_part, l.fill8, l.pool_next, l.pool_chunks, l.ctr
+                   (uint32_t *)l.pool, l.chunk_part, l.fill8, l.pool_next, l.pool_chunks, l.ctr, l.pcount, l.ptotal
 template <int KW>
 void launch_written(const L1Launch &l) {
     constexpr int MODE = (KW >= 16 && KW <= 24) ? KH_MUL_24 : KH_MUL_32;
diff --git a/krust_amd/csrc/level1_64.hip b/krust_amd/csrc/level1_64.hip
--- a/krust_amd/csrc/level1_64.hip
+++ b/krust_amd/csrc/level1_64.hip
@@ -6,7 +6,7 @@
 
 namespace {
 #define KH_L1_ARGS l.abase, l.qbase, l.qaligned, l.vbeg, l.vend, l.wlo, l.tile0, l.ntiles, l.tiles_per_block, l.k, l.thr, l.g, \
-                   (u64 *)l.pool, l.chunk_part, l.fill8, l.pool_next, l.pool_chunks, l.ctr
+                   (u64 *)l.pool, l.chunk_part, l.fill8, l.pool_next, l.pool_chunks, l.ctr, l.pcount, l.ptotal
 #ifndef KH_L1_FW_LOW
 #define KH_L1_FW_LOW 8
 #endif
diff --git a/krust_amd/csrc/level1_api.h b/krust_amd/csrc/level1_api.h
--- a/krust_amd/csrc/level1_api.h
+++ b/krust_amd/csrc/level1_api.h
@@ -25,6 +25,8 @@
     u64 *pool_next;
     u64 pool_chunks;
     Counters *ctr;
+    uint32_t *pcount;
+    u64 *ptotal;
     double survive;
     bool generic_k;
     bool legacy;
diff --git a/krust_amd/csrc/partition.hip.h b/krust_amd/csrc/partition.hip.h
--- a/krust_amd/csrc/partition.hip.h
+++ b/krust_amd/csrc/partition.hip.h
@@ -4,104 +4,6 @@
 #include "part_common.hip.h"
 
 namespace kh {
-
-KH_GLOBAL __launch_bounds__(1024) void chunk_hist_kernel(const uint16_t *__restrict__ chunk_part, const u64 *__restrict__ pool_next,
-                                                          u64 pool_chunks, uint32_t *__restrict__ pcount,
-                                                          const uint8_t *__restrict__ fill8, u64 *__restrict__ ptotal) {
-    __shared__ uint32_t s_h[MAX_P1];
-    __shared__ uint32_t s_f[MAX_P1];
-    const int tid = threadIdx.x;
-    s_h[tid] = 0;
-    s_f[tid] = 0;
-    __syncthreads();
-    u64 n = *pool_next;
-    if (n > pool_chunks) n = pool_chunks;
-    const u64 stride = (u64)gridDim.x * 1024;
-    for (u64 i = (u64)blockIdx.x * 1024 + tid; i < n; i += stride) {
-        const uint16_t p = chunk_part[i];
-        if (p != PART_NONE) {
-            atomicAdd(&s_h[p], 1u);
-            if (ptotal) atomicAdd(&s_f[p], (uint32_t)fill8[i] + 1u);
-        }
-    }
-    __syncthreads();
-    if (s_h[tid]) atomicAdd(&pcount[tid], s_h[tid]);
-    if (ptotal && s_f[tid]) atomicAdd(&ptotal[tid], (u64)s_f[tid]);
-}
-
-KH_GLOBAL __launch_bounds__(1024) void chunk_list_kernel(const uint16_t *__restrict__ chunk_part, const u64 *__restrict__ pool_next,
-                                                          u64 pool_chunks, uint32_t *__restrict__ cursors,
-                                                          uint32_t *__restrict__ plist) {
-    __shared__ uint32_t s_h[MAX_P1];
-    __shared__ uint32_t s_base[MAX_P1];
-    const int tid = threadIdx.x;
-    u64 n = *pool_next;
-    if (n > pool_chunks) n = pool_chunks;
-    const u64 lo = (u64)blockIdx.x * 16384;
-    if (lo >= n) return;
-    s_h[tid] = 0;
-    __syncthreads();
-    uint32_t tag[16];
-#pragma unroll
-    for (int j = 0; j < 16; ++j) {
-        const u64 i = lo + (u64)j * 1024 + tid;
-        tag[j] = 0xFFFFFFFFu;
-        if (i < n) {
-            const uint16_t p = chunk_part[i];
-            if (p != PART_NONE) tag[j] = ((uint32_t)p << 16) | atomicAdd(&s_h[p], 1u);
-        }
-    }
-    __syncthreads();
-    s_base[tid] = s_h[tid] ? atomicAdd(&cursors[tid], s_h[tid]) : 0u;
-    __syncthreads();
-#pragma unroll
-    for (int j = 0; j < 16; ++j)
-        if (tag[j] != 0xFFFFFFFFu) plist[s_base[tag[j] >> 16] + (tag[j] & 0xFFFFu)] = (uint32_t)(lo + (u64)j * 1024 + tid);
-}
-
-template <typename PT>
-__global__ __launch_bounds__(BLOCK) void distinct_sample_kernel(ChunkSrc cs, const u64 *__restrict__ pstart, uint32_t p_first, uint32_t np,
-                                                                uint32_t sub_bits, u64 *__restrict__ set, u64 set_mask, u64 *__restrict__ out) {
-    const u64 c0 = pstart[p_first], c1 = pstart[p_first + np];
-    uint32_t nd = 0, nf = 0;
-    u64 seen = 0;
-    uint32_t p = p_first;
-    for (u64 ci = c0 + blockIdx.x; ci < c1; ci += gridDim.x) {
-        while (pstart[p + 1] <= ci) ++p;
-        const uint32_t chunk = cs.plist[ci];
-        const uint32_t fill = (uint32_t)cs.fill8[chunk] + 1u;
-        if (threadIdx.x >= fill) continue;
-        const PT pay = reinterpret_cast<const PT *>(cs.pay)[(u64)chunk * CHUNK_PAY + threadIdx.x];
-        if (sizeof(PT) == 8 && (u64)pay == KH_EMPTY_KEY) continue;
-        if (sub_bits) {
-            const uint32_t sel = sizeof(PT) == 4 ? (uint32_t)pay >> (32 - sub_bits) : (uint32_t)(kh_mix64((u64)pay) >> 40) >> (24 - sub_bits);
-            if (sel) continue;
-        }
-        ++seen;
-        const u64 v = sizeof(PT) == 4 ? ((u64)(p - p_first) << 32) | (u64)pay : ((u64)pay | (u64)(p - p_first));
-        u64 h = kh_mix64(v) & set_mask;
-        uint32_t probes = 0;
-        for (; probes < 128; ++probes, h = (h + 1) & set_mask) {
-            u64 cur = set[h];
-            if (cur == ~0ull) {
-                cur = atomicCAS((unsigned long long *)&set[h], ~0ull, (unsigned long long)v);
-                if (cur == ~0ull) {
-                    ++nd;
-                    break;
-                }
-            }
-            if (cur == v) break;
-        }
-        nf += probes == 128;
-    }
-    const u64 d = wave_sum((u64)nd), f = wave_sum((u64)nf);
-    seen = wave_sum(seen);
-    if (lane_id() == 0) {
-        if (d) atomicAdd(&out[0], d);
-        if (seen) atomicAdd(&out[1], seen);
-        if (f) atomicAdd(&out[2], f);
-    }
-}
 
 __device__ __forceinline__ u64 block_scan_1024(u64 v, u64 *s_scan, int tid, u64 *total) {
     s_scan[tid] = v;
@@ -118,16 +20,202 @@
     return incl - v;
 }
 
+#ifndef KH_LIST_SLICE
+#define KH_LIST_SLICE 131072
+#endif
+constexpr u64 LIST_SLICE = KH_LIST_SLICE;
+static_assert(LIST_SLICE % POOL_GRAB == 0 && LIST_SLICE % 8192 == 0, "whole level-1 grabs, whole sweeps of 1024 lanes x 8 ids");
+KH_GLOBAL __launch_bounds__(1024) void chunk_list_kernel(const uint16_t *__restrict__ chunk_part, const u64 *__restrict__ pool_next,
+                                                          u64 pool_chunks, const uint32_t *__restrict__ pcount,
+                                                          uint32_t *__restrict__ cursors, uint32_t *__restrict__ plist,
+                                                          u64 *__restrict__ pstart) {
+    __shared__ u64 s_scan[1024];
+    __shared__ uint32_t s_h[MAX_P1];
+    const int tid = threadIdx.x;
+    u64 n = *pool_next;
+    if (n > pool_chunks) n = pool_chunks;
+    const u64 lo = (u64)blockIdx.x * LIST_SLICE;
+    if (lo >= n && blockIdx.x != 0) return;
+    u64 total = 0;
+    const u64 base = block_scan_1024((u64)pcount[tid], s_scan, tid, &total);
+    if (blockIdx.x == 0) {
+        pstart[tid] = base;
+        if (tid == 0) pstart[MAX_P1] = total;
+    }
+    if (lo >= n) return;
+    const u64 hi = lo + LIST_SLICE < n ? lo + LIST_SLICE : n;
+    constexpr int NV = (int)(LIST_SLICE / 8192);
+    uint4 v[NV];
+#pragma unroll
+    for (int j = 0; j < NV; ++j) {
+        const u64 i = lo + ((u64)j * 1024 + tid) * 8;
+        if (i + 8 <= hi) {
+            v[j] = *reinterpret_cast<const uint4 *>(chunk_part + i);
+        } else {
+            uint32_t w[4];
+#pragma unroll
+            for (int e = 0; e < 8; e += 2) {
+                const uint32_t a = i + e < hi ? chunk_part[i + e] : PART_NONE, b = i + e + 1 < hi ? chunk_part[i + e + 1] : PART_NONE;
+                w[e >> 1] = a | (b << 16);
+            }
+            v[j] = make_uint4(w[0], w[1], w[2], w[3]);
+        }
+    }
+    auto sweep = [&](auto &&f) {
+#pragma unroll
+        for (int j = 0; j < NV; ++j) {
+            const uint32_t w[4] = {v[j].x, v[j].y, v[j].z, v[j].w};
+#pragma unroll
+            for (int e = 0; e < 8; ++e) {
+                const uint32_t p = (w[e >> 1] >> (16 * (e & 1))) & 0xFFFFu;
+                if (p != PART_NONE) f(p, lo + ((u64)j * 1024 + tid) * 8 + e);
+            }
+        }
+    };
+    s_h[tid] = 0;
+    __syncthreads();
+    sweep([&](uint32_t p, u64) { atomicAdd(&s_h[p], 1u); });
+    __syncthreads();
+    const uint32_t mine = s_h[tid];
+    if (mine) s_h[tid] = (uint32_t)base + atomicAdd(&cursors[tid], mine);
+    __syncthreads();
+    sweep([&](uint32_t p, u64 id) {
+        const uint32_t at = atomicAdd(&s_h[p], 1u);
+        if (at < pool_chunks) plist[at] = (uint32_t)id;
+    });
+}
+
+constexpr uint32_t SAMPLE_TILE = 8192;
+constexpr int SAMPLE_FLIGHT = 4;
+static_assert(SAMPLE_TILE == BLOCK * 32 && SAMPLE_TILE <= 65536, "32 ids per lane; a match is kept as a 16-bit id within the tile");
+template <typename PT>
+struct alignas(16) SampleQuad {
+    PT v[4];
+};
+template <typename PT>
+__global__ __launch_bounds__(BLOCK) void distinct_sample_kernel(const uint16_t *__restrict__ chunk_part, const u64 *__restrict__ pool_next,
+                                                                u64 pool_chunks, ChunkSrc cs, uint32_t p_first, uint32_t np, uint32_t sub_bits,
+                                                                u64 *__restrict__ set, u64 set_mask, u64 *__restrict__ out) {
+    __shared__ uint16_t s_id[SAMPLE_TILE];
+    __shared__ uint8_t s_dp[SAMPLE_TILE];
+    __shared__ uint32_t s_n;
+    const int tid = threadIdx.x;
+    const uint32_t lane = lane_id(), wave = (uint32_t)tid >> 6;
+    u64 n = *pool_next;
+    if (n > pool_chunks) n = pool_chunks;
+    uint32_t nd = 0, nf = 0;
+    u64 seen = 0;
+    auto probe4 = [&](const SampleQuad<PT> &q, uint32_t fill, uint32_t dp) {
+        u64 v[4], h[4], cur[4];
+        bool ok[4];
+#pragma unroll
+        for (uint32_t j = 0; j < 4; ++j) {
+            const PT pay = q.v[j];
+            ok[j] = lane * 4 + j < fill && !(sizeof(PT) == 8 && (u64)pay == KH_EMPTY_KEY);
+            if (sub_bits) {
+                const uint32_t sel = sizeof(PT) == 4 ? (uint32_t)pay >> (32 - sub_bits) : (uint32_t)(kh_mix64((u64)pay) >> 40) >> (24 - sub_bits);
+                ok[j] = ok[j] && sel == 0;
+            }
+            v[j] = sizeof(PT) == 4 ? ((u64)dp << 32) | (u64)pay : ((u64)pay | (u64)dp);
+            h[j] = kh_mix64(v[j]) & set_mask;
+            cur[j] = ok[j] ? set[h[j]] : 0ull;
+        }
+#pragma unroll
+        for (uint32_t j = 0; j < 4; ++j) {
+            if (!ok[j]) continue;
+            ++seen;
+            u64 c = cur[j], at = h[j];
+            uint32_t probes = 0;
+            for (; probes < 128; ++probes) {
+                if (c == ~0ull) {
+                    c = atomicCAS((unsigned long long *)&set[at], ~0ull, (unsigned long long)v[j]);
+                    if (c == ~0ull) {
+                        ++nd;
+                        break;
+                    }
+                }
+                if (c == v[j]) break;
+                at = (at + 1) & set_mask;
+                c = set[at];
+            }
+            nf += probes == 128;
+        }
+    };
+    for (u64 t0 = (u64)blockIdx.x * SAMPLE_TILE; t0 < n; t0 += (u64)gridDim.x * SAMPLE_TILE) {
+        if (tid == 0) s_n = 0;
+        __syncthreads();
+        {
+            uint4 w4[4];
+#pragma unroll
+            for (int j = 0; j < 4; ++j) {
+                const u64 i = t0 + ((u64)j * BLOCK + tid) * 8;
+                if (i + 8 <= n) {
+                    w4[j] = *reinterpret_cast<const uint4 *>(chunk_part + i);
+                } else {
+                    uint32_t w[4];
+#pragma unroll
+                    for (int e = 0; e < 8; e += 2) {
+                        const uint32_t a = i + e < n ? chunk_part[i + e] : PART_NONE, b = i + e + 1 < n ? chunk_part[i + e + 1] : PART_NONE;
+                        w[e >> 1] = a | (b << 16);
+                    }
+                    w4[j] = make_uint4(w[0], w[1], w[2], w[3]);
+                }
+            }
+#pragma unroll
+            for (int j = 0; j < 4; ++j) {
+                const uint32_t w[4] = {w4[j].x, w4[j].y, w4[j].z, w4[j].w};
+#pragma unroll
+                for (int e = 0; e < 8; ++e) {
+                    const uint32_t dp = ((w[e >> 1] >> (16 * (e & 1))) & 0xFFFFu) - p_first;
+                    if (dp < np) {
+                        const uint32_t at = atomicAdd(&s_n, 1u);
+                        s_id[at] = (uint16_t)(((uint32_t)j * BLOCK + tid) * 8 + e);
+                        s_dp[at] = (uint8_t)dp;
+                    }
+                }
+            }
+        }
+        __syncthreads();
+        const uint32_t m = s_n;
+        for (uint32_t e0 = wave; e0 < m; e0 += (BLOCK / 64) * SAMPLE_FLIGHT) {
+            SampleQuad<PT> q[SAMPLE_FLIGHT];
+            uint32_t fill[SAMPLE_FLIGHT], dp[SAMPLE_FLIGHT];
+#pragma unroll
+            for (int u = 0; u < SAMPLE_FLIGHT; ++u) {
+                const uint32_t e = e0 + (uint32_t)u * (BLOCK / 64);
+                fill[u] = 0;
+                dp[u] = 0;
+                if (e < m) {
+                    const u64 chunk = t0 + s_id[e];
+                    dp[u] = s_dp[e];
+                    fill[u] = (uint32_t)cs.fill8[chunk] + 1u;
+                    q[u] = *reinterpret_cast<const SampleQuad<PT> *>(reinterpret_cast<const PT *>(cs.pay) + chunk * CHUNK_PAY + lane * 4);
+                }
+            }
+#pragma unroll
+            for (int u = 0; u < SAMPLE_FLIGHT; ++u)
+                if (fill[u]) probe4(q[u], fill[u], dp[u]);
+        }
+        __syncthreads();
+    }
+    const u64 d = wave_sum((u64)nd), f = wave_sum((u64)nf);
+    seen = wave_sum(seen);
+    if (lane == 0) {
+        if (d) atomicAdd(&out[0], d);
+        if (seen) atomicAdd(&out[1], seen);
+        if (f) atomicAdd(&out[2], f);
+    }
+}
+
 KH_GLOBAL __launch_bounds__(1024) void part2_plan_chunked_kernel(const u64 *__restrict__ pstart, PartGeom g,
                                                                   Part2Block *__restrict__ blocks, u64 max_blocks,
                                                                   u64 *__restrict__ moff, uint32_t *__restrict__ nch,
-                                                                  u64 *__restrict__ info, uint32_t *__restrict__ cursors,
-                                                                  uint32_t force_wide, const uint8_t *__restrict__ only) {
+                                                                  u64 *__restrict__ info, uint32_t force_wide,
+                                                                  const uint8_t *__restrict__ only) {
     __shared__ u64 s_bbase[MAX_P1 + 1];
     __shared__ u64 s_scan[1024];
     const int tid = threadIdx.x;
     const int P1 = 1 << g.p1_bits;
-    if (tid < P1 && !only) cursors[tid] = (uint32_t)pstart[tid];
     auto nchunks_of = [&](int p) -> u64 { return (only && !only[p]) ? 0ull : pstart[p + 1] - pstart[p]; };
     const u64 my_chunks = tid < P1 ? nchunks_of(tid) : 0ull;
     const u64 my_blocks = (my_chunks + CPB - 1) / CPB;
```

Measured after the change: 208.2 billion k-mers/s. Within noise of the previous version (-0.2%).
